# istellartech/GELATO

Measured on AMD Instinct MI355X. Metric: residual+Jacobian evals/sec (and ms/eval), 6-phase x 64-node LGR mesh, higher is better.
Workload: dtype f64

## Files before the change

gelato_amd/csrc/gel_eval_kernel.h:

```cpp
#pragma once

namespace gel {

enum ParkSlot { PK_Q0 = 0, PK_Q1, PK_Q2, PK_Q3, PK_V0, PK_V1, PK_V2, PK_DJJ, PK_LV0, PK_LV1, PK_LV2,
                PK_FP0, PK_FP1, PK_FP2, PK_FP3, PK_FP4, PK_FP5, PK_FP6, PK_FP7, PK_COUNT };
constexpr int kStageLd = 17;
constexpr int kWaveLds = PK_COUNT * 64;
static_assert(kWaveLds >= 64 * kStageLd, "the MFMA staging tile must fit the wave's park region");
constexpr int kCoopStageOff = PK_LV0 * 64;
static_assert(kWaveLds - kCoopStageOff >= 64 * 11, "the cooperative hand-over area must fit behind the early park slots");
constexpr int kXldsPipeFrom = kLongPhaseFrom;
constexpr int kSlabRowsMax = 68, kPackRows = 36, kParkRes = (PK_LV2 + 1) * 64;
constexpr int kPipeSlabK = 8;
constexpr int wave_lds_doubles(bool jac, bool mfma, bool pack, bool split = false, bool longp = true) {
  return jac ? kWaveLds : (!mfma ? kParkRes : (split ? 64 * kStageLd  : (pack ? kParkRes + 4 * 64  : (longp ? 2 * 4 * kPipeSlabK * 11 + 64 * kPipeSlabK  : kSlabRowsMax * 11))));
}
static_assert(wave_lds_doubles(false, true, false, true) >= kParkRes, "residual-only split form: park over the result tile");
static_assert(wave_lds_doubles(false, true, true) >= 64 * 11 && wave_lds_doubles(false, true, false) >= 64 * 11 && wave_lds_doubles(false, true, false, false, false) >= 64 * 11, "hand-over area");
static_assert(wave_lds_doubles(false, true, true) >= kParkRes && wave_lds_doubles(false, true, false) >= kParkRes && wave_lds_doubles(false, true, false, false, false) >= kParkRes, "residual-only park");

constexpr int kSlotPT = 0, kSlotVM = 3, kSlotVP = 6;

#ifndef GEL_MIN_WAVES_PER_SIMD
#define GEL_MIN_WAVES_PER_SIMD 4
#endif
#ifndef GEL_MIN_WAVES_PER_SIMD_PACKJAC
#define GEL_MIN_WAVES_PER_SIMD_PACKJAC 4
#endif
#ifndef GEL_MIN_WAVES_PER_SIMD_RES
#define GEL_MIN_WAVES_PER_SIMD_RES 5
#endif

typedef double gel_double4 __attribute__((ext_vector_type(4)));

#ifndef GEL_CA_CACHE
#define GEL_CA_CACHE 1
#endif
#ifndef GEL_XLDS_A_PF_JAC
#define GEL_XLDS_A_PF_JAC 4
#endif
#ifndef GEL_XLDS_A_PF_RES
#define GEL_XLDS_A_PF_RES 4
#endif
#ifndef GEL_PACK_A_PRELOAD
#define GEL_PACK_A_PRELOAD 1
#endif


#ifndef GEL_XCD_RANGES
#define GEL_XCD_RANGES 1
#endif
#ifndef GEL_XCD_BLOCK
#define GEL_XCD_BLOCK 0
#endif
#ifndef GEL_FRONT_BATCH
#define GEL_FRONT_BATCH 1
#endif
#ifndef GEL_DX_HOLD7
#define GEL_DX_HOLD7 1
#endif

#ifndef GEL_STORE_AUX
#define GEL_STORE_AUX 2
#endif

#ifndef GEL_AERO_STORE_AUX
#define GEL_AERO_STORE_AUX 2
#endif

template <bool JAC, bool MFMA, bool SPLIT = false, bool PACK = false, int SPLITB = 9, bool LONGP = true, bool NTS = true, bool AERO = false>
__device__ __forceinline__ void eval_body(const ProblemDev P, int B, const double* __restrict__ x, double* __restrict__ res,
                                          double* __restrict__ jvar, const unsigned vblk) {
  extern __shared__ double lds[];
  if (MFMA) __builtin_assume(res != nullptr);
  int fB = B, f_chunk0 = P.chunk0, f_vmajor = P.vmajor, f_nchunks = P.nchunks;
  const int4* f_chunks = P.chunks;
  const PhaseDev* f_phases = P.phases;
  if (GEL_FRONT_BATCH && MFMA && !SPLIT) asm volatile("" : "+s"(fB), "+s"(f_chunk0), "+s"(f_vmajor), "+s"(f_nchunks), "+s"(f_chunks), "+s"(f_phases));
  const int park_off = P.park_off;
  constexpr bool kSplitStage = MFMA && !SPLIT;
  const double tab_mine = kSplitStage ? stage_tables_issue(P) : 0.0;
  const Tables tb = kSplitStage ? table_view(lds, P.Kw, P.Kc) : stage_tables(P, lds, true);
  const int lane = threadIdx.x & 63;
  typedef __attribute__((address_space(3))) double lds_double;
  constexpr int kWL = wave_lds_doubles(JAC, MFMA, PACK, SPLIT, LONGP);
  constexpr int kHO = JAC ? kCoopStageOff : 0;
  static_assert(!(MFMA && !SPLIT) || kWL - kHO >= 64 * 11, "the cooperative hand-over area must fit the region");
  lds_double* wave_lds = (lds_double*)lds + park_off + (threadIdx.x >> 6) * kWL;
  lds_double* park = wave_lds + lane;
#define PARK_GET(slot) park[(slot) * 64]
#define PARK_SET(slot, val) park[(slot) * 64] = (val)

  constexpr bool COOP = MFMA && !SPLIT;
  static_assert(!AERO || (JAC && MFMA && !SPLIT && !PACK), "the aero rows ride in the cooperative form with derivatives, one vector per wavefront");
  static_assert(!COOP || kBlock == 256, "the cooperative D.X form is written for four wavefronts per workgroup");
  static_assert(!PACK || COOP, "two vectors per wavefront exist in the cooperative form only");
  constexpr int kVecWg = PACK ? 8 : 4;
  const int wv = __builtin_amdgcn_readfirstlane((int)(threadIdx.x >> 6));
  const int half = PACK ? (lane >> 5) : 0;
  const int nb4 = (fB + kVecWg - 1) / kVecWg;
  const long long item = COOP ? 0 : __builtin_amdgcn_readfirstlane((int)(((long long)vblk * blockDim.x + threadIdx.x) >> 6));
  if (!COOP && item >= (long long)B * (SPLIT ? P.nunits : P.nchunks)) return;
  int q, b0;
  int4 ck_it = int4{0, 0, 0, 0};
  bool ck_same = false;
  if (COOP) {
    const unsigned p = vblk, nb = (unsigned)nb4;
    unsigned it = p / nb, r = p - it * nb;
    if (f_vmajor) {
      const unsigned xcd = p & 7u, qq = p >> 3, items = (unsigned)f_nchunks;
      const unsigned gl = qq / items;
      it = qq - gl * items;
      r = gl * 8u + xcd;
      if (r >= nb) return;
    }
    ck_it = load_const_int4(f_chunks + f_chunk0 + it);
    const int cw = __builtin_amdgcn_readfirstlane(ck_it.w);
    const unsigned pos = (unsigned)cw >> 16, nc = (unsigned)cw & 0xffffu;
    unsigned c = pos, bg = r;
    if (nc > 1) {
      const unsigned l = pos * nb + r;
      const unsigned blk = l / (8 * nc), rem = l - blk * 8 * nc;
      const unsigned m = min(8u, nb - blk * 8);
      c = rem / m;
      bg = blk * 8 + (rem - c * m);
    }
    if (GEL_XCD_RANGES && !f_vmajor) {
      const unsigned G = GEL_XCD_BLOCK ? (unsigned)GEL_XCD_BLOCK : (nb >> 3), blk8 = 8u * G;
      if (G != 0) {
        const unsigned bq = bg / blk8, inb = bg - bq * blk8;
        if ((bq + 1u) * blk8 <= nb) bg = bq * blk8 + (p & 7u) * G + (inb >> 3);
      }
    }
    q = (int)(it - pos + c);
    ck_same = GEL_FRONT_BATCH && nc <= 1;
    b0 = (int)bg * kVecWg;
  } else {
    q = (int)(item / B);
    b0 = 0;
  }
  const int bw = PACK ? b0 + 2 * wv + half : b0 + wv;
  const bool ghost = COOP && bw >= fB;
  const bool pack_full = PACK && __builtin_amdgcn_ballot_w64(ghost) == 0;
  const int b = COOP ? min(bw, fB - 1) : (int)(item - (long long)q * B);
  const int ci = SPLIT ? ((P.unit0 + q) >> 2) : q;
  const int part = SPLIT ? ((P.unit0 + q) & 3) : 0;
  int4 ck = ck_it;
  if (!ck_same) ck = COOP ? load_const_int4(f_chunks + f_chunk0 + ci) : P.chunks[(SPLIT ? 0 : P.chunk0) + ci];
  const int sec = __builtin_amdgcn_readfirstlane(ck.x);
  const int j0 = __builtin_amdgcn_readfirstlane(ck.y);
  const int dsw = __builtin_amdgcn_readfirstlane(ck.z);
  const int j = PACK ? (lane & 31) : j0 + lane;
  const PhaseDev ph = load_phase((COOP ? f_phases : P.phases) + sec);
  const bool csplit = SPLIT && MFMA && !JAC && B == 1 && res != nullptr && P.split_vel && !((P.unit0 | P.nunits) & 3);
  const bool only_dx = SPLIT && part && (!ph.air || !JAC);
  if (only_dx && !csplit) return;
  const bool lead = !(SPLIT && part);
  const int n = ph.n;
  const bool active = j < n;
  if (!MFMA && !active) return;
  const int jc = active ? j : n - 1;
  const int g = ph.ua + j;
  const int xj = ph.xa + 1 + jc;
  const int M = P.M, N = P.N;

  const double* xb = x + (size_t)b * P.nvars;
  const double* xm = xb;
  const double* xr = xb + M;
  const double* xv = xb + 4 * M;
  const double* xq = xb + 7 * M;
  const double* xu = xb + 11 * M;
  const double* xt = xb + 11 * M + 2 * N;
#define GEL_UNI(v) (PACK ? (v) : wave_uniform(v))
#ifndef GEL_KNOT_VLOAD
#define GEL_KNOT_VLOAD 1
#endif
  int sec_ld = sec;
  if (GEL_KNOT_VLOAD && JAC && !SPLIT) asm volatile("" : "+v"(sec_ld));
  const double to_ld = xt[sec_ld], tf_ld = xt[sec_ld + 1];
  double to = 0.0, tf = 0.0, fds = 0.0, fdt = 0.0;
  const double dx = P.dx, ut = P.ut;
  const double hT = P.hT;
  const double inv_dx = P.inv_dx;
#define GEL_TAKE_KNOT_TIMES()                                   \
  do {                                                          \
    to = GEL_UNI(to_ld); tf = GEL_UNI(tf_ld);                   \
    fds = GEL_UNI(inv_dx * (tf - to) * ut / 2.0);               \
    fdt = GEL_UNI(inv_dx * ut / 2.0);                           \
  } while (0)
  unsigned long long bad = 0;
#define GEL_CHK(v) (bad |= __builtin_amdgcn_ballot_w64(!(fabs(v) <= 1.79769313486231570815e308)))
  const bool packed = SPLIT && P.shard_width != 0;
  const int nn = min(64, n - j0);
  const int sub_hi = packed ? (part ? kSlotVP + 3 * (part - 1) : (ph.air ? 9 : 0)) : 0;
  const int sub_lo = (packed && part) ? sub_hi : 0;
  const int pk_nj = (ph.K - sub_hi) * nn + (j0 == 0 ? 1 : 0);
  double* const pk_out = packed ? res + (size_t)b * P.shard_width + load_const(P.unit_base + P.unit0 + q) : nullptr;
  double* rb = packed ? (lead ? pk_out : nullptr) : ((res && lead) ? res + (size_t)b * 11 * N : nullptr);
  const int gn = packed ? lane : g;
  const int rs_m = packed ? pk_nj : 0, rs_p = packed ? pk_nj + nn : N, rs_v = packed ? pk_nj + 4 * nn : 4 * N,
            rs_q = packed ? pk_nj + 7 * nn : 7 * N;
  typedef unsigned gel_u2 __attribute__((ext_vector_type(2)));
  const __amdgpu_buffer_rsrc_t jrs =
      __builtin_amdgcn_make_buffer_rsrc(JAC ? (packed ? (void*)pk_out : (void*)(jvar + (size_t)(PACK ? min(b0 + 2 * wv, B - 1) : b) * P.V + ph.voff + (size_t)j0 * ph.K)) : (void*)nullptr,
                                        0, -1, 0x00020000);
  const int jvo = PACK ? (half * (int)P.V + j) * 8 : lane * 8;
  const int cw8 = nn * 8;
#define EMIT_AT(byteoff, val)                                                           \
  do {                                                                                  \
    const double _v = (val);                                                            \
    gel_u2 _d;                                                                          \
    __builtin_memcpy(&_d, &_v, 8);                                                      \
    __builtin_amdgcn_raw_buffer_store_b64(_d, jrs, jvo, (byteoff), NTS ? GEL_STORE_AUX : 0); \
    if (!rb) GEL_CHK(_v);                                                                 \
  } while (0)
#define EMIT(slot, val) EMIT_AT(((int)(slot) - (SPLIT ? (((int)(slot) >= kSlotVP) ? sub_hi : sub_lo) : 0)) * cw8, val)
  const AeroPhaseDev* const aph = AERO ? P.aero_ph + sec : nullptr;
  const int akinds = AERO ? __builtin_amdgcn_readfirstlane(load_const(&aph->kinds)) : 0;
  const __amdgpu_buffer_rsrc_t ars =
      __builtin_amdgcn_make_buffer_rsrc(AERO ? (void*)(P.aero_out + (size_t)b * P.aero_ld) : (void*)nullptr, 0, -1, 0x00020000);
#define AEMIT(byteoff, val)                                                              \
  do {                                                                                  \
    const double _v = (val);                                                            \
    gel_u2 _d;                                                                          \
    __builtin_memcpy(&_d, &_v, 8);                                                      \
    __builtin_amdgcn_raw_buffer_store_b64(_d, ars, jvo, (byteoff), GEL_AERO_STORE_AUX); \
  } while (0)
#define RSTORE(idx, val) do { if (SPLIT) __builtin_nontemporal_store((val), rb + (idx)); else rb[idx] = (val); } while (0)
#ifndef GEL_RES_XPOSE
#define GEL_RES_XPOSE 1
#endif
  constexpr int kTileOff = JAC ? PK_FP0 * 64 : kParkRes;
  constexpr bool kCanXpose = (GEL_RES_XPOSE != 0) && (kWL >= kTileOff + 4 * 64);
#define RSTORE_LINE(ptr, val) __builtin_nontemporal_store((val), (ptr))
#define xpose (kCanXpose && (PACK ? (cw8 == 256 && pack_full) : cw8 == 512))
#define RSTORE_ROWS(tile, w, rs_off, vals)                                                                   \
  do {                                                                                                       \
    _Pragma("unroll") for (int c_ = 0; c_ < (w); c_++) GEL_CHK((vals)[c_]);                                  \
    if (xpose) {                                                                                             \
      lds_double* t_ = (tile);                                                                               \
      _Pragma("unroll") for (int c_ = 0; c_ < (w); c_++) t_[(w) * lane + c_] = (vals)[c_];                   \
      _Pragma("unroll") for (int i_ = 0; i_ < (w); i_++) {                                                   \
        const double v_ = t_[64 * i_ + lane];                                                                \
        if (PACK) {                                                                                          \
          const int e_ = 64 * i_ + lane, h_ = (e_ >= 32 * (w)) ? 1 : 0;                                      \
          double* rbh_ = res + (size_t)(b0 + 2 * wv + h_) * 11 * N;                                          \
          RSTORE_LINE(rbh_ + (rs_off) + (w) * ph.ua + (e_ - 32 * (w) * h_), v_);                             \
        } else {                                                                                             \
          RSTORE_LINE(rb + (rs_off) + (w) * (gn - lane) + 64 * i_ + lane, v_);                               \
        }                                                                                                    \
      }                                                                                                      \
    } else {                                                                                                 \
      _Pragma("unroll") for (int c_ = 0; c_ < (w); c_++) RSTORE((rs_off) + (w) * gn + c_, (vals)[c_]);       \
    }                                                                                                        \
  } while (0)
  const double inv_uv = P.inv_uv;
#define FDQ(fp, fc) (((fc) - (fp)) * fds)
  const bool coo = SPLIT && !packed && P.coo_full != nullptr;
  enum { CG_PV = 0, CG_PT, CG_VM, CG_VP, CG_VQ, CG_VT, CG_QU, CG_QT };
#define GEL_COO_BASE(g) ((size_t)load_const(P.coo + 8 * sec + (g)))
#define GEL_COO_EMIT(W, base_, vals_, okl_, twin_)                                                                     \
  do {                                                                                                                 \
    double* d_ = P.coo_full + (base_) + (size_t)(W) * j0;                                                              \
    const unsigned long long okm_ = __builtin_amdgcn_ballot_w64(okl_);                                                 \
    _Pragma("unroll") for (int c_ = 0; c_ < (W); c_++) if (!rb) GEL_CHK((vals_)[c_]);                                  \
    if (cw8 == 512) {         \
      lds_double* t_ = wave_lds + kTileOff;                                                                            \
      _Pragma("unroll") for (int c_ = 0; c_ < (W); c_++) t_[(W) * lane + c_] = (vals_)[c_];                            \
      _Pragma("unroll") for (int i_ = 0; i_ < (W); i_++) {                                                             \
        const int e_ = 64 * i_ + lane;                                                                                 \
        const double v_ = t_[e_];                                                                                      \
        const int ln_ = ((W) == 4) ? (e_ >> 2) : ((e_ * 171) >> 9);             \
        if ((okm_ >> ln_) & 1ull) {                   \
          __builtin_nontemporal_store(v_, d_ + e_);                                                                    \
          if (twin_) __builtin_nontemporal_store(-v_, d_ + e_ + (W) * n);                                              \
        }                                                                                                              \
      }                                                                                                                \
    } else if (okl_) {         \
      _Pragma("unroll") for (int c_ = 0; c_ < (W); c_++) {                                                             \
        d_[(W) * lane + c_] = (vals_)[c_];                                                                             \
        if (twin_) d_[(W) * (n + lane) + c_] = -(vals_)[c_];                                                           \
      }                                                                                                                \
    }                                                                                                                  \
  } while (0)
#define EMIT_GROUP(W, slot0, vals_, g, k, twin_, okl_)                                                                 \
  do {                                                                                                                 \
    if (coo) {                                                                                                         \
      GEL_COO_EMIT(W, GEL_COO_BASE(g) + (size_t)(W) * n * (k), vals_, okl_, twin_);                                    \
    } else if (okl_) {                                                                                                 \
      _Pragma("unroll") for (int c_ = 0; c_ < (W); c_++) EMIT((slot0) + c_, (vals_)[c_]);                              \
    }                                                                                                                  \
  } while (0)

  constexpr bool XLDS = COOP;
  double me = 0.0, re[3] = {0.0, 0.0, 0.0};
  if (!XLDS) { me = xm[xj]; re[0] = xr[3 * xj]; re[1] = xr[3 * xj + 1]; re[2] = xr[3 * xj + 2]; }
  const double tau = P.tau[ph.toff + jc];
  {
    double q[4] = {0.0, 0.0, 0.0, 0.0}, ve[3] = {0.0, 0.0, 0.0};
    if (!XLDS) {
#pragma unroll
      for (int c = 0; c < 4; c++) q[c] = xq[4 * xj + c];
#pragma unroll
      for (int c = 0; c < 3; c++) ve[c] = xv[3 * xj + c];
    }
    double u0 = 0.0, u1 = 0.0;
    if (!ph.hold) { u0 = xu[2 * (ph.ua + jc)]; u1 = xu[2 * (ph.ua + jc) + 1]; }
    const double djj = JAC ? P.Dt[ph.doff + (size_t)(jc + 1) * n + jc] : 0.0;
    const bool tail1 = MFMA && ((n + 1) & 3) == 1 && n >= 4;
    const int ksteps = tail1 ? (n >> 2) : ((n + 4) >> 2);
    const double* const dcol = P.Dt + ph.doff + (size_t)n * n;
    double dl4[4] = {0, 0, 0, 0};
    if (COOP && tail1) {
      const int rt = PACK ? (wv & 1) : wv;
#pragma unroll
      for (int i = 0; i < 4; i++) dl4[i] = dcol[min(j0 + 16 * rt + (lane >> 4) + 4 * i, n - 1)];
    }
    const double dlast = (SPLIT && tail1) ? dcol[jc] : 0.0;
    double xl[11] = {0, 0, 0, 0, 0, 0, 0, 0, 0, 0, 0};
#define GEL_DX_TAIL_ACC(nct_, xn_of_ct)                                                             \
  do {                                                                                              \
    if (tail1) {                                                                                    \
      _Pragma("unroll") for (int ct = 0; ct < 3; ct++) {                                            \
        if (ct < (nct_)) {                                   \
          const double xn_ = (xn_of_ct);                                                            \
          _Pragma("unroll") for (int i = 0; i < 4; i++) acc[ct][i] = __builtin_fma(dl4[i], xn_, acc[ct][i]); \
        }                                                                                           \
      }                                                                                             \
    }                                                                                               \
  } while (0)

    double m0 = 0.0, q0[4] = {0, 0, 0, 0};
    bool ref0_done = false;
    double lm = 0.0, lr[3] = {0, 0, 0}, lv[3] = {0, 0, 0}, lq[4] = {0, 0, 0, 0};
    if (rb || csplit) {
      if (XLDS && (PACK || !LONGP || n < kXldsPipeFrom)) {
        const int c16 = lane & 15, kq = lane >> 4;
        constexpr int kSlabK = 17, kSlabRows = 4 * kSlabK;
        static_assert(kSlabRows == kSlabRowsMax, "slab size");
        static_assert(!COOP || kSlabRows * 11 <= kWL, "a slab of state rows must fit the wave's park region");
        lds_double* regions = (lds_double*)lds + park_off;
        const bool h7 = GEL_DX_HOLD7 && !PACK && ph.hold;
        const int ncv = h7 ? 7 : 11;
        const int ncols = ncv * kVecWg;
        const int ct0 = PACK ? (h7 ? 2 : 3) * (wv >> 1) : 0;
        int xoff[3];
#pragma unroll
        for (int ct = 0; ct < 3; ct++) {
          const int c = 16 * (ct0 + ct) + c16;
          const int vb = min(h7 ? c / 7 : c / 11, kVecWg - 1);
          const int col = (c < ncols) ? c - ncv * vb : 0;
          xoff[ct] = PACK ? (vb >> 1) * kWL + (vb & 1) * kPackRows * 11 + col + kq * 11 : vb * kWL + col + kq * 11;
        }
        gel_double4 acc[3];
        const double* ap = P.Dst + (size_t)dsw * 4 + (PACK ? (wv & 1) : wv) * 64 + lane;
        constexpr int kAPF = JAC ? GEL_XLDS_A_PF_JAC : GEL_XLDS_A_PF_RES;
        constexpr int kAllN = PACK ? 9 : kSlabK;
        constexpr bool kAAll = PACK ? (GEL_PACK_A_PRELOAD != 0) : (kAPF >= kSlabK);
        double a_all[kAAll ? kAllN : 1], a_ring[kAAll ? 1 : kAPF];
        if (kAAll) {
#pragma unroll
          for (int ks = 0; ks < kAllN; ks++) a_all[ks] = ap[min(ks, ksteps - 1) * 256];
        } else {
#pragma unroll
// ... 312 lines not shown
          lm = row[0];
#pragma unroll
          for (int c = 0; c < 3; c++) { lr[c] = row[1 + c]; lv[c] = row[4 + c]; }
#pragma unroll
          for (int c = 0; c < 4; c++) lq[c] = row[7 + c];
        }
      } else if (MFMA) {
        const int c16 = lane & 15, kq = lane >> 4;
        const double* bp = xm + ph.xa;
        int bs = 1;
        if (c16 >= 1 && c16 < 4) { bp = xr + 3 * ph.xa + (c16 - 1); bs = 3; }
        if (c16 >= 4 && c16 < 7) { bp = xv + 3 * ph.xa + (c16 - 4); bs = 3; }
        if (c16 >= 7) { bp = xq + 4 * ph.xa + ((c16 < 11) ? (c16 - 7) : 0); bs = 4; }
        gel_double4 acc[4];
#pragma unroll
        for (int t = 0; t < 4; t++) acc[t] = gel_double4{0.0, 0.0, 0.0, 0.0};
        const gel_double4* ap = reinterpret_cast<const gel_double4*>(P.Dsw) + (size_t)dsw * 1 + lane;
        const unsigned un = (unsigned)n, ubs = (unsigned)bs;
        if (tail1) {
          xl[0] = xm[ph.xa + n];
#pragma unroll
          for (int c = 0; c < 3; c++) { xl[1 + c] = xr[3 * (ph.xa + n) + c]; xl[4 + c] = xv[3 * (ph.xa + n) + c]; }
#pragma unroll
          for (int c = 0; c < 4; c++) xl[7 + c] = xq[4 * (ph.xa + n) + c];
        }
        constexpr int kSplitB = SPLITB, kSplitA = 2;
        for (int k0 = 0; k0 < ksteps; k0 += kSplitB) {
          double bl[kSplitB];
          gel_double4 a4[kSplitA];
#pragma unroll
          for (int i = 0; i < kSplitB; i++) bl[i] = bp[min(4u * (k0 + i) + kq, un) * ubs];
#pragma unroll
          for (int i = 0; i < kSplitA; i++) a4[i] = ap[min(k0 + i, ksteps - 1) * 64];
#pragma unroll
          for (int i = 0; i < kSplitB; i++) {
            if (k0 + i < ksteps) {
#pragma unroll
              for (int t = 0; t < 4; t++) acc[t] = __builtin_amdgcn_mfma_f64_16x16x4f64(a4[i % kSplitA][t], bl[i], acc[t], 0, 0, 0);
              a4[i % kSplitA] = ap[min(k0 + i + kSplitA, ksteps - 1) * 64];
            }
          }
        }
#pragma unroll
        for (int t = 0; t < 4; t++)
#pragma unroll
          for (int i = 0; i < 4; i++) wave_lds[(16 * t + kq + 4 * i) * kStageLd + c16] = acc[t][i];
        lds_double* row = wave_lds + lane * kStageLd;
        lm = row[0];
#pragma unroll
        for (int c = 0; c < 3; c++) { lr[c] = row[1 + c]; lv[c] = row[4 + c]; }
#pragma unroll
        for (int c = 0; c < 4; c++) lq[c] = row[7 + c];
      } else {
        const double* Dt = P.Dt + ph.doff + j;
        const double* pm = xm + ph.xa;
        const double* pr = xr + 3 * ph.xa;
        const double* pv = xv + 3 * ph.xa;
        const double* pq = xq + 4 * ph.xa;
        for (int i = 0; i <= n; i++) {
          const double d = Dt[(size_t)i * n];
          lm += d * pm[i];
#pragma unroll
          for (int c = 0; c < 3; c++) lr[c] += d * pr[3 * i + c];
#pragma unroll
          for (int c = 0; c < 3; c++) lv[c] += d * pv[3 * i + c];
#pragma unroll
          for (int c = 0; c < 4; c++) lq[c] += d * pq[4 * i + c];
        }
      }
    }
    GEL_TAKE_KNOT_TIMES();
#undef GEL_DX_TAIL_ACC
    if (SPLIT && tail1 && rb) {
      lm = __builtin_fma(dlast, xl[0], lm);
#pragma unroll
      for (int c = 0; c < 3; c++) { lr[c] = __builtin_fma(dlast, xl[1 + c], lr[c]); lv[c] = __builtin_fma(dlast, xl[4 + c], lv[c]); }
#pragma unroll
      for (int c = 0; c < 4; c++) lq[c] = __builtin_fma(dlast, xl[7 + c], lq[c]);
    }
    if (MFMA && !active) return;
    PARK_SET(PK_Q0, q[0]); PARK_SET(PK_Q1, q[1]); PARK_SET(PK_Q2, q[2]); PARK_SET(PK_Q3, q[3]);
    PARK_SET(PK_V0, ve[0]); PARK_SET(PK_V1, ve[1]); PARK_SET(PK_V2, ve[2]);
    if (JAC) PARK_SET(PK_DJJ, djj);
    if (rb) { PARK_SET(PK_LV0, lv[0]); PARK_SET(PK_LV1, lv[1]); PARK_SET(PK_LV2, lv[2]); }
    if (!ref0_done) {
      if (rb && !ph.engine_on) m0 = xm[ph.xa];
      if (rb && ph.hold) {
#pragma unroll
        for (int c = 0; c < 4; c++) q0[c] = xq[4 * ph.xa + c];
      }
    }

    if (JAC && lead) {
      if (coo) {
        const double sc = -(P.kpt * (tf - to));
        double* d_ = P.coo_full + GEL_COO_BASE(CG_PV) + (size_t)3 * j0;
#pragma unroll
        for (int i = 0; i < 3; i++) d_[(cw8 == 512) ? 64 * i + lane : 3 * lane + i] = sc;
      } else if (j == 0) EMIT_AT(packed ? (ph.K - sub_hi) * cw8 : ph.K * n * 8, -(P.kpt * (tf - to)));
      {
        const double pt[3] = {ve[0] * P.kpt, ve[1] * P.kpt, ve[2] * P.kpt};
        EMIT_GROUP(3, kSlotPT, pt, CG_PT, 0, true, true);
      }
    }
    if (!ph.hold && lead) {
      double fq[4];
      quat_rate(q, u0, u1, P.uu, fq);
      if (rb) {
        double cq[4];
#pragma unroll
        for (int c = 0; c < 4; c++) cq[c] = lq[c] - fq[c] * (tf - to) * hT;
        RSTORE_ROWS(wave_lds + kTileOff, 4, rs_q, cq);
      }
      if (JAC && ph.q_fd) {
        double f[4];
#pragma unroll
        for (int k = 0; k < 4; k++) {
          double qp[4];
#pragma unroll
          for (int c = 0; c < 4; c++) qp[c] = (k == c) ? (q[c] + dx) : q[c];
          quat_rate(qp, u0, u1, P.uu, f);
          const int c0 = (k < 2) ? 2 : 0;
          EMIT(ph.s_qq + 2 * k, FDQ(f[c0], fq[c0]));
          EMIT(ph.s_qq + 2 * k + 1, FDQ(f[c0 + 1], fq[c0 + 1]));
        }
#pragma unroll 1
        for (int k = 0; k < 2; k++) {
          quat_rate(q, (k == 0) ? u0 + dx : u0, (k == 1) ? u1 + dx : u1, P.uu, f);
#pragma unroll
          for (int c = 0; c < 4; c++) EMIT(ph.s_qq + 8 + 4 * k + c, FDQ(f[c], fq[c]));
        }
#pragma unroll
        for (int c = 0; c < 4; c++) EMIT(ph.s_qq + 16 + c, fq[c] * hT);
      } else if (JAC) {
        const double hS = (tf - to) * ut / 2.0;
        const double d2r = 0.017453292519943295769;
        EMIT(ph.s_qq + 0, 0.5 * ((u0 * P.uu) * d2r) * hS);
        EMIT(ph.s_qq + 1, 0.5 * ((u1 * P.uu) * d2r) * hS);
        const double kq = 0.5 * (P.uu * d2r) * hS;
        if (coo) {
          const double C0 = kq * q[0], C1 = kq * q[1], C2 = kq * q[2], C3 = kq * q[3];
          const double u0v[4] = {C2, C3, -C0, -C1}, u1v[4] = {C3, -C2, C1, -C0};
          EMIT_GROUP(4, 0, u0v, CG_QU, 0, false, true);
          EMIT_GROUP(4, 0, u1v, CG_QU, 1, false, true);
        } else {
          EMIT(ph.s_qq + 2, -(kq * q[0]));
          EMIT(ph.s_qq + 3, kq * q[1]);
          EMIT(ph.s_qq + 4, kq * q[2]);
          EMIT(ph.s_qq + 5, kq * q[3]);
        }
        {
          const double qt[4] = {fq[0] * hT, fq[1] * hT, fq[2] * hT, fq[3] * hT};
          EMIT_GROUP(4, ph.s_qq + 6, qt, CG_QT, 0, true, true);
        }
      }
    }
    if (rb) {
      double cm;
      if (ph.engine_on) {
        const double rh = ph.mf_um * (tf - to) * ut / 2.0;
        cm = lm - rh;
      } else {
        cm = me - m0;
      }
      RSTORE(rs_m + gn, cm);
      GEL_CHK(cm);
      {
        double cp[3];
        const double kpos = P.kpt * (tf - to);
#pragma unroll
        for (int c = 0; c < 3; c++) cp[c] = lr[c] - ve[c] * kpos;
        RSTORE_ROWS(wave_lds + kTileOff, 3, rs_p, cp);
      }
      if (ph.hold) {
        double cq[4];
#pragma unroll
        for (int c = 0; c < 4; c++) cq[c] = q[c] - q0[c];
        RSTORE_ROWS(wave_lds + kTileOff, 4, rs_q, cq);
      }
    }
  }
  asm volatile("" ::: "memory");

  double fc[3];
  {
    const double tn = tau * (tf - to) / 2 + (tf + to) / 2;
    const double inv_m = frcp(me * P.um);

#define GEL_QUAT_CLOSED(Tval)                                                                                          \
  do {                                                                                                                 \
    const double kq_ = ((Tval) * inv_m) * (inv_uv * fds);                                                              \
    const double q_[4] = {PARK_GET(PK_Q0), PARK_GET(PK_Q1), PARK_GET(PK_Q2), PARK_GET(PK_Q3)};                         \
    _Pragma("unroll") for (int k = 0; k < 4; k++) {                                                                    \
      const double dl_ = (q_[k] + dx) - q_[k];                                                                         \
      const double a_ = (k < 2) ? -(dl_ * kq_) : dl_ * kq_;    \
      const double b_ = -2.0 * (dl_ * kq_);                                                                            \
      const double vq_[3] = {(2.0 * q_[k] + dl_) * a_,                                                                 \
                             q_[3 - k] * b_,                                    \
                             ((k & 1) ? q_[k ^ 2] : -q_[k ^ 2]) * b_};        \
      EMIT_GROUP(3, ph.s_vq + 3 * k, vq_, CG_VQ, k, false, true);                                                      \
    }                                                                                                                  \
  } while (0)
#define GEL_MASS_CLOSED(tm_)                                                                                           \
  do {                                                                                                                 \
          \
    const double e_ = (fresh_product(me + dx, P.um) - fresh_product(me, P.um)) * inv_m;                                \
    const double k_ = (e_ * (1.0 - e_ * (1.0 - e_))) * (inv_uv * fds);                                                 \
    const double vm_[3] = {(tm_)[0] * k_, (tm_)[1] * k_, (tm_)[2] * k_};                                               \
    EMIT_GROUP(3, kSlotVM, vm_, CG_VM, 0, false, true);                                                                \
  } while (0)
    if (ph.air) {
      EarthHalf eh{1.0, 0.0};
      bool have_eh = false;
#define GEL_NEED_EARTH_ANGLE(ip_, wn_, we_)                                                                            \
  do {                                                                                                                 \
    if (!have_eh && __builtin_amdgcn_ballot_w64(wind_needs_angle(ip_, wn_, we_)) != 0) {                                \
      int jl_ = jc;                                                                                                    \
      if (AERO) asm volatile("" : "+v"(jl_));    \
      const double tau_ = P.tau[ph.toff + jl_];                                                                        \
      const EarthAngle e_ = earth_angle(tau_ * (tf - to) / 2 + (tf + to) / 2);                                         \
      eh.ch = e_.ch; eh.sh = e_.sh; have_eh = true;                                                                    \
    }                                                                                                                  \
  } while (0)
      PosCentreTail pt;
      double cen_rho = 0.0, cen_P = 0.0, cen_inv_a = 0.0;
      double dir2 = 0.0;
      EarthHalf aeh{1.0, 0.0};
      bool have_aeh = false;
#ifndef GEL_AEH
#define GEL_AEH aeh
#endif
#ifndef GEL_X_NOPOS
#define GEL_X_NOPOS 0
#endif
#ifndef GEL_X_NOQUAT
#define GEL_X_NOQUAT 0
#endif
#ifndef GEL_X_NOVEL
#define GEL_X_NOVEL 0
#endif
      const bool aero_on = AERO && akinds != 0;
      const bool a_need_alpha = AERO && (akinds & 5) != 0;
#define GEL_AERO_NEED_EA(ip_, wn_, we_)                                                                                \
  do {                                                                                                                 \
    if (!have_aeh && __builtin_amdgcn_ballot_w64(wind_needs_angle(ip_, wn_, we_)) != 0) {                               \
      int jl_ = jc;                                                                                                    \
      asm volatile("" : "+v"(jl_));    \
      const double tau_ = P.tau[ph.toff + jl_];                                                                        \
      const EarthAngle e_ = earth_angle((tau_ * (tf - to) / 2 + (tf + to) / 2) * P.ut);                                \
      aeh.ch = e_.ch; aeh.sh = e_.sh; have_aeh = true;                                                                 \
    }                                                                                                                  \
  } while (0)
#define GEL_AERO_FETCH()                                                                                               \
  const int ab_[3] = {load_const(&aph->base[0]), load_const(&aph->base[1]), load_const(&aph->base[2])};                \
  const double ax_[3] = {load_const(&aph->ilx[0]), load_const(&aph->ilx[1]), load_const(&aph->ilx[2])};                \
  const int n8_ = 8 * n, j08_ = 8 * j0
#define GEL_AERO_ENTRY(blk, col, a_, nv2_, d_, ind_, rho_, okl_, a_cc, a_ac, a_qc, a_isc, a_ok)                         \
  do {                                                                                                                 \
    double t_ = 0.0, dq_ = 0.0, qp_ = 0.0;                                                                             \
    const double ac_ = a_ac;                                                                                           \
    {                                                                                                                  \
      const double qc_ = a_qc;                                                                                         \
      qp_ = 0.5 * (rho_) * (nv2_);                                                                                     \
      dq_ = qp_ - qc_;                                                                                                 \
      if (a_need_alpha) {                                                                                              \
        const double cp_ = aero_cos(a_, nv2_, d_, ind_);                                                               \
        const bool okd_ = aero_dalpha(cp_, nv2_, a_cc, a_isc, a_ok, t_);                                               \
        if (__builtin_amdgcn_ballot_w64(!okd_) != 0) {                                                                 \
          const double t2_ = aero_acos(cp_, nv2_) - ac_;                                                               \
          t_ = okd_ ? t_ : t2_;                                                                                        \
        }                                                                                                              \
      }                                                                                                                \
    }                                                                                                                  \
    _Pragma("unroll") for (int kind = 0; kind < 3; kind++) {                                                           \
      if ((blk) == 2 && kind == 1) continue;                             \
      const double df_ = (kind == 0) ? t_ : ((kind == 1) ? dq_ : qp_ * t_ + dq_ * ac_);                                \
      const double gv = -(df_ * ax_[kind]);                                                                            \
      if (okl_) AEMIT(ab_[kind] + (((blk) == 0 ? 1 : ((blk) == 1 ? 4 : 7)) + (col)) * n8_ + j08_, gv);                 \
    }                                                                                                                  \
  } while (0)
#if GEL_CA_CACHE
      Bracket ca_br = no_bracket();
#define GEL_CA_BRACKET (JAC ? &ca_br : (Bracket*)nullptr)
#else
#define GEL_CA_BRACKET nullptr
#endif
      struct ParkSink { lds_double* park; GEL_DEV void put(int i, double v) const { if (!(AERO && (i == PCS_P || i == PCS_IH))) park[(PK_FP0 + i) * 64] = v; } };
      constexpr int PK_ACC = PK_FP0 + PCS_P, PK_AAC = PK_FP0 + PCS_IH, PK_AQC = PK_LV2;
      static_assert(PCS_COUNT == 8 && PK_FP7 == PK_FP0 + 7, "PosCentre's early members fill FP0-7");
      {
        PosPart pp;
        double v[3], w[3], F[3], dir[3];
        const double r[3] = {fresh_product(re[0], P.up), fresh_product(re[1], P.up), fresh_product(re[2], P.up)};
        if (JAC) pp = pos_part<true, ParkSink>(r, tb, P.barC20, nullptr, ParkSink{park}, &pt);
        else pp = pos_part(r, tb, P.barC20);
        const bool cen_windy = AERO && __builtin_amdgcn_ballot_w64(!(pp.wn == 0.0 && pp.we == 0.0)) != 0;
        if (__builtin_amdgcn_ballot_w64(wind_needs_angle(pp.inv_p, pp.wn, pp.we)) != 0) {
          const EarthAngle e0 = earth_angle(tn);
          eh.ch = e0.ch; eh.sh = e0.sh; have_eh = true;
          if (aero_on) PARK_SET(PK_ACC, tn);
        }
        EarthAngle ea{1.0, 0.0, 1.0, 0.0};
        if (have_eh) ea = full_angle(eh);
        wind_eci_or_calm(r, ea, pp.shp, pp.chp, pp.inv_p, pp.wn, pp.we, w);
#pragma unroll
        for (int c = 0; c < 3; c++) v[c] = PARK_GET(PK_V0 + c) * P.uv;
        aero_force(r, v, pp.rho, pp.inv_a, w, ph.area, tb, F, GEL_CA_BRACKET);
#define GEL_T (ph.thrust - ph.nozzle * pp.P)
#define GEL_TDC(name) const double name[3] = {GEL_T * dir[0], GEL_T * dir[1], GEL_T * dir[2]}
        {
          const double q[4] = {PARK_GET(PK_Q0), PARK_GET(PK_Q1), PARK_GET(PK_Q2), PARK_GET(PK_Q3)};
          thrust_dir(q, dir);
        }
        double tm[3];
        {
          GEL_TDC(Tdc);
          accel_parts(Tdc, F, inv_m, pp.g, inv_uv, tm, fc);
        }
        if (rb) {
#ifndef GEL_RES_XPOSE_VEL_AIR
#define GEL_RES_XPOSE_VEL_AIR 1
#endif
          if (!JAC || GEL_RES_XPOSE_VEL_AIR) {
            double cv[3];
#pragma unroll
            for (int c = 0; c < 3; c++) cv[c] = PARK_GET(PK_LV0 + c) - fc[c] * (tf - to) * hT;
            RSTORE_ROWS(wave_lds + PK_LV0 * 64, 3, rs_v, cv);
          } else {
#pragma unroll
            for (int c = 0; c < 3; c++) {
              const double cv = PARK_GET(PK_LV0 + c) - fc[c] * (tf - to) * hT;
              RSTORE(rs_v + 3 * gn + c, cv);
              GEL_CHK(cv);
            }
          }
        }
        if (JAC) {
          asm volatile("" ::: "memory");
          PARK_SET(PK_LV0, pp.shp); PARK_SET(PK_LV1, pp.chp);
          if (!AERO) PARK_SET(PK_LV2, pp.inv_p);
        }
        if (JAC && lead && !P.fd_recompute) GEL_MASS_CLOSED(tm);
        if (JAC && ph.air_fd && (SPLIT && P.split_vel ? !lead : lead)) {
          double f[3];
          {
            const double djj = PARK_GET(PK_DJJ);
#pragma unroll
            for (int k = 0; k < 3; k++) {
              if (SPLIT && P.split_vel && k != part - 1) continue;
              double vp[3], Fp[3];
#pragma unroll
              for (int c = 0; c < 3; c++) vp[c] = ((k == c) ? (PARK_GET(PK_V0 + c) + dx) : PARK_GET(PK_V0 + c)) * P.uv;
              const double r[3] = {fresh_product(re[0], P.up), fresh_product(re[1], P.up), fresh_product(re[2], P.up)};
              aero_force(r, vp, pp.rho, pp.inv_a, w, ph.area, tb, Fp, GEL_CA_BRACKET);
              GEL_TDC(Tdc);
              accel(Tdc, Fp, inv_m, pp.g, inv_uv, f);
#pragma unroll
              for (int c = 0; c < 3; c++) EMIT(ph.s_vv + 3 * k + c, ((c == k) ? djj : 0.0) + FDQ(f[c], fc[c]));
            }
          }
        }
        if (JAC && lead) {
          double f[3];
          if (!P.fd_recompute) {
            GEL_QUAT_CLOSED(GEL_T);
          } else if (P.fd_recompute) {
            const double q[4] = {PARK_GET(PK_Q0), PARK_GET(PK_Q1), PARK_GET(PK_Q2), PARK_GET(PK_Q3)};
#pragma unroll 1
            for (int k = 0; k < 4; k++) {
              double qp[4];
#pragma unroll
              for (int c = 0; c < 4; c++) qp[c] = (k == c) ? (q[c] + dx) : q[c];
              double dp[3];
              thrust_dir(qp, dp);
              const double Td[3] = {GEL_T * dp[0], GEL_T * dp[1], GEL_T * dp[2]};
              accel(Td, F, inv_m, pp.g, inv_uv, f);
#pragma unroll
              for (int c = 0; c < 3; c++) EMIT(ph.s_vq + 3 * k + c, FDQ(f[c], fc[c]));
            }
            GEL_TDC(Tdc);
            accel(Tdc, F, frcp((me + dx) * P.um), pp.g, inv_uv, f);
#pragma unroll
            for (int c = 0; c < 3; c++) EMIT(kSlotVM + c, FDQ(f[c], fc[c]));
          }
          if (!ph.t_fd) {
            const double vt[3] = {fc[0] * hT, fc[1] * hT, fc[2] * hT};
            EMIT_GROUP(3, ph.s_vt, vt, CG_VT, 0, true, true);
          }
        }
        if (aero_on) {
          asm volatile("" ::: "memory");
          const double ra[3] = {fresh_product(re[0], P.up), fresh_product(re[1], P.up), fresh_product(re[2], P.up)};
          double va[3], wa[3], a0[3];
#pragma unroll
          for (int c = 0; c < 3; c++) va[c] = PARK_GET(PK_V0 + c) * P.uv;
          if (have_eh) {
            const EarthAngle e1 = earth_angle(PARK_GET(PK_ACC) * P.ut);
            aeh.ch = e1.ch; aeh.sh = e1.sh; have_aeh = true;
          }
          if (cen_windy) {
            PosCentre pcx;
            double wn_, we_, p_, ip_, ih_;
            pos_centre_tail(pt, pp.rho, pp.P, tb, pcx, wn_, we_);
            geodetic_p_ih(ra[0], ra[1], ra[2], p_, ip_, ih_);
            EarthAngle e2{1.0, 0.0, 1.0, 0.0};
            if (have_aeh) e2 = full_angle(GEL_AEH);
            wind_eci(ra, e2, PARK_GET(PK_LV0), PARK_GET(PK_LV1), ip_, wn_, we_, wa);
          } else {
            wa[0] = 0.0; wa[1] = 0.0; wa[2] = 0.0;
          }
          const double nv2 = aero_vair2(ra, va, wa, a0);
          const double ind = frsqrt(fmax(dir[0] * dir[0] + dir[1] * dir[1] + dir[2] * dir[2], 1.0e-300));
          const double cc = a_need_alpha ? aero_cos(a0, nv2, dir, ind) : 0.0;
          const double alpha_c = a_need_alpha ? aero_acos(cc, nv2) : 0.0;
          const double qdyn_c = 0.5 * pp.rho * nv2;
          double sc, isc;
          fsqrt_rsqrt(fmax((1.0 - cc) * (1.0 + cc), 1.0e-300), sc, isc);
          const bool centre_ok = (cc <= 1.0) && (nv2 >= 1.0e-12) && (sc > 1.0e-6);
          GEL_AERO_FETCH();
          const double ail_[3] = {load_const(&aph->il[0]), load_const(&aph->il[1]), load_const(&aph->il[2])};
#pragma unroll
          for (int kind = 0; kind < 3; kind++) {
            const double il = ail_[kind];
            const double cv = 1.0 - ((kind == 0) ? alpha_c : (kind == 1) ? qdyn_c : qdyn_c * alpha_c) * il;
            AEMIT(ab_[kind] + j08_, cv);
            GEL_CHK(cv);
          }
          if (a_need_alpha && !GEL_X_NOQUAT) {
            const double q[4] = {PARK_GET(PK_Q0), PARK_GET(PK_Q1), PARK_GET(PK_Q2), PARK_GET(PK_Q3)};
#pragma unroll
            for (int c = 0; c < 4; c++) {
              double qp[4], dp[3];
#pragma unroll
              for (int d = 0; d < 4; d++) qp[d] = (d == c) ? q[d] + dx : q[d];
              thrust_dir(qp, dp);
              const double indp = frsqrt(fmax(dp[0] * dp[0] + dp[1] * dp[1] + dp[2] * dp[2], 1.0e-300));
              GEL_AERO_ENTRY(2, c, a0, nv2, dp, indp, pp.rho, true, cc, alpha_c, qdyn_c, isc, centre_ok);
              __builtin_amdgcn_sched_barrier(0);
            }
          }
#pragma unroll
          for (int c = 0; c < (GEL_X_NOVEL ? 0 : 3); c++) {
            double vp[3], a[3];
#pragma unroll
            for (int d = 0; d < 3; d++) vp[d] = ((d == c) ? PARK_GET(PK_V0 + d) + dx : PARK_GET(PK_V0 + d)) * P.uv;
            const double nv2p = aero_vair2(ra, vp, wa, a);
            GEL_AERO_ENTRY(1, c, a, nv2p, dir, ind, pp.rho, true, cc, alpha_c, qdyn_c, isc, centre_ok);
            __builtin_amdgcn_sched_barrier(0);
          }
          PARK_SET(PK_ACC, cc); PARK_SET(PK_AAC, centre_ok ? alpha_c : -alpha_c); PARK_SET(PK_AQC, qdyn_c);
        }
        if (JAC) {
          asm volatile("" ::: "memory");
          PARK_SET(PK_Q0, fc[0]); PARK_SET(PK_Q1, fc[1]); PARK_SET(PK_Q2, fc[2]); PARK_SET(PK_Q3, dir[0]); PARK_SET(PK_DJJ, dir[1]);
          dir2 = dir[2];
          cen_rho = pp.rho; cen_P = pp.P; cen_inv_a = pp.inv_a;
        }
#undef GEL_TDC
#undef GEL_T
      }
      if (JAC && (!SPLIT || part)) {
        const int k0 = SPLIT ? part - 1 : 0, k1 = SPLIT ? part : 3;
#define GEL_POS_SWEEP_F(rp, pq, f_)                                                                           \
  do {                                                                                                        \
    double wq_[3], Fp_[3];                                                                                    \
    GEL_NEED_EARTH_ANGLE((pq).inv_p, (pq).wn, (pq).we);                                                       \
    EarthAngle ea{1.0, 0.0, 1.0, 0.0};                                                                        \
    if (have_eh) ea = full_angle(eh);                                                                         \
    wind_eci_or_calm(rp, ea, (pq).shp, (pq).chp, (pq).inv_p, (pq).wn, (pq).we, wq_);                          \
    const double vq_[3] = {PARK_GET(PK_V0) * P.uv, PARK_GET(PK_V1) * P.uv, PARK_GET(PK_V2) * P.uv};           \
    aero_force(rp, vq_, (pq).rho, (pq).inv_a, wq_, ph.area, tb, Fp_, GEL_CA_BRACKET);                         \
    const double Tp_ = ph.thrust - ph.nozzle * (pq).P;                                                        \
    const double Td_[3] = {Tp_ * PARK_GET(PK_Q3), Tp_ * PARK_GET(PK_DJJ), Tp_ * dir2};                        \
    accel(Td_, Fp_, inv_m, (pq).g, inv_uv, f_);                                                               \
  } while (0)
#define GEL_POS_SWEEP_EMIT(kk, f_, okl_)                                                                      \
  do {                                                                                                        \
    const double vp_[3] = {FDQ((f_)[0], PARK_GET(PK_Q0)), FDQ((f_)[1], PARK_GET(PK_Q1)), FDQ((f_)[2], PARK_GET(PK_Q2))}; \
    EMIT_GROUP(3, kSlotVP + 3 * (kk), vp_, CG_VP, kk, false, okl_);                                           \
  } while (0)
#define GEL_AERO_POS(kk, rp, pq, okl_)                                                                        \
  do {                                                                                                        \
    double wq_[3], a_[3];                                                                                     \
    GEL_AERO_NEED_EA((pq).inv_p, (pq).wn, (pq).we);                                                           \
    EarthAngle ea_{1.0, 0.0, 1.0, 0.0};                                                                       \
    if (have_aeh) ea_ = full_angle(GEL_AEH);                                                                  \
    wind_eci_or_calm(rp, ea_, (pq).shp, (pq).chp, (pq).inv_p, (pq).wn, (pq).we, wq_);                         \
    const double vq_[3] = {PARK_GET(PK_V0) * P.uv, PARK_GET(PK_V1) * P.uv, PARK_GET(PK_V2) * P.uv};           \
    const double nv2_ = aero_vair2(rp, vq_, wq_, a_);                                                         \
    const double dd_[3] = {PARK_GET(PK_Q3), PARK_GET(PK_DJJ), dir2};                                          \
    const double ind_ = frsqrt(fmax(dd_[0] * dd_[0] + dd_[1] * dd_[1] + dd_[2] * dd_[2], 1.0e-300));          \
    const double cc_ = PARK_GET(PK_ACC);                                                                      \
    double sc_, isc_;                                                                                         \
    fsqrt_rsqrt(fmax((1.0 - cc_) * (1.0 + cc_), 1.0e-300), sc_, isc_);                                        \
    const double acs_ = PARK_GET(PK_AAC);    \
    GEL_AERO_FETCH();                                                                                         \
    GEL_AERO_ENTRY(0, kk, a_, nv2_, dd_, ind_, (pq).rho, okl_, cc_, fabs(acs_), PARK_GET(PK_AQC), isc_, !__builtin_signbit(acs_)); \
  } while (0)
#define GEL_LOAD_POS_CENTRE(pc, pcv)                                                                                   \
  PosCentre pc;                                                                                                        \
  pc.ihy = PARK_GET(PK_FP0 + PCS_IHY);                                                                                 \
  pc.sl = PARK_GET(PK_FP0 + PCS_SL); pc.cl = PARK_GET(PK_FP0 + PCS_CL); pc.icl = PARK_GET(PK_FP0 + PCS_ICL);           \
  pc.N = PARK_GET(PK_FP0 + PCS_N); pc.G = PARK_GET(PK_FP0 + PCS_G);                                                    \
  PosPart pcv;                                                                                                         \
  pcv.rho = cen_rho; pcv.P = cen_P; pcv.inv_a = cen_inv_a;                                                             \
  pcv.shp = PARK_GET(PK_LV0); pcv.chp = PARK_GET(PK_LV1);                                                              \
  if (AERO) {                                                                                                          \
    geodetic_p_ih(fresh_product(re[0], P.up), fresh_product(re[1], P.up), fresh_product(re[2], P.up), pc.p, pcv.inv_p, pc.ih); \
  } else {                                                                                                             \
    pc.p = PARK_GET(PK_FP0 + PCS_P); pc.ih = PARK_GET(PK_FP0 + PCS_IH); pcv.inv_p = PARK_GET(PK_LV2);                  \
  }                                                                                                                    \
  pos_centre_tail(pt, cen_rho, cen_P, tb, pc, pcv.wn, pcv.we)
        unsigned todo = 0;
        unsigned long long coo_okm = 0;
        if (P.fd_recompute) {
          todo = ((1u << k1) - 1u) & ~((1u << k0) - 1u);
        } else {
#pragma unroll
          for (int k = k0; k < k1; k++) {
            asm volatile("" ::: "memory");
            GEL_LOAD_POS_CENTRE(pc, pcv);
            const double r[3] = {fresh_product(re[0], P.up), fresh_product(re[1], P.up), fresh_product(re[2], P.up)};
            double rp[3];
#pragma unroll
            for (int c = 0; c < 3; c++) rp[c] = (k == c) ? (re[c] + dx) * P.up : r[c];
            const double dlt = (k == 0) ? rp[0] - r[0] : ((k == 1) ? rp[1] - r[1] : rp[2] - r[2]);
            PosPart pq;
            const bool ok = pos_delta(r, k, dlt, pcv, pc, tb, pq);
            if (coo) coo_okm = __builtin_amdgcn_ballot_w64(ok);
            if (__builtin_amdgcn_ballot_w64(!ok) != 0) {
              todo |= 1u << k;
              if (__builtin_amdgcn_ballot_w64(ok) == 0) continue;
            }
            gravity_eci(rp, P.barC20, pq.g);
            double f[3];
            GEL_POS_SWEEP_F(rp, pq, f);
            GEL_POS_SWEEP_EMIT(k, f, ok);
            if (aero_on && !GEL_X_NOPOS) GEL_AERO_POS(k, rp, pq, ok);
          }
        }
        if (todo) {
#pragma unroll 1
          for (int k = k0; k < k1; k++) {
            if (!((todo >> k) & 1u)) continue;
            asm volatile("" ::: "memory");
            double rp[3];
#pragma unroll
            for (int c = 0; c < 3; c++) rp[c] = fresh_product((k == c) ? re[c] + dx : re[c], P.up);
            bool ok = false;
            if (!P.fd_recompute && coo) {
              ok = ((coo_okm >> lane) & 1ull) != 0;
            } else if (!P.fd_recompute) {
              GEL_LOAD_POS_CENTRE(pc, pcv);
              const double r[3] = {fresh_product(re[0], P.up), fresh_product(re[1], P.up), fresh_product(re[2], P.up)};
              const double dlt = (k == 0) ? rp[0] - r[0] : ((k == 1) ? rp[1] - r[1] : rp[2] - r[2]);
              PosPart pd;
              ok = pos_delta(r, k, dlt, pcv, pc, tb, pd);
            }
            asm volatile("" ::: "memory");
            PosPart pq = pos_part(rp, tb, P.barC20);
            double f[3];
            GEL_POS_SWEEP_F(rp, pq, f);
            GEL_POS_SWEEP_EMIT(k, f, !ok);
            if (aero_on && !GEL_X_NOPOS) GEL_AERO_POS(k, rp, pq, !ok);
          }
        }
#undef GEL_AERO_POS
#undef GEL_LOAD_POS_CENTRE
#undef GEL_NEED_EARTH_ANGLE
#undef GEL_AERO_NEED_EA
#undef GEL_AERO_ENTRY
#undef GEL_AERO_FETCH
#undef GEL_POS_SWEEP_F
#undef GEL_POS_SWEEP_EMIT
      }
      if (JAC && lead && ph.t_fd) {
        asm volatile("" ::: "memory");
        const double fcc[3] = {PARK_GET(PK_Q0), PARK_GET(PK_Q1), PARK_GET(PK_Q2)};
        int jl2 = jc;
        if (AERO) asm volatile("" : "+v"(jl2));
        const double tau2 = P.tau[ph.toff + jl2];
        {
          const double r[3] = {fresh_product(re[0], P.up), fresh_product(re[1], P.up), fresh_product(re[2], P.up)};
          const PosPart p2 = pos_part(r, tb, P.barC20);
          const double T2 = ph.thrust - ph.nozzle * p2.P;
          PARK_SET(PK_FP0, p2.shp); PARK_SET(PK_FP1, p2.chp); PARK_SET(PK_FP2, p2.inv_p); PARK_SET(PK_FP3, p2.wn); PARK_SET(PK_FP4, p2.we);
          PARK_SET(PK_FP5, p2.rho); PARK_SET(PK_FP6, p2.inv_a);
          PARK_SET(PK_LV0, p2.g[0]); PARK_SET(PK_LV1, p2.g[1]); PARK_SET(PK_LV2, p2.g[2]);
          PARK_SET(PK_Q0, T2 * PARK_GET(PK_Q3)); PARK_SET(PK_Q1, T2 * PARK_GET(PK_DJJ)); PARK_SET(PK_Q2, T2 * dir2);
        }
#pragma unroll 1
        for (int k = 0; k < 2; k++) {
          asm volatile("" ::: "memory");
          const double to_p = (k == 0) ? to + dx : to;
          const double tf_p = (k == 1) ? tf + dx : tf;
          const double tnp = tau2 * (tf_p - to_p) / 2 + (tf_p + to_p) / 2;
          const EarthAngle eq = earth_angle(tnp);
          double wq[3], Fp[3], f[3];
          const double rq[3] = {re[0] * P.up, re[1] * P.up, re[2] * P.up};
          wind_eci_chain_or_calm(rq, eq, PARK_GET(PK_FP0), PARK_GET(PK_FP1), PARK_GET(PK_FP2), PARK_GET(PK_FP3), PARK_GET(PK_FP4), wq);
          const double vq[3] = {PARK_GET(PK_V0) * P.uv, PARK_GET(PK_V1) * P.uv, PARK_GET(PK_V2) * P.uv};
          aero_force(rq, vq, PARK_GET(PK_FP5), PARK_GET(PK_FP6), wq, ph.area, tb, Fp, GEL_CA_BRACKET);
          const double Tq[3] = {PARK_GET(PK_Q0), PARK_GET(PK_Q1), PARK_GET(PK_Q2)};
          const double gq[3] = {PARK_GET(PK_LV0), PARK_GET(PK_LV1), PARK_GET(PK_LV2)};
          accel(Tq, Fp, inv_m, gq, inv_uv, f);
#pragma unroll
          for (int c = 0; c < 3; c++)
            EMIT(ph.s_vt + 3 * k + c, (fcc[c] * (tf - to) - f[c] * (tf_p - to_p)) * fdt);
        }
      }
    } else {
      const double T = ph.thrust;
      double dir[3];
      {
        const double q[4] = {PARK_GET(PK_Q0), PARK_GET(PK_Q1), PARK_GET(PK_Q2), PARK_GET(PK_Q3)};
        thrust_dir(q, dir);
      }
      const double Td[3] = {T * dir[0], T * dir[1], T * dir[2]};
      double gc[3];
      {
        const double r[3] = {re[0] * P.up, re[1] * P.up, re[2] * P.up};
        gravity_eci(r, P.barC20, gc);
      }
      double tm[3];
#pragma unroll
      for (int c = 0; c < 3; c++) { tm[c] = Td[c] * inv_m; fc[c] = (tm[c] + gc[c]) * inv_uv; }
      if (rb) {
        double cv[3];
#pragma unroll
        for (int c = 0; c < 3; c++) cv[c] = PARK_GET(PK_LV0 + c) - fc[c] * (tf - to) * hT;
        RSTORE_ROWS(wave_lds + PK_LV0 * 64, 3, rs_v, cv);
      }
      if (JAC) {
        double f[3];
        if (!P.fd_recompute) {
          GEL_MASS_CLOSED(tm);
        } else {
          accel_noair(Td, frcp((me + dx) * P.um), gc, inv_uv, f);
#pragma unroll
          for (int c = 0; c < 3; c++) EMIT(kSlotVM + c, FDQ(f[c], fc[c]));
        }
#pragma unroll
        for (int k = 0; k < 3; k++) {
          double r[3], gp[3];
#pragma unroll
          for (int c = 0; c < 3; c++) r[c] = ((k == c) ? (re[c] + dx) : re[c]) * P.up;
          gravity_eci(r, P.barC20, gp);
          accel_noair(Td, inv_m, gp, inv_uv, f);
          const double vp[3] = {FDQ(f[0], fc[0]), FDQ(f[1], fc[1]), FDQ(f[2], fc[2])};
          EMIT_GROUP(3, kSlotVP + 3 * k, vp, CG_VP, k, false, true);
        }
        if (!P.fd_recompute) {
          GEL_QUAT_CLOSED(T);
        } else {
          const double q[4] = {PARK_GET(PK_Q0), PARK_GET(PK_Q1), PARK_GET(PK_Q2), PARK_GET(PK_Q3)};
#pragma unroll 1
          for (int k = 0; k < 4; k++) {
            double qp[4];
#pragma unroll
            for (int c = 0; c < 4; c++) qp[c] = (k == c) ? (q[c] + dx) : q[c];
            double dp[3];
            thrust_dir(qp, dp);
            const double Tp[3] = {T * dp[0], T * dp[1], T * dp[2]};
            accel_noair(Tp, inv_m, gc, inv_uv, f);
#pragma unroll
            for (int c = 0; c < 3; c++) EMIT(ph.s_vq + 3 * k + c, FDQ(f[c], fc[c]));
          }
        }
        {
          const double vt[3] = {fc[0] * hT, fc[1] * hT, fc[2] * hT};
          EMIT_GROUP(3, ph.s_vt, vt, CG_VT, 0, true, true);
        }
      }
    }
  }
#undef EMIT_GROUP
#undef GEL_COO_EMIT
#undef GEL_COO_BASE
#undef EMIT
#undef GEL_CA_BRACKET
#undef GEL_QUAT_CLOSED
#undef GEL_MASS_CLOSED
#undef AEMIT
#undef EMIT_AT
#undef RSTORE
#undef RSTORE_ROWS
#undef RSTORE_LINE
#undef xpose
#undef FDQ
#undef GEL_CHK
#undef GEL_UNI
#undef GEL_TAKE_KNOT_TIMES
#undef PARK_GET
#undef PARK_SET
  if (bad) *(volatile int32_t*)P.flag = 1;
}

__device__ __forceinline__ void signal_done(const ProblemDev& P) {
  if (!P.done_flag) return;
  __threadfence_system();
  __syncthreads();
  if (threadIdx.x == 0) {
    const int old = __hip_atomic_fetch_add(P.done_ctr, 1, __ATOMIC_ACQ_REL, __HIP_MEMORY_SCOPE_AGENT);
    if (old == P.done_total - 1) {
      __hip_atomic_store(P.done_ctr, 0, __ATOMIC_RELAXED, __HIP_MEMORY_SCOPE_AGENT);
      __hip_atomic_store(P.done_flag, P.done_seq, __ATOMIC_RELEASE, __HIP_MEMORY_SCOPE_SYSTEM);
    }
  }
}

template <bool JAC, bool MFMA, bool SPLIT = false, bool PACK = false, bool LONGP = true, bool NTS = true, bool AERO = false>
__global__ __launch_bounds__(kBlock, (!JAC && PACK) ? GEL_MIN_WAVES_PER_SIMD_RES : ((JAC && PACK) ? GEL_MIN_WAVES_PER_SIMD_PACKJAC : GEL_MIN_WAVES_PER_SIMD)) void eval_kernel(ProblemDev P, int B, const double* __restrict__ x,
                                                      double* __restrict__ res, double* __restrict__ jvar) {
  eval_body<JAC, MFMA, SPLIT, PACK, 9, LONGP, NTS, AERO>(P, B, x, res, jvar, blockIdx.x);
  if constexpr (SPLIT) signal_done(P);
}

}
```

gelato_amd/csrc/gel_host.hip:

```cpp
#include <hip/hip_runtime.h>

#include <algorithm>
#include <cmath>
#include <cstdio>
#include <chrono>
#include <atomic>
#include <cstdlib>
#include <cstring>
#include <memory>
#include <string>
#include <thread>
#include <vector>

#include "gel_host_handle.h"

namespace gelhost {
namespace {
thread_local std::string g_err;
}
int fail(int code, const std::string& msg) {
  g_err = msg;
  return code;
}
}
// ... 1036 lines not shown
        const int64_t nn = std::min(64, h.n - j0);
        const int skip = h.air ? 9 : 0;
        usize[4 * item] = (int64_t)(h.K - skip) * nn + (j0 == 0 ? 1 : 0) + 11 * nn;
        for (int k = 1; k < 4; k++) usize[4 * item + k] = h.air ? 3 * nn : 0;
      }
  }
  std::vector<int64_t> base(nunits, 0);
  int64_t w = 0;
  for (int r = 0; r < nranks; r++) {
    int64_t off = 0;
    for (int u = unit_begin[r]; u < unit_begin[r + 1]; u++) { base[u] = off; off += usize[u]; }
    w = std::max(w, off);
  }
  w = (w + 1) & ~(int64_t)1;
  {
    int item = 0;
    for (const HostPhase& h : p->ph)
      for (int j0 = 0; j0 < h.n; j0 += 64, item++) {
        const int nn = std::min(64, h.n - j0);
        const int skip = h.air ? 9 : 0;
        const int64_t nj = (int64_t)(h.K - skip) * nn + (j0 == 0 ? 1 : 0);
        const int u0 = 4 * item;
        const int64_t b0 = (int64_t)urank[u0] * w + base[u0];
        for (int jl = 0; jl < nn; jl++) {
          const int j = j0 + jl, g = h.ua + j;
          pos[g] = b0 + nj + jl;
          for (int c = 0; c < 3; c++) { pos[N + 3 * g + c] = b0 + nj + nn + 3 * jl + c; pos[4 * N + 3 * g + c] = b0 + nj + 4 * nn + 3 * jl + c; }
          for (int c = 0; c < 4; c++) pos[7 * N + 4 * g + c] = b0 + nj + 7 * nn + 4 * jl + c;
          for (int sl = 0; sl < h.K; sl++) {
            const int part = (h.air && sl >= 6 && sl < 15) ? 1 + (sl - 6) / 3 : 0;
            const int u = u0 + part;
            const int local = part ? sl - (6 + 3 * (part - 1)) : (sl >= 6 ? sl - skip : sl);
            pos[(size_t)11 * N + compact_index(h, sl, j)] = (int64_t)urank[u] * w + base[u] + (int64_t)local * nn + jl;
          }
        }
        if (j0 == 0) pos[(size_t)11 * N + h.voff + (int64_t)h.K * h.n] = b0 + (int64_t)(h.K - skip) * nn;
      }
  }
  for (int64_t v : pos)
    if (v < 0) return fail(GEL_ERR_ARG, "shard plan: an output entry without an owner (internal)");
  DeviceArray<int64_t> d_base, d_pos;
  if (p->device != GEL_DEVICE_NONE) {
    HIPCHK(hipSetDevice(p->device));
    HIPCHK(d_base.upload(base)); HIPCHK(d_pos.upload(pos));
    HIPCHK(drain(p));
  }
  p->d_unit_base = std::move(d_base);
  p->d_shard_pos = std::move(d_pos);
  p->shard_begin.assign(unit_begin, unit_begin + nranks + 1);
  p->unit_base = base;
  p->shard_width = w;
  *width = w;
  if (res_pos) std::memcpy(res_pos, pos.data(), sizeof(int64_t) * 11 * (size_t)N);
  if (jvar_pos) std::memcpy(jvar_pos, pos.data() + (size_t)11 * N, sizeof(int64_t) * (size_t)V);
  return GEL_OK;
}

static int check_plan(const gel_problem* p, int32_t nranks, int64_t width) {
  if (p->shard_width <= 0) return fail(GEL_ERR_ARG, "gel_shard_plan has not been called on this handle");
  if (nranks != (int32_t)p->shard_begin.size() - 1 || width != p->shard_width)
    return fail(GEL_ERR_ARG, "the handle's shard plan is not the one this buffer was sized for (gel_shard_plan was called again: plan once more, or use one handle per plan)");
  return GEL_OK;
}

int gel_eval_shard_packed_device(gel_problem* p, int32_t B, const double* d_x, double* d_out, int32_t rank, int32_t nranks_expected,
                                 int64_t width_expected, void* stream) {
  if (!p || !d_x || !d_out || B < 1) return fail(GEL_ERR_ARG, "bad argument");
  NO_EXACT(p, "gel_eval_shard_packed_device");
  NEED_DEVICE(p, GEL_ERR_HIP, kNoGpu);
  if (int rc = check_plan(p, nranks_expected, width_expected)) return rc;
  if (!p->d_unit_base.get()) return fail(GEL_ERR_ARG, "gel_shard_plan has not been called on this handle");
  const int nranks = (int)p->shard_begin.size() - 1;
  if (rank < 0 || rank >= nranks) return fail(GEL_ERR_ARG, "rank outside the plan");
  const int32_t u0 = p->shard_begin[rank], cnt = p->shard_begin[rank + 1] - u0;
  if (cnt == 0) return GEL_OK;
  gel::ProblemDev dv = p->dev;
  dv.chunks = p->d_chunks.get();
  dv.chunk0 = 0;
  dv.unit0 = u0;
  dv.nunits = cnt;
  dv.shard_width = p->shard_width;
  dv.unit_base = p->d_unit_base.get();
  double* slice = d_out + (size_t)rank * (size_t)B * (size_t)p->shard_width;
  HIPCHK(gel::launch_eval(dv, B, d_x, slice, slice, stream_of(p, stream)));
  return GEL_OK;
}

int gel_shard_unpack_device(gel_problem* p, int32_t B, const double* d_out, double* d_res, double* d_jvar, int32_t nranks_expected,
                            int64_t width_expected, void* stream) {
  if (!p || !d_out || B < 1 || (!d_res && !d_jvar)) return fail(GEL_ERR_ARG, "bad argument");
  NEED_DEVICE(p, GEL_ERR_HIP, kNoGpu);
  if (int rc = check_plan(p, nranks_expected, width_expected)) return rc;
  if (!p->d_shard_pos.get()) return fail(GEL_ERR_ARG, "gel_shard_plan has not been called on this handle");
  HIPCHK(gel::launch_shard_unpack(11 * p->dims.N, p->dims.num_var_entries, p->shard_width, B, p->d_shard_pos.get(), d_out, d_res, d_jvar,
                                  stream_of(p, stream)));
  return GEL_OK;
}

int gel_fill_full_device(gel_problem* p, int32_t B, double* d_jfull, void* stream) {
  if (!p || !d_jfull || B < 1) return fail(GEL_ERR_ARG, "bad argument");
  NEED_DEVICE(p, GEL_ERR_HIP, kNoGpu);
  HIPCHK(gel::launch_fill_full(p->dims.total_nnz, B, p->d_cval.get(), d_jfull, stream_of(p, stream)));
  return GEL_OK;
}

int gel_update_full_device(gel_problem* p, int32_t B, const double* d_jvar, double* d_jfull, void* stream) {
  if (!p || !d_jvar || !d_jfull || B < 1) return fail(GEL_ERR_ARG, "bad argument");
  NEED_DEVICE(p, GEL_ERR_HIP, kNoGpu);
  HIPCHK(gel::launch_update_full(p->dims.total_nnz, p->dims.num_var_entries, p->nvar_entries, B, p->d_vdst.get(), p->d_vsrc.get(),
                                 p->nvar_lines, p->d_vline.get(), p->d_src.get(), p->d_cval.get(), d_jvar, d_jfull,
                                 stream_of(p, stream)));
  return GEL_OK;
}

int gel_eval_full_device(gel_problem* p, int32_t B, const double* d_x, double* d_res, double* d_jvar, double* d_jfull, void* stream) {
  if (!p || !d_x || !d_jvar || !d_jfull || B < 1) return fail(GEL_ERR_ARG, "bad argument");
  NEED_DEVICE(p, GEL_ERR_HIP, kNoGpu);
  hipStream_t s = stream_of(p, stream);
  gel::ProblemDev dv = p->dev;
  dv.cached_out = 1;
  HIPCHK(launch_defects(p, dv, B, d_x, d_res, d_jvar, s));
  HIPCHK(gel::launch_update_full(p->dims.total_nnz, p->dims.num_var_entries, p->nvar_entries, B, p->d_vdst.get(), p->d_vsrc.get(),
                                 p->nvar_lines, p->d_vline.get(), p->d_src.get(), p->d_cval.get(), d_jvar, d_jfull, s));
  return GEL_OK;
}

int gel_expand_full_device(gel_problem* p, int32_t B, const double* d_jvar, double* d_jfull, void* stream) {
  if (!p || !d_jvar || !d_jfull || B < 1) return fail(GEL_ERR_ARG, "bad argument");
  NEED_DEVICE(p, GEL_ERR_HIP, kNoGpu);
  HIPCHK(gel::launch_expand(p->dims.total_nnz, p->dims.num_var_entries, B, p->d_cval.get(), p->d_src.get(), d_jvar, d_jfull,
                            stream_of(p, stream)));
  return GEL_OK;
}

int gel_sync(gel_problem* p, void* stream) {
  if (!p) return fail(GEL_ERR_ARG, "null argument");
  NEED_DEVICE(p, GEL_ERR_HIP, kNoGpu);
  hipStream_t s = stream_of(p, stream);
  HIPCHK(hipMemcpyAsync(p->h_flag.get(), p->d_flag.get(), 4, hipMemcpyDeviceToHost, s));
  HIPCHK(hipStreamSynchronize(s));
  int rc = GEL_OK;
  if (*p->h_flag.get()) {
    HIPCHK(clear_flag(p, s));
    *p->h_flag.get() = 0;
    rc = GEL_NONFINITE;
  }
  if (s == p->caller_stream) p->caller_stream = nullptr;
  return rc;
}

int gel_output_table(gel_problem* p, const double* x, const double* tx_res, double launch_lat_deg, double launch_lon_deg,
                     double* out) {
  if (!p || !x || !tx_res || !out) return fail(GEL_ERR_ARG, "null argument");
  NEED_DEVICE(p, GEL_ERR_HIP, kNoGpu);
  HIPCHK(hipSetDevice(p->device));
  const int M = p->dims.M;
  std::vector<int32_t> sec((size_t)M);
  for (size_t i = 0; i < p->ph.size(); i++)
    for (int k = 0; k <= p->ph[i].n; k++) sec[(size_t)p->ph[i].xa + k] = (int32_t)i;
  const size_t nx = (size_t)p->dims.num_vars, no = (size_t)M * gel::kOutputColumns;
  return staged_call(p, kStagedNoFlag, {staged_in(x, nx), staged_in(tx_res, (size_t)M), staged_in(sec.data(), (size_t)M), staged_out(out, no)},
                     [&](const gel::ProblemDev&, double* const* a) -> int {
                       HIPCHK(gel::launch_output(p->dev, M, a[0], a[1], reinterpret_cast<const int32_t*>(a[2]), launch_lat_deg, launch_lon_deg,
                                                 a[3], p->stream.get()));
                       return GEL_OK;
                     });
}

int gel_initial_guess(const gel_problem* p, int32_t nref, const double* t_ref, const double* table,
                      const double* knot_times, double* x) {
  if (!p || !t_ref || !table || !knot_times || !x || nref < 2) return fail(GEL_ERR_ARG, "bad argument (>= 2 reference rows)");
  for (int k = 1; k < nref; k++)
    if (!(t_ref[k] >= t_ref[k - 1])) return fail(GEL_ERR_ARG, "reference times must not decrease");
  const int S = p->dims.S, M = p->dims.M, N = p->dims.N;
  auto interp = [&](double t, int col0, int ncol, double unit, double* out) {
    int hi = (int)(std::lower_bound(t_ref, t_ref + nref, t) - t_ref);
    hi = std::min(std::max(hi, 1), nref - 1);
    const int lo = hi - 1;
    for (int c = 0; c < ncol; c++) {
      const double ylo = table[(size_t)lo * 13 + col0 + c], yhi = table[(size_t)hi * 13 + col0 + c];
      const double slope = (yhi - ylo) / (t_ref[hi] - t_ref[lo]);
      const double rise = slope * (t - t_ref[lo]);
      out[c] = (rise + ylo) / unit;
    }
  };
  double* xm = x; double* xr = x + M; double* xv = x + 4 * (size_t)M; double* xq = x + 7 * (size_t)M;
  double* xu = x + 11 * (size_t)M; double* xt = x + 11 * (size_t)M + 2 * (size_t)N;
  for (int i = 0; i < S; i++) {
    const HostPhase& h = p->ph[i];
    const double to = knot_times[i], tf = knot_times[i + 1];
    for (int k = 0; k <= h.n; k++) {
      const double tau = (k == 0) ? -1.0 : h.tau[k - 1];
      const double t = tau * (tf - to) / 2.0 + (tf + to) / 2.0;
      const int node = h.xa + k;
      interp(t, 0, 1, p->um, xm + node);
      interp(t, 1, 3, p->up, xr + 3 * (size_t)node);
      interp(t, 4, 3, p->uv, xv + 3 * (size_t)node);
      interp(t, 7, 4, 1.0, xq + 4 * (size_t)node);
    }
    for (int k = 0; k < h.n; k++) {
      const double t = h.tau[k] * (tf - to) / 2.0 + (tf + to) / 2.0;
      interp(t, 11, 2, p->uu, xu + 2 * (size_t)(h.ua + k));
    }
  }
  for (int i = 0; i <= S; i++) xt[i] = knot_times[i] / p->ut;
  for (int64_t i = 0; i < p->dims.num_vars; i++)
    if (!std::isfinite(x[i])) return GEL_NONFINITE;
  return GEL_OK;
}

int gel_eval_callback(gel_problem* p, const double* x, const gel_callback_io* io) {
  if (!p || !x || !io) return fail(GEL_ERR_ARG, "null argument");
  NEED_DEVICE(p, GEL_ERR_HIP, kNoGpu);
  HIPCHK(hipSetDevice(p->device));
  int rc = ensure_capacity(p, 1);
  if (rc) return rc;
  const size_t nlin = p->lin_rows.size(), nfn = p->fn_rows.size(), R = nlin + nfn;
  const bool rows = io->rows_con && R;
  size_t off_c[3], off_j[3], atotal = 0;
  bool aero = false;
  for (int k = 0; k < 3; k++) {
    const size_t n = p->aero.rows[k].size();
    off_c[k] = atotal; atotal += (io->aero_con[k] && n) ? n : 0;
    off_j[k] = atotal; atotal += (io->aero_con[k] && n && io->aero_jac[k]) ? aero_jac_len(p, k) : 0;
    aero = aero || (io->aero_con[k] && n);
  }
  const size_t nrows_out = rows ? R + 7 * nfn : 0;
  if (rows || aero) HIPCHK(p->h_arena.reserve(nrows_out + atotal));
  double* const h_rows = p->h_arena.get();
  double* const h_aero = h_rows + nrows_out;
  const bool x_pinned = p->cb_x[0].get() && (x == p->cb_x[0].get() || x == p->cb_x[1].get());
  if (!x_pinned) std::memcpy(p->h_x.get(), x, (size_t)p->dims.num_vars * 8);
  const double* const xin = x_pinned ? x : p->h_x.get();
  gel::ProblemDev dv = p->dev;
  dv.flag = p->h_flag.get();
  const bool want_jac = io->vals_full != nullptr;
  const bool fused = io->res || want_jac;
  static const int cb_mode = [] { const char* e = getenv("GEL_CB_MODE"); return e ? atoi(e) : 0; }();
  const bool split_exact = p->exact && want_jac;
  bool aero_jac = false;
  for (int k = 0; k < 3; k++) aero_jac = aero_jac || (io->aero_con[k] && io->aero_jac[k] && !p->aero.rows[k].empty());
  const bool split_aero = p->exact_aero && aero_jac;
  const bool split_rows = p->exact_rows && rows && io->rows_jfn;
  const bool coo = want_jac && cb_mode != 3 && !p->exact && !split_aero && !split_rows && coo_direct(p);
  if (coo) {
    if ((rc = ensure_full(p))) return rc;
    dv.coo_full = p->h_full.get(); dv.coo = p->d_coo.get();
  }
  dv.split_vel = 1;
  const bool own_res = io->res && p->cb_res.get() && io->res == p->cb_res.get();
  double* const res_to = own_res ? p->cb_res.get() : p->h_res.get();
  gel::AeroLaunchOut out;
  if (aero)
    for (int k = 0; k < 3; k++) {
      const size_t n = p->aero.rows[k].size();
      out.nrows[k] = (int32_t)n;
      out.con[k] = (io->aero_con[k] && n) ? h_aero + off_c[k] : nullptr;
      out.jac[k] = (out.con[k] && io->aero_jac[k]) ? h_aero + off_j[k] : nullptr;
    }
  if (cb_mode == 3 || !fused || split_exact || split_aero || split_rows) {
    if (fused) HIPCHK(launch_defects(p, dv, 1, xin, res_to, want_jac ? p->h_jv.get() : nullptr, p->stream.get()));
    if (rows) HIPCHK(launch_rows_kinds(p, dv, 1, xin, h_rows, io->rows_jfn ? h_rows + R : nullptr, p->stream.get()));
    if (aero) HIPCHK(launch_aero_kinds(p, dv, (int)p->aero.nodes.size(), p->aero.d_nodes.get(), 1, xin, out, p->stream.get()));
  } else {
    arm_done(p, dv);
    HIPCHK(gel::launch_callback(dv, want_jac, xin, res_to, want_jac ? p->h_jv.get() : nullptr,
                                aero ? (int)p->aero.nodes.size() : 0, p->aero.d_nodes.get(), aero ? &out : nullptr,
                                (int)nlin, p->d_lin_rows.get(), (int)nfn, p->d_fn_rows.get(), rows ? h_rows : nullptr,
                                (rows && io->rows_jfn) ? h_rows + R : nullptr, p->stream.get()));
  }
  HIPCHK(wait_done(p, dv));
  if (io->res && !own_res) std::memcpy(io->res, p->h_res.get(), (size_t)11 * p->dims.N * 8);
  if (want_jac) {
    if (coo) finish_full(p, io->vals_full, io->fill_constants);
    else scatter_full(p, p->h_jv.get(), io->vals_full, io->fill_constants);
  }
  if (rows) {
    std::memcpy(io->rows_con, h_rows, R * 8);
    if (io->rows_jfn) std::memcpy(io->rows_jfn, h_rows + R, 7 * nfn * 8);
  }
  if (aero)
    for (int k = 0; k < 3; k++) {
      if (out.con[k]) std::memcpy(io->aero_con[k], out.con[k], p->aero.rows[k].size() * 8);
      if (out.jac[k]) std::memcpy(io->aero_jac[k], out.jac[k], aero_jac_len(p, k) * 8);
    }
  if (*p->h_flag.get()) { *p->h_flag.get() = 0; return GEL_NONFINITE; }
  return GEL_OK;
}

int gel_table_limits(int32_t wind_rows, int32_t ca_rows, int32_t n, int64_t* info) {
  if (wind_rows < 2 || ca_rows < 2 || !info) return fail(GEL_ERR_ARG, "bad argument");
  const size_t T = gel::staged_table_doubles(wind_rows, ca_rows), Tp = gel::padded_table_doubles(wind_rows, ca_rows);
  info[0] = (int64_t)T;
  info[1] = (int64_t)lds_room(gel::eval_lds_bytes_max(wind_rows, ca_rows) / 8 - Tp, true);
  info[2] = (int64_t)lds_room(gel::aero_lds_bytes(wind_rows, ca_rows) / 8 - Tp, true);
  info[3] = (n >= 2 && n < gel::kMeshMaxThreads) ? (int64_t)lds_room(gel::mesh_vector_doubles(n), true) : -1;
  info[4] = (int64_t)lds_room(gel::table_lds_bytes(wind_rows, ca_rows) / 8 - T, false);
  info[5] = (int64_t)gel::kLaunchMaxLds;
  info[6] = info[3] < 0 ? -1 : (int64_t)gel::mesh_vectors_per_group(wind_rows, ca_rows, n);
  return GEL_OK;
}

int gel_point_eval(int32_t kind, int32_t n, const double* in, const double* aux, int32_t aux_rows, double* out) {
  static const int nin[16] = {1, 3, 3, 6, 7, 1, 1, 2, 2, 8, 8, 8, 7, 4, 1, 5}, nout[16] = {5, 3, 3, 3, 3, 3, 1, 4, 6, 8, 16, 4, 3, 7, 2, 18};
  if (kind < 0 || kind > 15 || n < 0 || !in || !out) return fail(GEL_ERR_ARG, "bad argument");
  if (n == 0) return GEL_OK;
  const bool tabulated = kind == 5 || kind == 6 || kind == 9 || kind == 10 || kind == 15;
  int rc = tabulated ? check_launch_lds("gel_point_eval", gel::point_lds_bytes(aux_rows), 5 * (size_t)std::max(aux_rows, 0), 5 * (size_t)std::max(aux_rows, 0), false) : GEL_OK;
  if (rc) return rc;
  rc = need_device();
  if (rc) return rc;
  double atm[gel::kAtmTableDoubles];
  size_t naux = 0;
  const double* hax = aux;
  std::vector<double> ext;
  if (kind == 0) { gel::fill_atmosphere_table(atm); hax = atm; naux = gel::kAtmTableDoubles; aux_rows = 0; }
  else if (kind == 2) { if (!aux) return fail(GEL_ERR_ARG, "kind 2 needs aux[0] = barC20"); naux = 1; aux_rows = 0; }
  else if (tabulated) {
    const int w = (kind == 5 || kind == 10 || kind == 15) ? 3 : 2;
    if (!aux || aux_rows < 2) return fail(GEL_ERR_ARG, "kinds 5, 6, 9, 10 and 15 need a table of at least two rows");
    if (kind == 15) { gel::fill_atmosphere_table(atm); ext.assign(atm, atm + gel::kAtmTableDoubles); }
    for (int k = 1; k < aux_rows; k++)
      if (!(aux[(size_t)w * k] > aux[(size_t)w * (k - 1)])) return fail(GEL_ERR_ARG, "table abscissae must increase strictly");
    std::vector<double> slopes;
    gel::append_rows_and_slopes(ext, slopes, aux, aux_rows, w);
    ext.insert(ext.end(), slopes.begin(), slopes.end());
    hax = ext.data(); naux = ext.size();
  }
  else { aux_rows = 0; }
  DeviceArray<double> i, a, o;
  HIPCHK(i.upload(in, (size_t)n * nin[kind])); HIPCHK(a.upload(hax, naux)); HIPCHK(o.reserve((size_t)n * nout[kind]));
  HIPCHK(gel::launch_point(kind, n, i.get(), a.get(), aux_rows, o.get(), nullptr));
  HIPCHK(hipMemcpy(out, o.get(), (size_t)n * nout[kind] * 8, hipMemcpyDeviceToHost));
  return GEL_OK;
}

}
```

gelato_amd/csrc/gel_kernels.hip:

```cpp
#include <hip/hip_runtime.h>

#include "gel_tables.h"
#include "gel_output_row.h"

#include "gel_eval_kernel.h"
namespace gel {

constexpr int kExpandGroup = 8;
__global__ __launch_bounds__(kBlock) void expand_kernel(long long nnz, long long V, int B, const double* __restrict__ cval,
                                                        const int32_t* __restrict__ src,
                                                        const double* __restrict__ jvar, double* __restrict__ full) {
  const int b0 = blockIdx.y * kExpandGroup;
  const int nb = min(kExpandGroup, B - b0);
  const bool even = (nnz & 1) == 0;
  for (long long i = 2 * ((long long)blockIdx.x * kBlock + threadIdx.x); i < nnz; i += 2LL * gridDim.x * kBlock) {
    const bool two = i + 1 < nnz;
    const int s0 = src[i], s1 = two ? src[i + 1] : -1;
    const double c0 = (s0 == -1) ? cval[i] : 0.0, c1 = (two && s1 == -1) ? cval[i + 1] : 0.0;
    const int g0 = (s0 >= 0) ? s0 : -2 - s0, g1 = (s1 >= 0) ? s1 : -2 - s1;
    for (int g = 0; g < nb; g++) {
      const double* jv = jvar + (size_t)(b0 + g) * V;
      double* out = full + (size_t)(b0 + g) * nnz + i;
      const double v0 = (s0 == -1) ? c0 : ((s0 >= 0) ? jv[g0] : -jv[g0]);
      const double v1 = (s1 == -1) ? c1 : ((s1 >= 0) ? jv[g1] : -jv[g1]);
      if (two && (even || ((b0 + g) & 1) == 0)) {
        typedef double gel_d2 __attribute__((ext_vector_type(2)));
        __builtin_nontemporal_store(gel_d2{v0, v1}, reinterpret_cast<gel_d2*>(out));
      } else {
        __builtin_nontemporal_store(v0, out);
        if (two) __builtin_nontemporal_store(v1, out + 1);
      }
    }
  }
}

__global__ __launch_bounds__(kBlock) void update_full_kernel(long long nnz, long long V, int nvar, int B, const int32_t* __restrict__ vdst,
                                                             const int32_t* __restrict__ vsrc, const double* __restrict__ jvar,
                                                             double* __restrict__ full) {
  const int i = blockIdx.x * kBlock + threadIdx.x;
  if (i >= nvar) return;
  const int d = vdst[i], s = vsrc[i];
  const int g = (s >= 0) ? s : -2 - s;
  for (int b = blockIdx.y; b < B; b += gridDim.y) {
    const double v = jvar[(size_t)b * V + g];
    full[(size_t)b * nnz + d] = (s >= 0) ? v : -v;
  }
}
__global__ __launch_bounds__(kBlock) void update_lines_kernel(long long nnz, long long V, int nlines, int B, const int32_t* __restrict__ vline,
                                                              const int32_t* __restrict__ src, const double* __restrict__ cval,
                                                              const double* __restrict__ jvar, double* __restrict__ full) {
  const int t = blockIdx.x * kBlock + threadIdx.x;
  if (t >= 8 * nlines) return;
  const long long i = 8LL * vline[t >> 3] + (t & 7);
  const int s = src[i];
  const double c = (s == -1) ? cval[i] : 0.0;
  const int g = (s >= 0) ? s : -2 - s;
  for (int b = blockIdx.y; b < B; b += gridDim.y) {
    double v = c;
    if (s != -1) { const double w = jvar[(size_t)b * V + g]; v = (s >= 0) ? w : -w; }
    __builtin_nontemporal_store(v, full + (size_t)b * nnz + i);
  }
}
__global__ __launch_bounds__(kBlock) void fill_full_kernel(long long nnz, int B, const double* __restrict__ cval, double* __restrict__ full) {
  for (long long i = (long long)blockIdx.x * kBlock + threadIdx.x; i < nnz; i += (long long)gridDim.x * kBlock) {
    const double c = cval[i];
    for (int b = blockIdx.y; b < B; b += gridDim.y) __builtin_nontemporal_store(c, full + (size_t)b * nnz + i);
  }
}

__global__ void perturb_local_kernel(int nloc, double dx, const double* __restrict__ x, const int32_t* __restrict__ colmap,
                                     double* __restrict__ Xp) {
  const long long t = (long long)blockIdx.x * blockDim.x + threadIdx.x;
  if (t >= (long long)(nloc + 1) * nloc) return;
  const int row = (int)(t / nloc), col = (int)(t - (long long)row * nloc);
  double v = x[colmap[col]];
  if (row == col + 1) v += dx;
  Xp[t] = v;
}

__global__ void quotient_local_kernel(int nloc, int nres, int roff, int nrows, double dx, const double* __restrict__ res,
                                      double* __restrict__ J, long long ldJ, int row0, const int32_t* __restrict__ colmap) {
  __shared__ double tile[32][33];
  const int c0 = blockIdx.x * 32, r0 = blockIdx.y * 32;
  for (int k = threadIdx.y; k < 32; k += blockDim.y) {
    const int c = c0 + k, r = r0 + threadIdx.x;
    if (c < nloc && r < nrows) tile[k][threadIdx.x] = res[(size_t)(c + 1) * nres + roff + r];
  }
  __syncthreads();
  for (int k = threadIdx.y; k < 32; k += blockDim.y) {
    const int r = r0 + k, c = c0 + threadIdx.x;
    if (c < nloc && r < nrows) J[(size_t)(row0 + r) * ldJ + (colmap ? colmap[c] : c)] = (tile[threadIdx.x][k] - res[roff + r]) / dx;
  }
}

struct RhsArgs {
  int n, Kw, Kc;
  const double *mass_e, *pos_e, *vel_e, *quat, *t, *tables;
  double thrust, area, nozzle, um, up, uv, barC20;
  double* out;
};

__global__ void rhs_vel_air_kernel(RhsArgs A) {
  extern __shared__ double lds[];
  ProblemDev P{};
  P.Kw = A.Kw; P.Kc = A.Kc; P.tables = A.tables;
  const Tables tb = stage_tables(P, lds);
  const int i = blockIdx.x * blockDim.x + threadIdx.x;
  if (i >= A.n) return;
  const double m = A.mass_e[i] * A.um;
  const double r[3] = {A.pos_e[3 * i] * A.up, A.pos_e[3 * i + 1] * A.up, A.pos_e[3 * i + 2] * A.up};
  const double v[3] = {A.vel_e[3 * i] * A.uv, A.vel_e[3 * i + 1] * A.uv, A.vel_e[3 * i + 2] * A.uv};
  const double q[4] = {A.quat[4 * i], A.quat[4 * i + 1], A.quat[4 * i + 2], A.quat[4 * i + 3]};
  const PosPart pp = pos_part(r, tb, A.barC20);
  const EarthAngle ea = earth_angle(A.t[i]);
  double w[3], F[3], dir[3], f[3];
  wind_eci(r, ea, pp.shp, pp.chp, pp.inv_p, pp.wn, pp.we, w);
  aero_force(r, v, pp.rho, pp.inv_a, w, A.area, tb, F);
  thrust_dir(q, dir);
  const double T = A.thrust - A.nozzle * pp.P;
  const double Td[3] = {T * dir[0], T * dir[1], T * dir[2]};
  accel(Td, F, 1.0 / m, pp.g, 1.0 / A.uv, f);
  for (int c = 0; c < 3; c++) A.out[3 * i + c] = f[c];
}

__global__ void rhs_vel_noair_kernel(RhsArgs A) {
  const int i = blockIdx.x * blockDim.x + threadIdx.x;
  if (i >= A.n) return;
  const double m = A.mass_e[i] * A.um;
  const double r[3] = {A.pos_e[3 * i] * A.up, A.pos_e[3 * i + 1] * A.up, A.pos_e[3 * i + 2] * A.up};
  const double q[4] = {A.quat[4 * i], A.quat[4 * i + 1], A.quat[4 * i + 2], A.quat[4 * i + 3]};
  double dir[3], g[3], f[3];
  thrust_dir(q, dir);
  gravity_eci(r, A.barC20, g);
  const double Td[3] = {A.thrust * dir[0], A.thrust * dir[1], A.thrust * dir[2]};
  accel_noair(Td, 1.0 / m, g, 1.0 / A.uv, f);
  for (int c = 0; c < 3; c++) A.out[3 * i + c] = f[c];
}

__global__ void rhs_quat_kernel(int n, const double* quat, const double* u_e, double unit_u, double* out) {
  const int i = blockIdx.x * blockDim.x + threadIdx.x;
  if (i >= n) return;
  const double q[4] = {quat[4 * i], quat[4 * i + 1], quat[4 * i + 2], quat[4 * i + 3]};
  double dq[4];
  quat_rate(q, u_e[2 * i], u_e[2 * i + 1], unit_u, dq);
  for (int c = 0; c < 4; c++) out[4 * i + c] = dq[c];
}

__global__ void point_kernel(int kind, int n, const double* in, const double* aux, int aux_rows, double* out) {
  extern __shared__ double lds[];
  const int naux = (kind == 5 || kind == 10) ? 3 * aux_rows + 2 * (aux_rows - 1)
                   : (kind == 6 || kind == 9) ? 2 * aux_rows + (aux_rows - 1)
                   : (kind == 15) ? kAtmDoubles + 3 * aux_rows + 2 * (aux_rows - 1) : (kind == 0 ? kAtmDoubles : 0);
  for (int i = threadIdx.x; i < naux; i += blockDim.x) lds[i] = aux[i];
  __syncthreads();
  const int i = blockIdx.x * blockDim.x + threadIdx.x;
  if (i >= n) return;
  switch (kind) {
    case 0: {
      const double h = geopotential_altitude(in[i]);
      const Air a = atmosphere(h, lds);
      out[5 * i] = h; out[5 * i + 1] = a.T; out[5 * i + 2] = a.P; out[5 * i + 3] = a.rho; out[5 * i + 4] = a.a;
    } break;
    case 1: {
      double lat, sl, cl, p, ip;
      geodetic_lat_p(in[3 * i], in[3 * i + 1], in[3 * i + 2], lat, p, ip);
      geodetic_sincos_p(in[3 * i], in[3 * i + 1], in[3 * i + 2], sl, cl, p, ip);
      const double lon = atan2(in[3 * i + 1], in[3 * i]);
      out[3 * i] = lat * 180.0 / kPi; out[3 * i + 1] = lon * 180.0 / kPi;
      out[3 * i + 2] = geodetic_alt_from(p, sl, cl);
    } break;
    case 2: {
      const double r[3] = {in[3 * i], in[3 * i + 1], in[3 * i + 2]};
      double g[3];
      gravity_eci(r, aux[0], g);
      out[3 * i] = g[0]; out[3 * i + 1] = g[1]; out[3 * i + 2] = g[2];
    } break;
    case 3: {
      const double* a = in + 6 * i;
      const double r[3] = {a[0], a[1], a[2]};
      double sl, cl, p, ip, w[3];
      geodetic_sincos_p(r[0], r[1], r[2], sl, cl, p, ip);
      const EarthAngle ea = earth_angle(a[3]);
      double chp, irt;
      fsqrt_rsqrt(0.5 * (1.0 + cl), chp, irt);
      wind_eci(r, ea, (0.5 * sl) * irt, chp, ip, a[4], a[5], w);
      out[3 * i] = w[0]; out[3 * i + 1] = w[1]; out[3 * i + 2] = w[2];
    } break;
    case 4: {
      const double* a = in + 7 * i;
      double s, c;
      sincos(kOmega * a[6], &s, &c);
      const double d0 = a[0] - (0.0 * a[5] - kOmega * a[4]);
      const double d1 = a[1] - (kOmega * a[3] - 0.0 * a[5]);
      const double d2 = a[2] - (0.0 * a[4] - 0.0 * a[3]);
      out[3 * i] = d0 * c + d1 * s; out[3 * i + 1] = -d0 * s + d1 * c; out[3 * i + 2] = d2;
    } break;
    case 5: {
      double wn, we;
      wind_ned2(in[i], lds, lds + 3 * aux_rows, aux_rows, wn, we);
      out[3 * i] = wn; out[3 * i + 1] = we; out[3 * i + 2] = 0.0;
    } break;
    case 6: out[i] = interp_tab(in[i], lds, lds + 2 * aux_rows, aux_rows, 2, 1); break;
    case 7: {
      const double a = in[2 * i], b = in[2 * i + 1];
      out[4 * i] = fsqrt(a); out[4 * i + 1] = sqrt(a); out[4 * i + 2] = fdiv(a, b); out[4 * i + 3] = a / b;
    } break;
    case 8: {
      double s1, c1, s2, c2;
      fsincos(in[2 * i], &s1, &c1);
      sincos(in[2 * i], &s2, &c2);
      out[6 * i] = s1; out[6 * i + 1] = c1; out[6 * i + 2] = s2; out[6 * i + 3] = c2;
      out[6 * i + 4] = flog_ratio(in[2 * i + 1]); out[6 * i + 5] = log(in[2 * i + 1]);
    } break;
    case 9: {
      Bracket br = no_bracket();
      for (int k = 0; k < 8; k++) out[8 * i + k] = interp_tab_cached(in[8 * i + k], lds, lds + 2 * aux_rows, aux_rows, 2, 1, br);
    } break;
    case 10: {
      Bracket2 br = no_bracket2();
      for (int k = 0; k < 8; k++) {
        double wn, we;
        wind_ned2_cached(in[8 * i + k], lds, lds + 3 * aux_rows, aux_rows, wn, we, br);
        out[16 * i + 2 * k] = wn; out[16 * i + 2 * k + 1] = we;
      }
    } break;
    case 11: {
      double o[4];
      quatmult(in + 8 * i, in + 8 * i + 4, o);
      for (int c = 0; c < 4; c++) out[4 * i + c] = o[c];
    } break;
    case 12: {
      double o[3];
      quatrot(in + 7 * i, in + 7 * i + 4, o);
      for (int c = 0; c < 3; c++) out[3 * i + c] = o[c];
    } break;
    case 13: {
      const double* q = in + 4 * i;
      out[7 * i] = q[0]; out[7 * i + 1] = -q[1]; out[7 * i + 2] = -q[2]; out[7 * i + 3] = -q[3];
      double d[3];
      thrust_dir(q, d);
      for (int c = 0; c < 3; c++) out[7 * i + 4 + c] = d[c];
    } break;
    case 14: out[2 * i] = fexp(in[i]); out[2 * i + 1] = exp(in[i]); break;
    case 15: {
      Tables tb;
      tb.atm = lds; tb.wind = lds + kAtmDoubles; tb.winds = tb.wind + 3 * aux_rows; tb.ca = nullptr; tb.cas = nullptr;
      tb.Kw = aux_rows; tb.Kc = 0;
      const double* a = in + 5 * i;
      const double r[3] = {a[0], a[1], a[2]};
      const int kk = min(max((int)a[3], 0), 2);
      PosCentre pc;
      PosCentreTail pt;
      PosPart pp = pos_part<true, PosCentreSink, false>(r, tb, 0.0, nullptr, PosCentreSink{&pc}, &pt);
      pos_centre_tail(pt, pp.rho, pp.P, tb, pc, pp.wn, pp.we);
      PosPart pq;
      const bool ok = pos_delta(r, kk, a[4], pp, pc, tb, pq);
      double* o = out + 18 * i;
      o[0] = pp.rho; o[1] = pp.P; o[2] = pp.inv_a; o[3] = pp.wn; o[4] = pp.we; o[5] = pp.shp; o[6] = pp.chp; o[7] = pp.inv_p;
      o[8] = pq.rho; o[9] = pq.P; o[10] = pq.inv_a; o[11] = pq.wn; o[12] = pq.we; o[13] = pq.shp; o[14] = pq.chp; o[15] = pq.inv_p;
      o[16] = ok ? 1.0 : 0.0; o[17] = pc.margin;
    } break;
    default: break;
  }
}

struct AeroPos {
  double rho;
  double wn, we;
  double shp, chp, inv_p;
};

GEL_DEV AeroPos aero_pos_part(const double r[3], const Tables& tb) {
  AeroPos o;
  double lat, p, sl, cl;
  geodetic_lat_p(r[0], r[1], r[2], lat, p, o.inv_p);
  fsincos(lat, &sl, &cl);
  const double h = geopotential_altitude(geodetic_alt_from(p, sl, cl));
  wind_ned2(h, tb.wind, tb.winds, tb.Kw, o.wn, o.we);
  double irt;
  fsqrt_rsqrt(0.5 * (1.0 + cl), o.chp, irt);
  o.shp = (0.5 * sl) * irt;
  o.rho = atmosphere(h, tb.atm).rho;
  return o;
}

GEL_DEV double aero_vair(const double r[3], const double v[3], const EarthAngle& ea, const double w[3], double a[3]) {
  const double d0 = v[0] + kOmega * r[1], d1 = v[1] - kOmega * r[0];
  const double e0 = d0 * ea.c + d1 * ea.s, e1 = -d0 * ea.s + d1 * ea.c;
  a[0] = (e0 * ea.c - e1 * ea.s) - w[0]; a[1] = (e0 * ea.s + e1 * ea.c) - w[1]; a[2] = v[2] - w[2];
  return sqrt(a[0] * a[0] + a[1] * a[1] + a[2] * a[2]);
}

GEL_DEV double aero_alpha(const double a[3], double nv, const double q[4]) {
  double dir[3];
  thrust_dir(q, dir);
  const double nd = sqrt(dir[0] * dir[0] + dir[1] * dir[1] + dir[2] * dir[2]);
  const double c_alpha = (a[0] / nv) * (dir[0] / nd) + (a[1] / nv) * (dir[1] / nd) + (a[2] / nv) * (dir[2] / nd);
  return (c_alpha > 1.0) ? 0.0 : ((nv < 1e-6) ? 0.0 : acos(c_alpha));
}

struct AeroOut {
  double* con[3];
  double* jac[3];
  int32_t nrows[3];
  int64_t ld;
  int32_t sm;
};

#ifndef GEL_AERO_UNROLL
#define GEL_AERO_UNROLL 1
#endif
constexpr int kAeroWaves = 4;
enum { AP_ILIM = 0, AP_AC = 3, AP_QC, AP_CC, AP_IS, AP_IND, AP_W = 8, AP_A0 = 11, AP_DIR = 14, AP_RHO = 17, AP_NV2 = 18, AP_INTS = 19,
       kAeroParkSlots = 25 };
static_assert(wave_lds_doubles(false, false, false) <= kWaveLds && wave_lds_doubles(false, true, false, true) <= kWaveLds &&
              wave_lds_doubles(false, true, true) <= kWaveLds && wave_lds_doubles(false, true, false, false, true) <= kWaveLds &&
              wave_lds_doubles(false, true, false, false, false) <= kWaveLds, "kWaveLds is the largest region");
static size_t eval_lds_bytes(size_t park_off, int wave_doubles) { return sizeof(double) * (park_off + (size_t)wave_doubles * (kBlock / 64)); }
size_t eval_lds_bytes_max(int Kw, int Kc) { return eval_lds_bytes(padded_table_doubles(Kw, Kc), kWaveLds); }
size_t aero_lds_bytes(int Kw, int Kc) { return sizeof(double) * (padded_table_doubles(Kw, Kc) + (size_t)kAeroWaves * kAeroParkSlots * 64); }
typedef __attribute__((address_space(3))) int lds_int;
typedef __attribute__((address_space(3))) double lds_f64;
template <bool ROLES, bool WIDE = false, bool SM = false>
__device__ __forceinline__ void aero_body(const ProblemDev P, int nnodes, const AeroNodeDev* __restrict__ nodes, int tiles, int B,
                                          const double* __restrict__ x, const AeroOut O, const unsigned vblk) {
  extern __shared__ double lds[];
  const Tables tb = stage_tables(P, lds);
  const int lane = (int)(threadIdx.x & 63);
  const int sw = ROLES ? (int)(threadIdx.x >> 6) : -1;
  const long long wid = ROLES ? (long long)vblk : (long long)vblk * kAeroWaves + __builtin_amdgcn_readfirstlane((int)(threadIdx.x >> 6));
  const bool flat = !ROLES && !WIDE && tiles == 0;
  int b, ni_raw;
  bool live;
  if (WIDE) {
    const long long total = (long long)B * nnodes, f = wid * 64 + lane;
    if (wid * 64 >= total) return;
    live = f < total;
    const long long fc = live ? f : total - 1;
    b = (int)(fc / nnodes);
    ni_raw = live ? (int)(fc - (long long)b * nnodes) : nnodes;
  } else if (flat) {
    const long long total = (long long)B * nnodes, f0 = wid * 64;
    if (f0 >= total) return;
    const int b0 = (int)(f0 / nnodes), r0 = (int)(f0 - (long long)b0 * nnodes);
    const bool wrap = r0 + lane >= nnodes;
    live = f0 + lane < total;
    b = live ? (wrap ? b0 + 1 : b0) : b0;
    ni_raw = live ? (wrap ? r0 + lane - nnodes : r0 + lane) : nnodes;
  } else {
    if (wid >= (long long)B * tiles) return;
    b = (int)(wid / tiles);
    ni_raw = (int)(wid - (long long)b * tiles) * 64 + lane;
    live = ni_raw < nnodes;
  }
  const int ni = live ? ni_raw : nnodes - 1;
  const AeroNodeDev Nd = nodes[ni];
  const PhaseDev& ph = P.phases[Nd.phase];
  const double* xb = x + (size_t)b * P.nvars;
  const int M = P.M, N = P.N, xi = ph.xa + Nd.k;
  const double dx = P.dx;
  double re[3];
#pragma unroll
  for (int c = 0; c < 3; c++) re[c] = xb[M + 3 * xi + c];
  const bool want_jac = O.jac[0] || O.jac[1] || O.jac[2];
  const bool need_alpha = __builtin_amdgcn_ballot_w64(live && ((O.con[0] && Nd.row[0] >= 0) || (O.con[2] && Nd.row[2] >= 0))) != 0;
  lds_f64* park = (lds_f64*)lds + ((table_doubles(P.Kw, P.Kc) + 1) & ~1) + (size_t)(threadIdx.x >> 6) * (kAeroParkSlots * 64) + lane;
  lds_int* ipark = (lds_int*)(park - lane + AP_INTS * 64) + lane;
#define AP_AIDX(kind, w) ((kind) == 0 ? ((w) == 3 ? 3 : ((w) == 4 ? 4 : 5)) : ((kind) == 1 ? ((w) == 3 ? 6 : 7) : ((w) == 3 ? 8 : ((w) == 4 ? 9 : 10))))
#define AP_GET(i) (park[(i) * 64])
#define AP_SET(i, v) (park[(i) * 64] = (v))
  PosCentre pc;
  PosPart pp;
  EarthAngle ea{1.0, 0.0, 1.0, 0.0};
  bool have_ea = false;
#define GEL_AERO_NEED_EA(ip_, wn_, we_)                                                                                \
  do {                                                                                                                 \
    if (!have_ea && __builtin_amdgcn_ballot_w64(wind_needs_angle(ip_, wn_, we_)) != 0) {                                \
      const int kn_ = nodes[ni].k, phn_ = nodes[ni].phase;                                                             \
      const double to_ = xb[11 * M + 2 * N + phn_], tf_ = xb[11 * M + 2 * N + phn_ + 1];                               \
      const double tau_ = (kn_ == 0) ? 0.0 : P.tau[P.phases[phn_].toff + kn_ - 1];                                     \
         \
      ea = earth_angle(((kn_ == 0) ? to_ : (tau_ * (tf_ - to_) / 2 + (tf_ + to_) / 2)) * P.ut);                         \
      have_ea = true;                                                                                                  \
    }                                                                                                                  \
  } while (0)
  double chk = 0.0;
  {
    double r[3], v[3], q[4], w[3], a0[3], dir[3];
#pragma unroll
    for (int c = 0; c < 3; c++) { r[c] = re[c] * P.up; v[c] = xb[4 * M + 3 * xi + c] * P.uv; }
#pragma unroll
    for (int c = 0; c < 4; c++) q[c] = xb[7 * M + 4 * xi + c];
    PosCentreTail pt;
    pp = pos_part<true, PosCentreSink, false>(r, tb, 0.0, nullptr, PosCentreSink{&pc}, &pt);
    pos_centre_tail(pt, pp.rho, pp.P, tb, pc, pp.wn, pp.we);
    GEL_AERO_NEED_EA(pp.inv_p, pp.wn, pp.we);
    wind_eci_or_calm(r, ea, pp.shp, pp.chp, pp.inv_p, pp.wn, pp.we, w);
    const double nv2 = aero_vair2(r, v, w, a0);
    thrust_dir(q, dir);
    const double ind = frsqrt(fmax(dir[0] * dir[0] + dir[1] * dir[1] + dir[2] * dir[2], 1.0e-300));
    const double cc = need_alpha ? aero_cos(a0, nv2, dir, ind) : 0.0;
    const double alpha_c = need_alpha ? aero_acos(cc, nv2) : 0.0;
    const double qdyn_c = 0.5 * pp.rho * nv2;
    double sc, isc;
    fsqrt_rsqrt(fmax((1.0 - cc) * (1.0 + cc), 1.0e-300), sc, isc);
    const bool centre_ok = (cc <= 1.0) && (nv2 >= 1.0e-12) && (sc > 1.0e-6);
#pragma unroll
    for (int kind = 0; kind < 3; kind++) {
      const double il = frcp(Nd.limit[kind]);
      AP_SET(AP_ILIM + kind, il * P.inv_dx);
      const int row = Nd.row[kind];
      {
        const bool has = live && O.jac[kind] && row >= 0;
        const unsigned vb = flat ? (unsigned)b * (unsigned)(O.ld ? (int)O.ld * 8 : O.nrows[kind] * (8 + ((kind == 1) ? 0 : 4)) * 8) : 0u;
        ipark[kind * 64] = 8 * Nd.nk[kind];
        ipark[AP_AIDX(kind, 3) * 64] = has ? (int)(vb + 8u * (unsigned)((SM ? 1 : 3) * Nd.row0[kind] + Nd.ko)) : -1;
        ipark[AP_AIDX(kind, 2) * 64] = has ? (int)(vb + 8u * (unsigned)((SM ? 1 : 2) * Nd.row0[kind] + Nd.ko)) : -1;
        if (kind != 1) ipark[AP_AIDX(kind, 4) * 64] = has ? (int)(vb + 8u * (unsigned)((SM ? 1 : 4) * Nd.row0[kind] + Nd.ko)) : -1;
      }
      if (!live || row < 0 || !O.con[kind] || (ROLES && sw != 0)) continue;
      const double cv = 1.0 - ((kind == 0) ? alpha_c : (kind == 1) ? qdyn_c : qdyn_c * alpha_c) * il;
      if (ROLES) __builtin_nontemporal_store(cv, O.con[kind] + (size_t)b * O.nrows[kind] + row);
      else if (WIDE) O.con[kind][(size_t)b * O.ld + row] = cv;
      else O.con[kind][(size_t)b * (O.ld ? (size_t)O.ld : (size_t)O.nrows[kind]) + row] = cv;
      chk += cv;
    }
    ipark[11 * 64] = centre_ok ? 1 : 0;
    AP_SET(AP_AC, alpha_c); AP_SET(AP_QC, qdyn_c); AP_SET(AP_CC, cc); AP_SET(AP_IS, isc); AP_SET(AP_IND, ind);
#pragma unroll
    for (int c = 0; c < 3; c++) { AP_SET(AP_W + c, w[c]); AP_SET(AP_A0 + c, a0[c]); AP_SET(AP_DIR + c, dir[c]); }
    AP_SET(AP_RHO, pp.rho); AP_SET(AP_NV2, nv2);
  }
#define GEL_AERO_EMIT(boff, width, col, a, nv2, d, ind, rho, skip_q, zero, skip_lane)                                      \
  do {                                                                                                            \
    double t_ = 0.0, dq_ = 0.0, qp_ = 0.0;                                                                        \
    const double ac_ = AP_GET(AP_AC);                                                                             \
    if (!(zero)) {                                                                                                \
      const double qc_ = AP_GET(AP_QC);                                                                           \
      qp_ = 0.5 * (rho) * (nv2);                                                                                  \
      dq_ = qp_ - qc_;                                                                                            \
      if (need_alpha) {                                                                                           \
        const double cp_ = aero_cos(a, nv2, d, ind);                                                              \
        const bool okd_ = aero_dalpha(cp_, nv2, AP_GET(AP_CC), AP_GET(AP_IS), ipark[11 * 64] != 0, t_);           \
        if (__builtin_amdgcn_ballot_w64(!okd_) != 0) {                                                            \
          const double t2_ = aero_acos(cp_, nv2) - ac_;                                                           \
          t_ = okd_ ? t_ : t2_;                                                                                   \
        }                                                                                                         \
      }                                                                                                           \
    }                                                                                                             \
    _Pragma("unroll") for (int kind = 0; kind < 3; kind++) {                                                      \
      if ((skip_q) && kind == 1) continue;                         \
      const int a8_ = ipark[AP_AIDX(kind, width) * 64];                                                           \
      if (a8_ == -1 || (skip_lane)) continue;                                                                     \
      if (SM && (zero)) continue;                           \
      const int nq = (kind == 1) ? 0 : 4;                                                                         \
      const int bo = ((boff) < 0) ? (6 + nq) : (boff);                                                            \
      const double df_ = (kind == 0) ? t_ : ((kind == 1) ? dq_ : qp_ * t_ + dq_ * ac_);                           \
      const double gv = (zero) ? 0.0 : -(df_ * AP_GET(AP_ILIM + kind));                                           \
      gel_au2 gd_;                                                                                                \
      __builtin_memcpy(&gd_, &gv, 8);                                                                             \
      if (WIDE) O.jac[kind][(size_t)b * O.ld + (size_t)bo * O.nrows[kind] + ((a8_ + (col) * ipark[kind * 64]) >> 3)] = gv;                     \
      else if (SM) __builtin_amdgcn_raw_buffer_store_b64(gd_, jrs[kind], a8_ + ((((boff) < 0) ? 11 : ((boff) == 0 ? 1 : ((boff) == 3 ? 4 : 7))) + (col)) * ipark[kind * 64], 0, 0); \
      else __builtin_amdgcn_raw_buffer_store_b64(gd_, jrs[kind], ((col) == 0) ? a8_ : a8_ + (col) * ipark[kind * 64], 8 * bo * O.nrows[kind], ROLES ? 2 : 0);  \
      chk += gv;                                                                                                  \
    }                                                                                                             \
  } while (0)
  typedef unsigned gel_au2 __attribute__((ext_vector_type(2)));
  __amdgpu_buffer_rsrc_t jrs[3];
#pragma unroll
  for (int kind = 0; kind < 3; kind++)
    jrs[kind] = __builtin_amdgcn_make_buffer_rsrc((O.jac[kind] && !WIDE) ? (void*)(O.jac[kind] + (flat ? (size_t)0 : (size_t)__builtin_amdgcn_readfirstlane(b) * (O.ld ? (size_t)O.ld : (size_t)O.nrows[kind] * (8 + ((kind == 1) ? 0 : 4))))) : (void*)nullptr,
                                                  0, -1, 0x00020000);
  if (want_jac) {
#pragma unroll 1
    for (int c = (ROLES && sw != 0) ? 2 : 0; c < 2; c++) {
      if (P.fd_recompute) {
        const int kn = nodes[ni].k, phn = nodes[ni].phase;
        const double to2 = xb[11 * M + 2 * N + phn], tf2 = xb[11 * M + 2 * N + phn + 1];
        const double tau2 = (kn == 0) ? 0.0 : P.tau[P.phases[phn].toff + kn - 1];
        const double to_p = (c == 0) ? to2 + dx : to2, tf_p = (c == 1) ? tf2 + dx : tf2;
        const double tp = ((kn == 0) ? to_p : (tau2 * (tf_p - to_p) / 2 + (tf_p + to_p) / 2)) * P.ut;
        const EarthAngle eq = earth_angle(tp);
        const double r[3] = {fresh_product(re[0], P.up), fresh_product(re[1], P.up), fresh_product(re[2], P.up)};
        const double vq[3] = {xb[4 * M + 3 * xi] * P.uv, xb[4 * M + 3 * xi + 1] * P.uv, xb[4 * M + 3 * xi + 2] * P.uv};
        double wq[3], aq[3];
        wind_eci_chain(r, eq, pp.shp, pp.chp, pp.inv_p, pp.wn, pp.we, wq);
        const double nvq = aero_vair2(r, vq, wq, aq);
        const double dq[3] = {AP_GET(AP_DIR), AP_GET(AP_DIR + 1), AP_GET(AP_DIR + 2)};
        GEL_AERO_EMIT(-1, 2, c, aq, nvq, dq, AP_GET(AP_IND), pp.rho, false, false, false);
      } else {
        const double none[3] = {0.0, 0.0, 0.0};
        GEL_AERO_EMIT(-1, 2, c, none, 0.0, none, 0.0, 0.0, false, true, false);
      }
    }
#define GEL_AERO_POS_TAIL(c, rp, pq, skip_)                                                          \
  do {                                                                                               \
    double wq_[3], a_[3];                                                                            \
    GEL_AERO_NEED_EA((pq).inv_p, (pq).wn, (pq).we);                                                  \
    wind_eci_or_calm(rp, ea, (pq).shp, (pq).chp, (pq).inv_p, (pq).wn, (pq).we, wq_);                 \
    const double vq_[3] = {xb[4 * M + 3 * xi] * P.uv, xb[4 * M + 3 * xi + 1] * P.uv, xb[4 * M + 3 * xi + 2] * P.uv}; \
    const double nv2_ = aero_vair2(rp, vq_, wq_, a_);                                                \
    const double dd_[3] = {AP_GET(AP_DIR), AP_GET(AP_DIR + 1), AP_GET(AP_DIR + 2)};                  \
    GEL_AERO_EMIT(0, 3, c, a_, nv2_, dd_, AP_GET(AP_IND), (pq).rho, false, false, skip_);                  \
  } while (0)
    const unsigned mine = ROLES ? ((sw == 0) ? 0u : (1u << (sw - 1))) : 7u;
    unsigned todo = P.fd_recompute ? mine : 0u;
    unsigned bad = P.fd_recompute ? 7u : 0u;
    if (!P.fd_recompute) {
#if GEL_AERO_UNROLL
#pragma unroll
#else
#pragma unroll 1
#endif
      for (int c = 0; c < 3; c++) {
        if (!((mine >> c) & 1u)) continue;
        asm volatile("" ::: "memory");
        const double r[3] = {fresh_product(re[0], P.up), fresh_product(re[1], P.up), fresh_product(re[2], P.up)};
        double rp[3];
#pragma unroll
        for (int d = 0; d < 3; d++) rp[d] = (d == c) ? (re[d] + dx) * P.up : r[d];
        const double dlt = (c == 0) ? rp[0] - r[0] : ((c == 1) ? rp[1] - r[1] : rp[2] - r[2]);
        PosPart pq;
        const bool okp = pos_delta(r, c, dlt, pp, pc, tb, pq);
        if (__builtin_amdgcn_ballot_w64(!okp) != 0) { todo |= 1u << c; if (!okp) bad |= 1u << c; }
        GEL_AERO_POS_TAIL(c, rp, pq, !okp);
      }
    }
    if (todo) {
      asm volatile("" ::: "memory");
#pragma unroll 1
      for (int c = 0; c < 3; c++) {
        if (!((todo >> c) & 1u)) continue;
        double rp[3];
#pragma unroll
        for (int d = 0; d < 3; d++) rp[d] = ((d == c) ? xb[M + 3 * xi + d] + dx : xb[M + 3 * xi + d]) * P.up;
        const PosPart pf = pos_part<false, NoSink, false>(rp, tb, 0.0);
        GEL_AERO_POS_TAIL(c, rp, pf, !((bad >> c) & 1u));
      }
    }
#undef GEL_AERO_POS_TAIL
    asm volatile("" ::: "memory");
#if GEL_AERO_UNROLL
#pragma unroll
#else
#pragma unroll 1
#endif
    for (int c = (ROLES && sw != 0) ? 3 : 0; c < 3; c++) {
      double vp[3], a[3];
      const double r[3] = {xb[M + 3 * xi] * P.up, xb[M + 3 * xi + 1] * P.up, xb[M + 3 * xi + 2] * P.up};
#pragma unroll
      for (int d = 0; d < 3; d++) vp[d] = ((d == c) ? xb[4 * M + 3 * xi + d] + dx : xb[4 * M + 3 * xi + d]) * P.uv;
      const double wc[3] = {AP_GET(AP_W), AP_GET(AP_W + 1), AP_GET(AP_W + 2)};
      const double dc[3] = {AP_GET(AP_DIR), AP_GET(AP_DIR + 1), AP_GET(AP_DIR + 2)};
      const double nv2 = aero_vair2(r, vp, wc, a);
      GEL_AERO_EMIT(3, 3, c, a, nv2, dc, AP_GET(AP_IND), AP_GET(AP_RHO), false, false, false);
    }
    if (need_alpha && !(ROLES && sw != 0)) {
#if GEL_AERO_UNROLL
#pragma unroll
#else
#pragma unroll 1
#endif
      for (int c = 0; c < 4; c++) {
        double qp[4], dp[3];
#pragma unroll
        for (int d = 0; d < 4; d++) qp[d] = (d == c) ? xb[7 * M + 4 * xi + d] + dx : xb[7 * M + 4 * xi + d];
        thrust_dir(qp, dp);
        const double indp = frsqrt(fmax(dp[0] * dp[0] + dp[1] * dp[1] + dp[2] * dp[2], 1.0e-300));
        const double ac[3] = {AP_GET(AP_A0), AP_GET(AP_A0 + 1), AP_GET(AP_A0 + 2)};
        GEL_AERO_EMIT(6, 4, c, ac, AP_GET(AP_NV2), dp, indp, AP_GET(AP_RHO), true, false, false);
      }
    }
  }
#undef GEL_AERO_EMIT
#undef GEL_AERO_NEED_EA
#undef AP_AIDX
#undef AP_GET
#undef AP_SET
  if (!(fabs(chk) <= 1.79769313486231570815e308)) *(volatile int32_t*)P.flag = 1;
}

#ifndef GEL_AERO_MIN_WAVES
#define GEL_AERO_MIN_WAVES 3
#endif
#ifndef GEL_AERO_XCD_RANGES
#define GEL_AERO_XCD_RANGES 1
#endif
__device__ __forceinline__ unsigned aero_xcd_block(unsigned p, unsigned n) {
  const unsigned n8 = n >> 3;
  return (GEL_AERO_XCD_RANGES && p < 8u * n8) ? (p & 7u) * n8 + (p >> 3) : p;
}
__global__ __launch_bounds__(64 * kAeroWaves, GEL_AERO_MIN_WAVES) void aero_kernel(ProblemDev P, int nnodes, const AeroNodeDev* __restrict__ nodes,
                                                                int tiles, int B, const double* __restrict__ x, AeroOut O) {
  aero_body<false>(P, nnodes, nodes, tiles, B, x, O, aero_xcd_block(blockIdx.x, gridDim.x));
}
__global__ __launch_bounds__(64 * kAeroWaves, GEL_AERO_MIN_WAVES) void aero_sm_kernel(ProblemDev P, int nnodes, const AeroNodeDev* __restrict__ nodes,
                                                                   int tiles, int B, const double* __restrict__ x, AeroOut O) {
  aero_body<false, false, true>(P, nnodes, nodes, tiles, B, x, O, aero_xcd_block(blockIdx.x, gridDim.x));
}
__global__ __launch_bounds__(64 * kAeroWaves, 2) void aero_wide_kernel(ProblemDev P, int nnodes, const AeroNodeDev* __restrict__ nodes,
                                                                int B, const double* __restrict__ x, AeroOut O) {
  aero_body<false, true>(P, nnodes, nodes, 0, B, x, O, blockIdx.x);
}

hipError_t launch_aero_wide(const ProblemDev& P, int nnodes, const AeroNodeDev* nodes, int B, const double* d_x,
                            const AeroLaunchOut& out, long long ld, hipStream_t s) {
  if (B <= 0 || nnodes <= 0) return hipSuccess;
  AeroOut O;
  for (int k = 0; k < 3; k++) { O.con[k] = out.con[k]; O.jac[k] = out.jac[k]; O.nrows[k] = out.nrows[k]; }
  O.ld = ld; O.sm = 0;
  const size_t lds = aero_lds_bytes(P.Kw, P.Kc);
  const long long waves = ((long long)B * nnodes + 63) / 64;
  hipLaunchKernelGGL(aero_wide_kernel, dim3((unsigned)((waves + kAeroWaves - 1) / kAeroWaves)), dim3(64 * kAeroWaves), lds, s, P, nnodes, nodes, B, d_x, O);
  return hipGetLastError();
}

AeroForm aero_form(int nnodes, int B, const int32_t* nrows, long long ld) {
  AeroForm f{false, 1, B, 0};
  if (B <= 0 || nnodes <= 0) return f;
  const bool flat_shape = B > 1 && nnodes >= 64 && (nnodes & 63) != 0;
  if (ld > 0 && flat_shape) {
    const long long run = ((1LL << 32) - (1LL << 25)) / (ld * 8);
    if (run >= 1 && run < B) { f.runs = (B + run - 1) / run; f.run_len = run; }
  }
  for (int k = 0; k < 3; k++) f.max_bytes = std::max(f.max_bytes, f.run_len * (ld ? ld : (long long)nrows[k] * (8 + ((k == 1) ? 0 : 4))) * 8);
  f.flat = f.run_len > 1 && nnodes >= 64 && (nnodes & 63) != 0 && f.max_bytes < (1LL << 32) - (1LL << 24);
  return f;
}

hipError_t launch_aero(const ProblemDev& P, int nnodes, const AeroNodeDev* nodes, int B, const double* d_x,
                       const AeroLaunchOut& out, hipStream_t s, long long ld, bool spec_major) {
  if (B <= 0 || nnodes <= 0) return hipSuccess;
  const AeroForm form = aero_form(nnodes, B, out.nrows, ld);
  if (form.runs > 1) {
    for (long long b0 = 0; b0 < B; b0 += form.run_len) {
      AeroLaunchOut o = out;
      for (int k = 0; k < 3; k++) { if (o.con[k]) o.con[k] += b0 * ld; if (o.jac[k]) o.jac[k] += b0 * ld; }
      const hipError_t e = launch_aero(P, nnodes, nodes, (int)std::min<long long>(form.run_len, B - b0), d_x + b0 * P.nvars, o, s, ld, spec_major);
      if (e != hipSuccess) return e;
    }
    return hipSuccess;
  }
  AeroOut O;
  for (int k = 0; k < 3; k++) { O.con[k] = out.con[k]; O.jac[k] = out.jac[k]; O.nrows[k] = out.nrows[k]; }
  O.ld = ld; O.sm = (ld > 0 && spec_major) ? 1 : 0;
  int tiles = (nnodes + 63) / 64;
  const size_t lds = aero_lds_bytes(P.Kw, P.Kc);
  long long waves = (long long)B * tiles;
  if (form.flat) {
    waves = ((long long)B * nnodes + 63) / 64;
    tiles = 0;
  }
  const unsigned grid = (unsigned)((waves + kAeroWaves - 1) / kAeroWaves);
  if (O.sm) hipLaunchKernelGGL(aero_sm_kernel, dim3(grid), dim3(64 * kAeroWaves), lds, s, P, nnodes, nodes, tiles, B, d_x, O);
  else hipLaunchKernelGGL(aero_kernel, dim3(grid), dim3(64 * kAeroWaves), lds, s, P, nnodes, nodes, tiles, B, d_x, O);
  return hipGetLastError();
}

GEL_DEV double node_fn(int fn, const double r[3], const double v[3], double t, const double* p) {
  if (fn >= 9) {
    double sn, cs;
    sincos(kOmega * t, &sn, &cs);
    const double pe[3] = {r[0] * cs + r[1] * sn, -r[0] * sn + r[1] * cs, r[2]};
    if (fn <= 11) {
      double lat, lon, alt;
      geodetic_full(pe[0], pe[1], pe[2], lat, lon, alt);
      return (fn == 9) ? lat * (180.0 / kPi) : (fn == 10) ? lon * (180.0 / kPi) : alt;
    }
    if (fn == 15) {
      double lat, lon, alt;
      geodetic_full(pe[0], pe[1], pe[2], lat, lon, alt);
      return distance_vincenty(p[2], p[3], lat * (180.0 / kPi), lon * (180.0 / kPi));
    }
    if (fn <= 13) {
      const double d0 = v[0] + kOmega * r[1], d1 = v[1] - kOmega * r[0];
      const double ve[3] = {d0 * cs + d1 * sn, -d0 * sn + d1 * cs, v[2]};
      double la, lo;
      iip_faa(pe, ve, la, lo);
      return (fn == 12) ? la : lo;
    }
    const double d[3] = {pe[0] - p[2], pe[1] - p[3], pe[2] - p[4]};
    const double dn = sqrt(d[0] * d[0] + d[1] * d[1] + d[2] * d[2]);
    return (d[0] / dn) * p[5] + (d[1] / dn) * p[6] + (d[2] / dn) * p[7];
  }
  const double rn = sqrt(r[0] * r[0] + r[1] * r[1] + r[2] * r[2]);
  const double vn = sqrt(v[0] * v[0] + v[1] * v[1] + v[2] * v[2]);
  if (fn == 0) return 0.5 * vn * vn - kMu / rn;
  if (fn == 7) return rn;
  if (fn == 8) return vn;
  const double c[3] = {r[1] * v[2] - r[2] * v[1], r[2] * v[0] - r[0] * v[2], r[0] * v[1] - r[1] * v[0]};
  const double c2 = c[0] * c[0] + c[1] * c[1] + c[2] * c[2];
  if (fn == 1) return sqrt(c2);
  if (fn == 2) return acos(c[2] / sqrt(c2));
  const double f[3] = {v[1] * c[2] - v[2] * c[1] - kMu * (r[0] / rn), v[2] * c[0] - v[0] * c[2] - kMu * (r[1] / rn),
                       v[0] * c[1] - v[1] * c[0] - kMu * (r[2] / rn)};
  const double e = sqrt(f[0] * f[0] + f[1] * f[1] + f[2] * f[2]) / kMu;
  if (fn == 4) return e;
  const double a = (c2 / kMu) / (1.0 - e * e);
  if (fn == 3) return a;
  return (fn == 5) ? a * (1.0 - e) : a * (1.0 + e);
}

__device__ __forceinline__ void rows_body(const ProblemDev P, int nlin, const LinRowDev* __restrict__ lin, int nfn,
                                          const FnRowDev* __restrict__ fr, int B, int lin_blocks, const double* __restrict__ x,
                                          double* __restrict__ con, double* __restrict__ jfn, const unsigned vblk) {
  const int R = nlin + nfn;
  double chk = 0.0;
  if ((int)vblk < lin_blocks) {
    const long long t = (long long)vblk * blockDim.x + threadIdx.x;
    if (t >= (long long)B * nlin) return;
    const int b = (int)(t / nlin), r = (int)(t - (long long)b * nlin);
    const LinRowDev L = lin[r];
    const double* xb = x + (size_t)b * P.nvars;
    double s = L.coef0 * xb[L.idx0];
    if (L.idx1 >= 0) s += L.coef1 * xb[L.idx1];
    chk = con[(size_t)b * R + r] = s + L.c0;
  } else {
    const long long t = (long long)(vblk - lin_blocks) * blockDim.x + threadIdx.x;
    const long long grp = t >> 3;
    const int sw = (int)(t & 7);
    const bool live = grp < (long long)B * nfn;
    const long long g2 = live ? grp : 0;
    const int b = (int)(g2 / nfn), row = (int)(g2 - (long long)b * nfn);
    const FnRowDev F = fr[row];
    const double* xb = x + (size_t)b * P.nvars;
    double r[3], v[3];
#pragma unroll
    for (int c = 0; c < 3; c++) {
      const double pe = xb[P.M + 3 * F.node + c], ve = xb[4 * P.M + 3 * F.node + c];
      r[c] = ((sw == 1 + c) ? pe + P.dx : pe) * P.up;
      v[c] = ((sw == 4 + c) ? ve + P.dx : ve) * P.uv;
    }
    double tk = 0.0;
    if (F.tcol >= 0) {
      const double te = xb[11 * P.M + 2 * P.N + F.tcol];
      tk = ((sw == 7) ? te + P.dx : te) * P.ut;
    }
    const double f = node_fn(F.fn, r, v, tk, F.p);
    const int vm = F.mode & 3;
    double g = (vm == 0) ? f / F.p[0] - F.p[1] : (f - F.p[1]) / F.p[0];
    if (F.mode & 8) g = -g;
    const int lane0 = (int)(threadIdx.x & 63 & ~7);
    const double gc = __shfl(g, lane0, 64), fc = __shfl(f, lane0, 64);
    if (!live) return;
    if (sw == 0) chk = con[(size_t)b * R + nlin + row] = g;
    else if (jfn) {
      double d;
      if (F.mode & 4) { d = ((f - fc) / P.dx) / F.p[0]; if (F.mode & 8) d = -d; }
      else d = (g - gc) / P.dx;
      chk = jfn[((size_t)b * nfn + row) * 7 + (sw - 1)] = d;
    }
  }
  if (!(fabs(chk) <= 1.79769313486231570815e308)) *(volatile int32_t*)P.flag = 1;
}

__global__ void rows_kernel(ProblemDev P, int nlin, const LinRowDev* __restrict__ lin, int nfn,
                            const FnRowDev* __restrict__ fr, int B, int lin_blocks, const double* __restrict__ x,
                            double* __restrict__ con, double* __restrict__ jfn) {
  rows_body(P, nlin, lin, nfn, fr, B, lin_blocks, x, con, jfn, blockIdx.x);
}

struct CallbackArgs {
  int32_t nb_eval, nb_aero;
  int32_t nnodes, tiles;
  const AeroNodeDev* nodes;
  AeroOut O;
  int32_t nlin, nfn, lin_blocks;
  const LinRowDev* lin;
  const FnRowDev* fr;
  double* con;
  double* jfn;
};
static_assert(64 * kAeroWaves == 256, "callback_kernel's workgroup is the aero workgroup (four roles of one tile)");
template <bool JAC, bool MFMA>
__global__ __launch_bounds__(256) void callback_kernel(ProblemDev P, const double* __restrict__ x, double* __restrict__ res,
                                                       double* __restrict__ jvar, CallbackArgs A) {
  const unsigned b = blockIdx.x;
  if (b < (unsigned)A.nb_eval) eval_body<JAC, MFMA, true, false, 17>(P, 1, x, res, jvar, b);
  else if (b < (unsigned)(A.nb_eval + A.nb_aero)) aero_body<true>(P, A.nnodes, A.nodes, A.tiles, 1, x, A.O, b - (unsigned)A.nb_eval);
  else rows_body(P, A.nlin, A.lin, A.nfn, A.fr, 1, A.lin_blocks, x, A.con, A.jfn, b - (unsigned)(A.nb_eval + A.nb_aero));
  signal_done(P);
}

hipError_t launch_callback(const ProblemDev& P0, bool want_jac, const double* d_x, double* d_res, double* d_jvar,
                           int nnodes, const AeroNodeDev* nodes, const AeroLaunchOut* aero,
                           int nlin, const LinRowDev* lin, int nfn, const FnRowDev* fr, double* d_con, double* d_jfn, hipStream_t s) {
  ProblemDev P = P0;
  P.unit0 = 4 * P0.chunk0;
  P.nunits = 4 * P0.nchunks;
  CallbackArgs A{};
  A.nb_eval = (P.nunits + 3) / 4;
  if (aero && nnodes > 0) {
    for (int k = 0; k < 3; k++) { A.O.con[k] = aero->con[k]; A.O.jac[k] = aero->jac[k]; A.O.nrows[k] = aero->nrows[k]; }
    A.O.ld = 0; A.O.sm = 0;
    A.nnodes = nnodes; A.nodes = nodes; A.tiles = (nnodes + 63) / 64; A.nb_aero = A.tiles;
  }
  int rows_blocks = 0;
  if (d_con && nlin + nfn > 0) {
    A.nlin = nlin; A.nfn = nfn; A.lin = lin; A.fr = fr; A.con = d_con; A.jfn = d_jfn;
    A.lin_blocks = (nlin + 255) / 256;
    rows_blocks = A.lin_blocks + (nfn * 8 + 255) / 256;
  }
// ... 197 lines not shown
```

gelato_amd/csrc/gel_kernels_exact.hip:

```cpp
#include <hip/hip_runtime.h>

#include "gel_tables.h"
#include "gel_eval_kernel.h"
#include "gel_exact.h"

namespace gel {

constexpr int kExactBlock = 256;

__global__ __launch_bounds__(kExactBlock) void exact_jac_kernel(ProblemDev P, int B, const double* __restrict__ x,
                                                                double* __restrict__ jvar) {
  extern __shared__ double lds[];
  const Tables tb = stage_tables(P, lds, true);
  const long long t = (long long)blockIdx.x * blockDim.x + threadIdx.x;
  if (t >= (long long)B * P.N) return;
  const int N = P.N, M = P.M;
  const int b = (int)(t / N), g = (int)(t - (long long)b * N);
  const int sec = P.node_phase[g];
  const PhaseDev ph = P.phases[sec];
  const int n = ph.n, j = g - ph.ua;
  const int xj = ph.xa + 1 + j;
  const double* xb = x + (size_t)b * P.nvars;
  const double me = xb[xj];
  const double re[3] = {xb[M + 3 * xj], xb[M + 3 * xj + 1], xb[M + 3 * xj + 2]};
  const double ve[3] = {xb[4 * M + 3 * xj], xb[4 * M + 3 * xj + 1], xb[4 * M + 3 * xj + 2]};
  const double q[4] = {xb[7 * M + 4 * xj], xb[7 * M + 4 * xj + 1], xb[7 * M + 4 * xj + 2], xb[7 * M + 4 * xj + 3]};
  const double u0 = ph.hold ? 0.0 : xb[11 * M + 2 * g], u1 = ph.hold ? 0.0 : xb[11 * M + 2 * g + 1];
  const double to = xb[11 * M + 2 * N + sec], tf = xb[11 * M + 2 * N + sec + 1];
  const double tau = P.tau[ph.toff + j];
  const double djj = P.Dt[ph.doff + (size_t)(j + 1) * n + j];
  const double ut = P.ut, hT = P.hT;
  const double S = (tf - to) * ut / 2.0;
  const double inv_uv = P.inv_uv;

  const int j0 = j & ~63, w = min(64, n - j0);
  double* const out = jvar + (size_t)b * P.V + ph.voff + (size_t)j0 * ph.K + (j - j0);
  bool bad = false;
#define XPUT(slot, val)                                        \
  do {                                                         \
    const double v_ = (val);                                   \
    out[(size_t)(slot) * w] = v_;                              \
    bad = bad || !(fabs(v_) <= 1.79769313486231570815e308);    \
  } while (0)

#pragma unroll
  for (int c = 0; c < 3; c++) XPUT(kSlotPT + c, ve[c] * P.kpt);
  if (j == 0) {
    const double sc = -(P.kpt * (tf - to));
    jvar[(size_t)b * P.V + ph.voff + (size_t)ph.K * n] = sc;
    bad = bad || !(fabs(sc) <= 1.79769313486231570815e308);
  }

  if (!ph.hold) {
    const double hS = (tf - to) * ut / 2.0;
    const double d2r = 0.017453292519943295769;
    XPUT(ph.s_qq + 0, 0.5 * ((u0 * P.uu) * d2r) * hS);
    XPUT(ph.s_qq + 1, 0.5 * ((u1 * P.uu) * d2r) * hS);
    const double kq = 0.5 * (P.uu * d2r) * hS;
    XPUT(ph.s_qq + 2, -(kq * q[0]));
    XPUT(ph.s_qq + 3, kq * q[1]);
    XPUT(ph.s_qq + 4, kq * q[2]);
    XPUT(ph.s_qq + 5, kq * q[3]);
    double fq[4];
    quat_rate(q, u0, u1, P.uu, fq);
#pragma unroll
    for (int c = 0; c < 4; c++) XPUT(ph.s_qq + 6 + c, fq[c] * hT);
  }

  const double tn = tau * (tf - to) / 2 + (tf + to) / 2;
  const double inv_m = frcp(me * P.um);
  const double r[3] = {re[0] * P.up, re[1] * P.up, re[2] * P.up};
  double dir[3];
  thrust_dir(q, dir);
  double T, fc[3], tm[3];
  double dfr[3][3];
  if (ph.air) {
    PosCentre pc;
    PosCentreTail tail;
    const PosPart pp = pos_part<true, PosCentreSink>(r, tb, P.barC20, nullptr, PosCentreSink{&pc}, &tail);
    const EarthAngle ea = earth_angle(tn);
    double wv[3], F[3];
    wind_eci_or_calm(r, ea, pp.shp, pp.chp, pp.inv_p, pp.wn, pp.we, wv);
    const double v[3] = {ve[0] * P.uv, ve[1] * P.uv, ve[2] * P.uv};
    aero_force(r, v, pp.rho, pp.inv_a, wv, ph.area, tb, F);
    T = ph.thrust - ph.nozzle * pp.P;
    {
      const double Td[3] = {T * dir[0], T * dir[1], T * dir[2]};
      accel_parts(Td, F, inv_m, pp.g, inv_uv, tm, fc);
    }
    const double a[3] = {(v[0] + kOmega * r[1]) - wv[0], (v[1] - kOmega * r[0]) - wv[1], v[2] - wv[2]};
    const double s2 = a[0] * a[0] + a[1] * a[1] + a[2] * a[2];
    const double s = fsqrt(fmax(s2, 1.0e-200));
    const double mach = s * pp.inv_a;
    const double ca = interp_tab(mach, tb.ca, tb.cas, tb.Kc, 2, 1);
    const double cas = interp_tab_slope(mach, tb.ca, tb.cas, tb.Kc, 2);
    const double kk = (s2 > 0.0) ? 0.5 * pp.rho * ph.area * ca * s : 0.0;
    if (ph.air_fd) {
#pragma unroll
      for (int k = 0; k < 3; k++) {
        const double da[3] = {(k == 0) ? 1.0 : 0.0, (k == 1) ? 1.0 : 0.0, (k == 2) ? 1.0 : 0.0};
        double dF[3];
        aero_force_tangent(a, s2, s, pp.rho, pp.inv_a, ph.area, ca, cas, kk, da, 0.0, 0.0, dF);
#pragma unroll
        for (int c = 0; c < 3; c++) XPUT(ph.s_vv + 3 * k + c, ((c == k) ? djj : 0.0) - S * ((dF[c] * P.uv) * inv_m * inv_uv));
      }
    }
    double dsl[3], dcl[3], dalt[3], dh[3];
    geodetic_tangent(r, pp.inv_p, pc, dsl, dcl, dalt);
#pragma unroll
    for (int k = 0; k < 3; k++) dh[k] = (pc.G * pc.G) * dalt[k];
    const double Tk = pp.P / (pp.rho * tb.atm[33 + tail.k]);
    const AirTangent at = atmosphere_tangent(tail.h, Tk, pp.P, pp.rho, pp.inv_a, tb.atm);
    const bool in = tail.piece >= 0;
    const double s0 = in ? tb.winds[2 * tail.piece] : 0.0, s1 = in ? tb.winds[2 * tail.piece + 1] : 0.0;
    const double clon = (pp.inv_p > 0.0) ? r[0] * pp.inv_p : ea.c, slon = (pp.inv_p > 0.0) ? r[1] * pp.inv_p : ea.s;
    double dw[3][3];
    wind_eci_tangent(r, pp.inv_p, clon, slon, pc.sl, pc.cl, pp.wn, pp.we, s0, s1, dh, dsl, dcl, dw);
    double dg[3][3];
    gravity_tangent(r, P.barC20, dg);
#pragma unroll
    for (int k = 0; k < 3; k++) {
      const double da[3] = {((k == 1) ? kOmega : 0.0) - dw[k][0], ((k == 0) ? -kOmega : 0.0) - dw[k][1], -dw[k][2]};
      double dF[3];
      aero_force_tangent(a, s2, s, pp.rho, pp.inv_a, ph.area, ca, cas, kk, da, at.drho * dh[k], at.dinv_a * dh[k], dF);
      const double dT = -ph.nozzle * (at.dP * dh[k]);
#pragma unroll
      for (int c = 0; c < 3; c++) dfr[k][c] = ((dT * dir[c] + dF[c]) * inv_m + dg[k][c]) * inv_uv;
    }
  } else {
    T = ph.thrust;
    double gc[3];
    gravity_eci(r, P.barC20, gc);
#pragma unroll
    for (int c = 0; c < 3; c++) { tm[c] = (T * dir[c]) * inv_m; fc[c] = (tm[c] + gc[c]) * inv_uv; }
    double dg[3][3];
    gravity_tangent(r, P.barC20, dg);
#pragma unroll
    for (int k = 0; k < 3; k++)
#pragma unroll
      for (int c = 0; c < 3; c++) dfr[k][c] = dg[k][c] * inv_uv;
  }
#pragma unroll
  for (int k = 0; k < 3; k++)
#pragma unroll
    for (int c = 0; c < 3; c++) XPUT(kSlotVP + 3 * k + c, -S * (P.up * dfr[k][c]));
  {
    const double km = (P.um * inv_m) * (inv_uv * S);
#pragma unroll
    for (int c = 0; c < 3; c++) XPUT(kSlotVM + c, tm[c] * km);
  }
  {
    const double kqe = (T * inv_m) * (inv_uv * S);
#pragma unroll
    for (int k = 0; k < 4; k++) {
      const double a_ = (k < 2) ? -kqe : kqe;
      const double b_ = -2.0 * kqe;
      XPUT(ph.s_vq + 3 * k + 0, (2.0 * q[k]) * a_);
      XPUT(ph.s_vq + 3 * k + 1, q[3 - k] * b_);
      XPUT(ph.s_vq + 3 * k + 2, ((k & 1) ? q[k ^ 2] : -q[k ^ 2]) * b_);
    }
  }
#pragma unroll
  for (int c = 0; c < 3; c++) XPUT(ph.s_vt + c, fc[c] * hT);
#undef XPUT
  if (bad) *(volatile int32_t*)P.flag = 1;
}

hipError_t launch_eval_exact(const ProblemDev& P, int B, const double* d_x, double* d_jvar, hipStream_t s) {
  if (B <= 0) return hipSuccess;
  if (P.fd_recompute || !d_jvar) return hipErrorInvalidValue;
  const long long threads = (long long)B * P.N;
  const unsigned grid = (unsigned)((threads + kExactBlock - 1) / kExactBlock);
  const size_t lds = table_lds_bytes(P.Kw, P.Kc);
  hipLaunchKernelGGL(exact_jac_kernel, dim3(grid), dim3(kExactBlock), lds, s, P, B, d_x, d_jvar);
  return hipGetLastError();
}

}
```

gelato_amd/csrc/gel_kernels_exact_aero.hip:

```cpp
#include <hip/hip_runtime.h>

#include "gel_tables.h"
#include "gel_launch.h"
#include "gel_exact.h"

namespace gel {

constexpr int kExactAeroBlock = 256;

__global__ __launch_bounds__(kExactAeroBlock) void exact_aero_kernel(ProblemDev P, int nnodes, const AeroNodeDev* __restrict__ nodes,
                                                                      int B, const double* __restrict__ x, AeroLaunchOut O,
                                                                      long long ld, int sm) {
  extern __shared__ double lds[];
  const Tables tb = stage_tables(P, lds, true);
  const long long t = (long long)blockIdx.x * blockDim.x + threadIdx.x;
  if (t >= (long long)B * nnodes) return;
  const int b = (int)(t / nnodes), ni = (int)(t - (long long)b * nnodes);
  const AeroNodeDev Nd = nodes[ni];
  const PhaseDev ph = P.phases[Nd.phase];
  const int M = P.M, N = P.N, xi = ph.xa + Nd.k;
  const double* xb = x + (size_t)b * P.nvars;
  const double r[3] = {xb[M + 3 * xi] * P.up, xb[M + 3 * xi + 1] * P.up, xb[M + 3 * xi + 2] * P.up};
  const double v[3] = {xb[4 * M + 3 * xi] * P.uv, xb[4 * M + 3 * xi + 1] * P.uv, xb[4 * M + 3 * xi + 2] * P.uv};
  const double q[4] = {xb[7 * M + 4 * xi], xb[7 * M + 4 * xi + 1], xb[7 * M + 4 * xi + 2], xb[7 * M + 4 * xi + 3]};

  PosCentre pc;
  PosCentreTail tail;
  PosPart pp = pos_part<true, PosCentreSink, false>(r, tb, 0.0, nullptr, PosCentreSink{&pc}, &tail);
  pos_centre_tail(tail, pp.rho, pp.P, tb, pc, pp.wn, pp.we);
  const double to = xb[11 * M + 2 * N + Nd.phase], tf = xb[11 * M + 2 * N + Nd.phase + 1];
  const double tau = (Nd.k == 0) ? 0.0 : P.tau[ph.toff + Nd.k - 1];
  const EarthAngle ea = earth_angle(((Nd.k == 0) ? to : (tau * (tf - to) / 2 + (tf + to) / 2)) * P.ut);
  double w[3], a[3], dir[3];
  wind_eci_or_calm(r, ea, pp.shp, pp.chp, pp.inv_p, pp.wn, pp.we, w);
  const double nv2 = aero_vair2(r, v, w, a);
  thrust_dir(q, dir);
  const double ind = frsqrt(fmax(dir[0] * dir[0] + dir[1] * dir[1] + dir[2] * dir[2], 1.0e-300));
  const double cc = aero_cos(a, nv2, dir, ind);
  const double alpha = aero_acos(cc, nv2);
  const double qdyn = 0.5 * pp.rho * nv2;

  double dsl[3], dcl[3], dalt[3], dh[3];
  geodetic_tangent(r, pp.inv_p, pc, dsl, dcl, dalt);
#pragma unroll
  for (int k = 0; k < 3; k++) dh[k] = (pc.G * pc.G) * dalt[k];
  const double Tk = pp.P / (pp.rho * tb.atm[33 + tail.k]);
  const AirTangent at = atmosphere_tangent(tail.h, Tk, pp.P, pp.rho, pp.inv_a, tb.atm);
  const bool in = tail.piece >= 0;
  const double s0 = in ? tb.winds[2 * tail.piece] : 0.0, s1 = in ? tb.winds[2 * tail.piece + 1] : 0.0;
  const double clon = (pp.inv_p > 0.0) ? r[0] * pp.inv_p : ea.c, slon = (pp.inv_p > 0.0) ? r[1] * pp.inv_p : ea.s;
  double dw[3][3];
  wind_eci_tangent(r, pp.inv_p, clon, slon, pc.sl, pc.cl, pp.wn, pp.we, s0, s1, dh, dsl, dcl, dw);
  const double is = frsqrt(fmax(nv2, 1.0e-300));
  const double u[3] = {a[0] * is, a[1] * is, a[2] * is}, e[3] = {dir[0] * ind, dir[1] * ind, dir[2] * ind};
  double ep[3], upp[3];
#pragma unroll
  for (int c = 0; c < 3; c++) { ep[c] = e[c] - cc * u[c]; upp[c] = u[c] - cc * e[c]; }
  const double ne2 = ep[0] * ep[0] + ep[1] * ep[1] + ep[2] * ep[2], nu2 = upp[0] * upp[0] + upp[1] * upp[1] + upp[2] * upp[2];
  const bool has_da = (cc <= 1.0) && (nv2 >= 1.0e-12) && ne2 > 0.0 && nu2 > 0.0;
  const double kep = has_da ? frsqrt(ne2) * is : 0.0;
  const double kup = has_da ? frsqrt(nu2) * ind : 0.0;
#pragma unroll
  for (int c = 0; c < 3; c++) { ep[c] *= kep; upp[c] *= kup; }

  double* base[3];
  int32_t rowst[3];
#pragma unroll
  for (int kind = 0; kind < 3; kind++) {
    const int nq = (kind == 1) ? 0 : 4;
    const bool has = O.jac[kind] && Nd.row[kind] >= 0;
    const long long vs = ld ? ld : (long long)O.nrows[kind] * (8 + nq);
    base[kind] = has ? O.jac[kind] + (size_t)b * vs + (sm ? (size_t)Nd.row0[kind] : 0) + Nd.ko : nullptr;
    rowst[kind] = Nd.nk[kind];
  }
  const double il[3] = {frcp(Nd.limit[0]), frcp(Nd.limit[1]), frcp(Nd.limit[2])};
  bool bad = false;
#define EXPUT(bo, wd, col, dal, dq_)                                                                                   \
  do {                                                                                                                 \
    const double da_ = (dal), dqv_ = (dq_);                                                                            \
    _Pragma("unroll") for (int kind = 0; kind < 3; kind++) {                                                           \
      if (!base[kind] || ((bo) == 6 && kind == 1) || (sm && (bo) < 0)) continue;                                      \
      const double df_ = (kind == 0) ? da_ : ((kind == 1) ? dqv_ : qdyn * da_ + alpha * dqv_);                        \
      const double gv_ = ((bo) < 0) ? 0.0 : -(df_ * il[kind]);                                                       \
      const int nq_ = (kind == 1) ? 0 : 4, b_ = ((bo) < 0) ? 6 + nq_ : (bo);                                           \
      const size_t o_ = sm ? (size_t)(((bo) == 0 ? 1 : ((bo) == 3 ? 4 : 7)) + (col)) * rowst[kind]                     \
                           : (size_t)b_ * O.nrows[kind] + (size_t)(wd) * Nd.row0[kind] + (size_t)(col) * rowst[kind];  \
      base[kind][o_] = gv_;                                                                                            \
      bad = bad || !(fabs(gv_) <= 1.79769313486231570815e308);                                                         \
    }                                                                                                                  \
  } while (0)

#pragma unroll
  for (int k = 0; k < 3; k++) {
    const double da[3] = {((k == 1) ? kOmega : 0.0) - dw[k][0], ((k == 0) ? -kOmega : 0.0) - dw[k][1], -dw[k][2]};
    const double ada = a[0] * da[0] + a[1] * da[1] + a[2] * da[2];
    const double dq = pp.rho * ada + 0.5 * (at.drho * dh[k]) * nv2;
    const double dal = -(da[0] * ep[0] + da[1] * ep[1] + da[2] * ep[2]);
    EXPUT(0, 3, k, P.up * dal, P.up * dq);
  }
#pragma unroll
  for (int k = 0; k < 3; k++) EXPUT(3, 3, k, P.uv * -ep[k], P.uv * (pp.rho * a[k]));
#pragma unroll
  for (int k = 0; k < 4; k++) {
    const double dd[3] = {(k < 2) ? 2.0 * q[k] : -2.0 * q[k], 2.0 * q[3 - k], 2.0 * ((k & 1) ? q[k ^ 2] : -q[k ^ 2])};
    EXPUT(6, 4, k, -(dd[0] * upp[0] + dd[1] * upp[1] + dd[2] * upp[2]), 0.0);
  }
  EXPUT(-1, 2, 0, 0.0, 0.0);
  EXPUT(-1, 2, 1, 0.0, 0.0);
#undef EXPUT
  if (bad) *(volatile int32_t*)P.flag = 1;
}

hipError_t launch_aero_exact(const ProblemDev& P, int nnodes, const AeroNodeDev* nodes, int B, const double* d_x,
                             const AeroLaunchOut& out, hipStream_t s, long long ld, bool spec_major) {
  if (B <= 0 || nnodes <= 0) return hipSuccess;
  if (P.fd_recompute) return hipErrorInvalidValue;
  const long long threads = (long long)B * nnodes;
  const unsigned grid = (unsigned)((threads + kExactAeroBlock - 1) / kExactAeroBlock);
  const size_t lds = table_lds_bytes(P.Kw, P.Kc);
  hipLaunchKernelGGL(exact_aero_kernel, dim3(grid), dim3(kExactAeroBlock), lds, s, P, nnodes, nodes, B, d_x, out, ld,
                     (ld > 0 && spec_major) ? 1 : 0);
  return hipGetLastError();
}

}
```

gelato_amd/csrc/gel_rhs_parts.h:

```cpp
#pragma once
#include "gel_physics.h"

#ifndef GEL_CALM_SHORTCUT
#define GEL_CALM_SHORTCUT 1
#endif

namespace gel {

struct PosPart {
  double rho, P, inv_a;
  double wn, we;
  double g[3];
  double shp, chp;
  double inv_p;
};

GEL_DEV void geodetic_sincos(double x, double y, double z, double& sl, double& cl, double& p) {
  p = sqrt(x * x + y * y);
  const double a = z * kRa, b = p * kRb;
  const double ih = 1.0 / sqrt(a * a + b * b);
  const double st = a * ih, ct = b * ih;
  const double zz = z + kEp2 * kRb * (st * st * st);
  const double pp = p - kE2 * kRa * (ct * ct * ct);
  const double ihy = 1.0 / sqrt(zz * zz + pp * pp);
  sl = zz * ihy;
  cl = pp * ihy;
}

struct PosCentre {
  double p, ih, ihy;
  double sl, cl, icl;
  double N;
  double G;
  double s0, s1;
  double margin;
  AirCentre air;
};
enum PosCentreSlot { PCS_P = 0, PCS_IH, PCS_IHY, PCS_SL, PCS_CL, PCS_ICL, PCS_N, PCS_G, PCS_COUNT };
struct PosCentreTail { double h; int k, piece; };
struct NoSink { GEL_DEV void put(int, double) const {} };
struct PosCentreSink {
  PosCentre* pc;
  GEL_DEV void put(int i, double v) const {
    if (i == PCS_P) pc->p = v; else if (i == PCS_IH) pc->ih = v; else if (i == PCS_IHY) pc->ihy = v; else if (i == PCS_SL) pc->sl = v;
    else if (i == PCS_CL) pc->cl = v; else if (i == PCS_ICL) pc->icl = v; else if (i == PCS_N) pc->N = v; else pc->G = v;
  }
};

template <bool CENTRE = false, class Sink = NoSink, bool GRAV = true>
GEL_DEV PosPart pos_part(const double r[3], const Tables& tb, double barC20, Bracket2* wbr = nullptr, Sink sink = Sink(),
                         PosCentreTail* tail = nullptr) {
  PosPart o;
  double p, sl, cl;
  if (CENTRE) {
    double ih, ihy;
    geodetic_sincos_p(r[0], r[1], r[2], sl, cl, p, o.inv_p, &ih, &ihy);
    sink.put(PCS_IH, ih); sink.put(PCS_IHY, ihy); sink.put(PCS_P, p);
  } else geodetic_sincos_p(r[0], r[1], r[2], sl, cl, p, o.inv_p);
  {
    double irt;
    fsqrt_rsqrt(0.5 * (1.0 + cl), o.chp, irt);
    o.shp = (0.5 * sl) * irt;
  }
  const double N = fdiv(kRa, fsqrt(1.0 - kE2 * sl * sl));
  const double q = fdiv(p, cl);
  const double alt = q - N;
  if (CENTRE) {
    sink.put(PCS_SL, sl); sink.put(PCS_CL, cl); sink.put(PCS_N, N);
    sink.put(PCS_ICL, q * o.inv_p);
    sink.put(PCS_G, (alt < 86000.0) ? fdiv(6356766.0, 6356766.0 + alt) : 1.0);
  }
  const double h = geopotential_altitude(alt);
  const Air air = atmosphere(h, tb.atm);
  o.rho = air.rho; o.P = air.P; o.inv_a = air.inv_a;
  if (CENTRE) {
    wind_ned2_centre(h, tb.wind, tb.winds, tb.Kw, o.wn, o.we, tail->piece);
    tail->h = h; tail->k = us76_layer(h);
  } else if (wbr) wind_ned2_cached(h, tb.wind, tb.winds, tb.Kw, o.wn, o.we, *wbr);
  else wind_ned2(h, tb.wind, tb.winds, tb.Kw, o.wn, o.we);
  if (GRAV) gravity_eci(r, barC20, o.g);
  else o.g[0] = o.g[1] = o.g[2] = 0.0;
  return o;
}

GEL_DEV void pos_centre_tail(const PosCentreTail& t, double rho, double P, const Tables& tb, PosCentre& pc, double& wn, double& we) {
  double wm;
  wind_piece(t.h, t.piece, tb.wind, tb.winds, tb.Kw, wn, we, pc.s0, pc.s1, wm);
  const double lo = (t.k == 0) ? -1.0e300 : tb.atm[66 + t.k];
  const double hi = (t.k == 6) ? kGeopot86 : ((t.k < 10) ? tb.atm[67 + min(t.k, 9)] : 1.0e300);
  pc.margin = fmin(wm, fmin(t.h - lo, hi - t.h));
  pc.air.iT = rho * tb.atm[33 + t.k] * frcp(P);
  pc.air.h = t.h; pc.air.k = t.k;
}

GEL_DEV bool pos_delta(const double r[3], int kk, double dlt, const PosPart& c, const PosCentre& pc, const Tables& tb, PosPart& o) {
  const bool along_z = kk == 2;
  const double a = r[2] * kRa, b = pc.p * kRb;
  double u = 0.0, dp = 0.0, dh2, dst, dct, dih, ih1;
  o.inv_p = c.inv_p;
  if (!along_z) {
    const double xs = (kk == 0) ? r[0] : r[1];
    const double dp2 = dlt * __builtin_fma(2.0, xs, dlt);
    u = dp2 * c.inv_p * c.inv_p;
    dp = (0.5 * dp2 * c.inv_p) * (1.0 + u * (-0.25 + 0.125 * u));
    o.inv_p = c.inv_p * (1.0 + u * (-0.5 + 0.375 * u));
    const double db = dp * kRb;
    dh2 = db * __builtin_fma(2.0, b, db);
    const double uh = dh2 * pc.ih * pc.ih;
    dih = pc.ih * (uh * (-0.5 + 0.375 * uh));
    ih1 = pc.ih + dih;
    dst = a * dih;
    dct = db * ih1 + b * dih;
  } else {
    const double da = dlt * kRa;
    dh2 = da * __builtin_fma(2.0, a, da);
    const double uh = dh2 * pc.ih * pc.ih;
    dih = pc.ih * (uh * (-0.5 + 0.375 * uh));
    ih1 = pc.ih + dih;
    dst = da * ih1 + a * dih;
    dct = b * dih;
  }
  const double st = a * pc.ih, ct = b * pc.ih;
  const double dst3 = dst * (3.0 * st * (st + dst) + dst * dst);
  const double dct3 = dct * (3.0 * ct * (ct + dct) + dct * dct);
  const double dzz = along_z ? dlt + (kEp2 * kRb) * dst3 : (kEp2 * kRb) * dst3;
  const double dpp = along_z ? -((kE2 * kRa) * dct3) : dp - (kE2 * kRa) * dct3;
  const double e = (pc.cl * dpp + pc.sl * dzz) * pc.ihy;
  const double dlat = ((dzz * pc.cl - dpp * pc.sl) * pc.ihy) * (1.0 + e * (e - 1.0));
  const double hl2 = 0.5 * dlat * dlat;
  const double dsl = pc.cl * dlat - pc.sl * hl2, dcl = -(pc.sl * dlat + pc.cl * hl2);
  const double hd = 0.5 * dlat, hd2 = 0.5 * hd * hd;
  o.shp = c.shp + (c.chp * hd - c.shp * hd2);
  o.chp = c.chp - (c.shp * hd + c.chp * hd2);
  const double v = dcl * pc.icl;
  const double dq = ((dp - (pc.p * pc.icl) * dcl) * pc.icl) * (1.0 + v * (v - 1.0));
  const double nr = pc.N * (1.0 / kRa);
  const double uw = (-kE2 * dsl * __builtin_fma(2.0, pc.sl, dsl)) * (nr * nr);
  const double dN = pc.N * (uw * (-0.5 + 0.375 * uw));
  const double dalt = dq - dN;
  const double g1 = (pc.air.k <= 6) ? pc.G * (1.0 / 6356766.0) : 0.0;
  const double dh = (pc.G * pc.G) * dalt * (1.0 - dalt * g1);
  Air ca_;
  ca_.P = c.P; ca_.rho = c.rho; ca_.inv_a = c.inv_a; ca_.T = 0.0; ca_.a = 0.0;
  atmosphere_delta(ca_, pc.air, dh, tb.atm, o.P, o.rho, o.inv_a);
  o.wn = __builtin_fma(pc.s0, dh, c.wn);
  o.we = __builtin_fma(pc.s1, dh, c.we);
  return (c.inv_p > 0.0) && (fabs(u) < 1.0e-4) && (fabs(v) < 1.0e-4) && (fmax(fabs(dalt), fabs(dh)) < pc.margin);
}

struct EarthAngle { double c, s, ch, sh; };

struct EarthHalf { double ch, sh; };
GEL_DEV EarthAngle full_angle(const EarthHalf& h) {
  EarthAngle e;
  e.ch = h.ch; e.sh = h.sh;
  e.s = fresh_mul(2.0 * h.sh, h.ch);
  e.c = fresh_mul(h.ch - h.sh, h.ch + h.sh);
  return e;
}
GEL_DEV EarthAngle earth_angle(double t) {
  EarthAngle e;
  fsincos(kOmega * t / 2.0, &e.sh, &e.ch);
  e.s = 2.0 * e.sh * e.ch;
  e.c = (e.ch - e.sh) * (e.ch + e.sh);
  return e;
}

#ifndef GEL_WIND_CHAIN
#define GEL_WIND_CHAIN 0
#endif
GEL_DEV bool wind_needs_angle(double inv_p, double wn, double we) {
  const bool windy = !(wn == 0.0 && we == 0.0);
#if GEL_WIND_CHAIN
  return windy;
#else
  return windy && !(inv_p > 0.0);
#endif
}
GEL_DEV void wind_eci_chain(const double r[3], const EarthAngle& e, double s_hp, double c_hp, double inv_p, double wn,
                            double we, double w[3]) {
  const double px = r[0] * e.c + r[1] * e.s;
  const double py = -r[0] * e.s + r[1] * e.c;
  const double clon = (inv_p > 0.0) ? px * inv_p : 1.0, slon = py * inv_p;
  double th, ith;
  fsqrt_rsqrt(0.5 * (1.0 + fabs(clon)), th, ith);
  const double uh = (0.5 * slon) * ith;
  const double c_hl = (clon >= 0.0) ? th : fabs(uh);
  const double s_hl = (clon >= 0.0) ? uh : copysign(th, slon);
  const double irt2 = 0.70710678118654752440;
  const double b0 = c_hl * (c_hp - s_hp) * irt2, b1 = s_hl * (c_hp + s_hp) * irt2;
  const double b2 = -c_hl * (c_hp + s_hp) * irt2, b3 = s_hl * (c_hp - s_hp) * irt2;
  const double q0 = e.ch * b0 - e.sh * b3;
  const double q1 = -(e.ch * b1 - e.sh * b2);
  const double q2 = -(e.ch * b2 + e.sh * b1);
  const double q3 = -(e.ch * b3 + e.sh * b0);
  const double t0 = -wn * q1 - we * q2;
  const double t1 = wn * q0 + we * q3;
  const double t2 = -wn * q3 + we * q0;
  const double t3 = wn * q2 - we * q1;
  w[0] = q0 * t1 - q1 * t0 - q2 * t3 + q3 * t2;
  w[1] = q0 * t2 + q1 * t3 - q2 * t0 - q3 * t1;
  w[2] = q0 * t3 - q1 * t2 + q2 * t1 - q3 * t0;
}
GEL_DEV void wind_eci(const double r[3], const EarthAngle& e, double s_hp, double c_hp, double inv_p, double wn,
                      double we, double w[3]) {
#if GEL_WIND_CHAIN
  wind_eci_chain(r, e, s_hp, c_hp, inv_p, wn, we, w);
#else
  const bool off_axis = inv_p > 0.0;
  const double clon = off_axis ? r[0] * inv_p : e.c;
  const double slon = off_axis ? r[1] * inv_p : e.s;
  const double sl = fresh_mul(2.0 * s_hp, c_hp);
  const double cl = fresh_mul(c_hp - s_hp, c_hp + s_hp);
  const double nh = -fresh_mul(wn, sl);
  w[0] = __builtin_fma(nh, clon, -fresh_mul(we, slon));
  w[1] = __builtin_fma(nh, slon, fresh_mul(we, clon));
  w[2] = fresh_mul(wn, cl);
#endif
}

GEL_DEV void wind_eci_or_calm(const double r[3], const EarthAngle& e, double s_hp, double c_hp, double inv_p, double wn,
                              double we, double w[3]) {
#if GEL_CALM_SHORTCUT
  if (__builtin_amdgcn_ballot_w64(!(wn == 0.0 && we == 0.0)) == 0) {
    w[0] = 0.0; w[1] = 0.0; w[2] = 0.0;
    return;
  }
#endif
  wind_eci(r, e, s_hp, c_hp, inv_p, wn, we, w);
}
GEL_DEV void wind_eci_chain_or_calm(const double r[3], const EarthAngle& e, double s_hp, double c_hp, double inv_p, double wn,
                                    double we, double w[3]) {
#if GEL_CALM_SHORTCUT
  if (__builtin_amdgcn_ballot_w64(!(wn == 0.0 && we == 0.0)) == 0) {
    w[0] = 0.0; w[1] = 0.0; w[2] = 0.0;
    return;
  }
#endif
  wind_eci_chain(r, e, s_hp, c_hp, inv_p, wn, we, w);
}

GEL_DEV void aero_force(const double r[3], const double v[3], double rho, double inv_a_sound, const double w[3], double area,
                        const Tables& tb, double F[3], Bracket* br = nullptr) {
  const double d0 = v[0] + kOmega * r[1];
  const double d1 = v[1] - kOmega * r[0];
  const double a0 = d0 - w[0];
  const double a1 = d1 - w[1];
  const double a2 = v[2] - w[2];
  const double vn = fsqrt(fmax(a0 * a0 + a1 * a1 + a2 * a2, 1.0e-200));
  const double mach = vn * inv_a_sound;
  const double ca = br ? interp_tab_cached(mach, tb.ca, tb.cas, tb.Kc, 2, 1, *br) : interp_tab(mach, tb.ca, tb.cas, tb.Kc, 2, 1);
  const double k = 0.5 * rho * area * ca * vn;
  F[0] = k * -a0; F[1] = k * -a1; F[2] = k * -a2;
}

GEL_DEV void accel(const double Td[3], const double F[3], double inv_m, const double g[3], double inv_uv,
                   double out[3]) {
#pragma unroll
  for (int c = 0; c < 3; c++) out[c] = ((Td[c] + F[c]) * inv_m + g[c]) * inv_uv;
}
GEL_DEV void accel_parts(const double Td[3], const double F[3], double inv_m, const double g[3], double inv_uv, double tm[3],
                         double out[3]) {
#pragma unroll
  for (int c = 0; c < 3; c++) { tm[c] = (Td[c] + F[c]) * inv_m; out[c] = (tm[c] + g[c]) * inv_uv; }
}
GEL_DEV void accel_noair(const double Td[3], double inv_m, const double g[3], double inv_uv, double out[3]) {
#pragma unroll
  for (int c = 0; c < 3; c++) out[c] = (Td[c] * inv_m + g[c]) * inv_uv;
}

GEL_DEV void thrust_dir(const double q[4], double dir[3]) {
  dir[0] = q[0] * q[0] + q[1] * q[1] - q[2] * q[2] - q[3] * q[3];
  dir[1] = q[0] * q[3] + q[1] * q[2] + q[2] * q[1] + q[3] * q[0];
  dir[2] = -q[0] * q[2] + q[1] * q[3] - q[2] * q[0] + q[3] * q[1];
}

GEL_DEV void quat_rate(const double q[4], double u0, double u1, double unit_u, double dq[4]) {
  const double d2r = 0.017453292519943295769;
  const double oy = (u0 * unit_u) * d2r, oz = (u1 * unit_u) * d2r;
  dq[0] = 0.5 * (-q[2] * oy - q[3] * oz);
  dq[1] = 0.5 * (q[2] * oz - q[3] * oy);
  dq[2] = 0.5 * (q[0] * oy - q[1] * oz);
  dq[3] = 0.5 * (q[0] * oz + q[1] * oy);
}

GEL_DEV double aero_vair2(const double r[3], const double v[3], const double w[3], double a[3]) {
  a[0] = (v[0] + kOmega * r[1]) - w[0]; a[1] = (v[1] - kOmega * r[0]) - w[1]; a[2] = v[2] - w[2];
  return a[0] * a[0] + a[1] * a[1] + a[2] * a[2];
}
GEL_DEV double aero_cos(const double a[3], double nv2, const double d[3], double ind) {
  return ((a[0] * d[0] + a[1] * d[1] + a[2] * d[2]) * frsqrt(fmax(nv2, 1.0e-300))) * ind;
}
GEL_DEV double aero_acos(double c, double nv2) { return (c > 1.0) ? 0.0 : ((nv2 < 1.0e-12) ? 0.0 : acos(c)); }
GEL_DEV bool aero_dalpha(double c_p, double nv2_p, double c_c, double inv_s, bool centre_ok, double& t) {
  const double t0 = (c_c - c_p) * inv_s, k = (0.5 * c_c) * inv_s;
  const double t1 = t0 - (k * t0) * t0;
  t = (t0 - (k * t1) * t1) + (t1 * t1) * (t1 * (1.0 / 6.0));
  return centre_ok && (c_p <= 1.0) && (nv2_p >= 1.0e-12) && (fabs(k * t0) < 1.0e-4);
}


}
```

gelato_amd/csrc/gel_section_rhs.h:

```cpp
#pragma once
#include "gel_tables.h"

namespace gel {

template <bool kDisp = false, bool kEns = false>
GEL_DEV void section_rhs(const ProblemDev& P, const PhaseDev& ph, const Tables& tb, double vp, double sig, double to, double tf,
                         const double xt[11], double u0, double u1, double F[11], double fw = 1.0, Bracket2* wbr = nullptr) {
  F[0] = ph.engine_on ? ph.mf_um : 0.0;
#pragma unroll
  for (int c = 0; c < 3; c++) F[1 + c] = xt[4 + c] * vp;
  const double m = xt[0] * P.um;
  const double r[3] = {xt[1] * P.up, xt[2] * P.up, xt[3] * P.up};
  const double q[4] = {xt[7], xt[8], xt[9], xt[10]};
  double dir[3], f[3];
  thrust_dir(q, dir);
  if (ph.air) {
    const double v3[3] = {xt[4] * P.uv, xt[5] * P.uv, xt[6] * P.uv};
    const PosPart pp = pos_part(r, tb, P.barC20, kEns ? wbr : nullptr);
    const EarthAngle ea = earth_angle(sig * (tf - to) / 2 + (tf + to) / 2);
    double w[3], Fa[3];
    if constexpr (kDisp) {
      const double wn = pp.wn * fw, we = pp.we * fw;
      wind_eci_or_calm(r, ea, pp.shp, pp.chp, pp.inv_p, wn, we, w);
    } else {
      wind_eci_or_calm(r, ea, pp.shp, pp.chp, pp.inv_p, pp.wn, pp.we, w);
    }
    aero_force(r, v3, pp.rho, pp.inv_a, w, ph.area, tb, Fa);
    const double T = ph.thrust - ph.nozzle * pp.P;
    const double Td[3] = {T * dir[0], T * dir[1], T * dir[2]};
    accel(Td, Fa, 1.0 / m, pp.g, P.inv_uv, f);
  } else {
    double g[3];
    gravity_eci(r, P.barC20, g);
    const double Td[3] = {ph.thrust * dir[0], ph.thrust * dir[1], ph.thrust * dir[2]};
    accel_noair(Td, 1.0 / m, g, P.inv_uv, f);
  }
#pragma unroll
  for (int c = 0; c < 3; c++) F[4 + c] = f[c];
  double dq[4] = {0.0, 0.0, 0.0, 0.0};
  if (!ph.hold) quat_rate(q, u0, u1, P.uu, dq);
#pragma unroll
  for (int c = 0; c < 4; c++) F[7 + c] = dq[c];
}

}
```

gelato_amd/csrc/gel_section_rhs_lin.h:

```cpp
#pragma once
#include "gel_exact.h"
#include "gel_section_rhs.h"

namespace gel {

struct AirLinearisation {
  PosPart pp;
  PosCentre pc;
  PosCentreTail tail;
  EarthAngle ea;
  AirTangent at;
  double wn, we;
  double T, Td[3], Fa[3];
  double a[3], s2, s;
  double ca, cas, kk;
  double dh[3], clon, slon, dw3[3][3];
};

GEL_DEV void linearise_air(const ProblemDev& P, const PhaseDev& ph, const Tables& tb, double sig, double to, double tf, const double xt[11],
                           const double r[3], const double dir[3], double inv_m, double fw, AirLinearisation& L, double f[3]) {
  const double v3[3] = {xt[4] * P.uv, xt[5] * P.uv, xt[6] * P.uv};
  L.pp = pos_part<true, PosCentreSink>(r, tb, P.barC20, nullptr, PosCentreSink{&L.pc}, &L.tail);
  const PosPart& pp = L.pp;
  const PosCentre& pc = L.pc;
  L.ea = earth_angle(sig * (tf - to) / 2 + (tf + to) / 2);
  double w[3];
  L.wn = pp.wn * fw;
  L.we = pp.we * fw;
  wind_eci_or_calm(r, L.ea, pp.shp, pp.chp, pp.inv_p, L.wn, L.we, w);
  aero_force(r, v3, pp.rho, pp.inv_a, w, ph.area, tb, L.Fa);
  L.T = ph.thrust - ph.nozzle * pp.P;
#pragma unroll
  for (int c = 0; c < 3; c++) L.Td[c] = L.T * dir[c];
  accel(L.Td, L.Fa, inv_m, pp.g, P.inv_uv, f);
  L.a[0] = (v3[0] + kOmega * r[1]) - w[0];
  L.a[1] = (v3[1] - kOmega * r[0]) - w[1];
  L.a[2] = v3[2] - w[2];
  L.s2 = L.a[0] * L.a[0] + L.a[1] * L.a[1] + L.a[2] * L.a[2];
  L.s = fsqrt(fmax(L.s2, 1.0e-200));
  const double mach = L.s * pp.inv_a;
  L.ca = interp_tab(mach, tb.ca, tb.cas, tb.Kc, 2, 1);
  L.cas = interp_tab_slope(mach, tb.ca, tb.cas, tb.Kc, 2);
  L.kk = (L.s2 > 0.0) ? 0.5 * pp.rho * ph.area * L.ca * L.s : 0.0;
  double dsl[3], dcl[3], dalt[3];
  geodetic_tangent(r, pp.inv_p, pc, dsl, dcl, dalt);
#pragma unroll
  for (int k = 0; k < 3; k++) L.dh[k] = (pc.G * pc.G) * dalt[k];
  const double Tk = pp.P / (pp.rho * tb.atm[33 + L.tail.k]);
  L.at = atmosphere_tangent(L.tail.h, Tk, pp.P, pp.rho, pp.inv_a, tb.atm);
  const bool in = L.tail.piece >= 0;
  const double s0 = in ? tb.winds[2 * L.tail.piece] * fw : 0.0, s1 = in ? tb.winds[2 * L.tail.piece + 1] * fw : 0.0;
  L.clon = (pp.inv_p > 0.0) ? r[0] * pp.inv_p : L.ea.c;
  L.slon = (pp.inv_p > 0.0) ? r[1] * pp.inv_p : L.ea.s;
  wind_eci_tangent(r, pp.inv_p, L.clon, L.slon, pc.sl, pc.cl, L.wn, L.we, s0, s1, L.dh, dsl, dcl, L.dw3);
}

}
```

gelato_amd/dynamics.py:

```python
import ctypes as C

import numpy as np

from ._lib import check, lib

_dp = C.POINTER(C.c_double)


def _f(a):
    return np.ascontiguousarray(a, dtype=np.float64)


def _d(a):
    return a.ctypes.data_as(_dp)


def dynamics_velocity(mass_e, pos_eci_e, vel_eci_e, quat_eci2body, t, param, wind_table, CA_table, units, barC20=0.0):
    mass_e, pos, vel, quat, t = _f(mass_e), _f(pos_eci_e), _f(vel_eci_e), _f(quat_eci2body), _f(t)
    param, wind, ca, units = _f(param), _f(wind_table), _f(CA_table), _f(units)
    n = mass_e.shape[0]
    if pos.shape != (n, 3) or vel.shape != (n, 3) or quat.shape != (n, 4) or t.shape != (n,):
        raise TypeError("dynamics_velocity(): incompatible function arguments (shape mismatch)")
    out = np.zeros((n, 3))
    check(lib().gel_dynamics_velocity(n, _d(mass_e), _d(pos), _d(vel), _d(quat), _d(t), _d(param), _d(wind),
                                      wind.shape[0], _d(ca), ca.shape[0], _d(units), float(barC20), _d(out)))
    return out


def dynamics_velocity_NoAir(mass_e, pos_eci_e, quat_eci2body, param, units, barC20=0.0):
    mass_e, pos, quat, param, units = _f(mass_e), _f(pos_eci_e), _f(quat_eci2body), _f(param), _f(units)
    n = mass_e.shape[0]
    if pos.shape != (n, 3) or quat.shape != (n, 4):
        raise TypeError("dynamics_velocity_NoAir(): incompatible function arguments (shape mismatch)")
    out = np.zeros((n, 3))
    check(lib().gel_dynamics_velocity_NoAir(n, _d(mass_e), _d(pos), _d(quat), _d(param), _d(units), float(barC20),
                                            _d(out)))
    return out


def dynamics_quaternion(quat_eci2body, u_e, unit_u):
    quat, u = _f(quat_eci2body), _f(u_e)
    n = quat.shape[0]
    if quat.shape != (n, 4) or u.shape != (n, 2):
        raise TypeError("dynamics_quaternion(): incompatible function arguments (shape mismatch)")
    out = np.zeros((n, 4))
    check(lib().gel_dynamics_quaternion(n, _d(quat), _d(u), float(unit_u), _d(out)))
    return out


def point_eval(kind, x, aux=None):
    nin = [1, 3, 3, 6, 7, 1, 1, 2, 2, 8, 8, 8, 7, 4, 1, 5][kind]
    nout = [5, 3, 3, 3, 3, 3, 1, 4, 6, 8, 16, 4, 3, 7, 2, 18][kind]
    x = _f(x).reshape(-1, nin)
    n = x.shape[0]
    out = np.zeros((n, nout))
    a = _f(aux) if aux is not None else None
    rows = 0 if a is None else (a.shape[0] if a.ndim == 2 else 0)
    check(lib().gel_point_eval(kind, n, _d(x), _d(a) if a is not None else None, rows, _d(out)))
    return out
```

Baseline: 22.85 million.

## Carry geodetic sin/cos latitude instead of half-angles; repark atmosphere tail terms

PosPart now carries sin/cos of latitude directly rather than the half-angle pair. This drops the sqrt/rsqrt that built the half-angles and the products that rebuilt sl/cl inside wind_eci. In the Jacobian path the freed park slots now hold the atmosphere tail's inverse temperature and margin (or ih in the aero variant), so the later centre reconstruction can skip recomputing part of pos_centre_tail. This adds extra work in the primary pass (a pos_centre_tail or geodetic_p_ih call) and changes rounding in the perturbed-latitude updates. A new point_eval kind exercises the kept-tail path for testing.

After: 23.22 million, median of 6. 1.02x the previous value.

```diff
diff --git a/gelato_amd/csrc/gel_eval_kernel.h b/gelato_amd/csrc/gel_eval_kernel.h
--- a/gelato_amd/csrc/gel_eval_kernel.h
+++ b/gelato_amd/csrc/gel_eval_kernel.h
@@ -60,6 +60,9 @@
 #define GEL_DX_HOLD7 1
 #endif
 
+#ifndef GEL_POS_REPARK
+#define GEL_POS_REPARK 1
+#endif
 #ifndef GEL_STORE_AUX
 #define GEL_STORE_AUX 2
 #endif
@@ -978,7 +981,7 @@
         }
         EarthAngle ea{1.0, 0.0, 1.0, 0.0};
         if (have_eh) ea = full_angle(eh);
-        wind_eci_or_calm(r, ea, pp.shp, pp.chp, pp.inv_p, pp.wn, pp.we, w);
+        wind_eci_or_calm(r, ea, pp.sl, pp.cl, pp.inv_p, pp.wn, pp.we, w);
 #pragma unroll
         for (int c = 0; c < 3; c++) v[c] = PARK_GET(PK_V0 + c) * P.uv;
         aero_force(r, v, pp.rho, pp.inv_a, w, ph.area, tb, F, GEL_CA_BRACKET);
@@ -1013,8 +1016,21 @@
         }
         if (JAC) {
           asm volatile("" ::: "memory");
-          PARK_SET(PK_LV0, pp.shp); PARK_SET(PK_LV1, pp.chp);
           if (!AERO) PARK_SET(PK_LV2, pp.inv_p);
+#if GEL_POS_REPARK
+          if (!SPLIT || part) {
+            if (AERO) {
+              double p_, ip_, ih_;
+              geodetic_p_ih(r[0], r[1], r[2], p_, ip_, ih_);
+              PARK_SET(PK_LV1, ih_);
+            } else {
+              PosCentre pcx;
+              double wn_, we_;
+              pos_centre_tail(pt, pp.rho, pp.P, tb, pcx, wn_, we_);
+              PARK_SET(PK_LV0, pcx.air.iT); PARK_SET(PK_LV1, pcx.margin);
+            }
+          }
+#endif
         }
         if (JAC && lead && !P.fd_recompute) GEL_MASS_CLOSED(tm);
         if (JAC && ph.air_fd && (SPLIT && P.split_vel ? !lead : lead)) {
@@ -1081,7 +1097,7 @@
             geodetic_p_ih(ra[0], ra[1], ra[2], p_, ip_, ih_);
             EarthAngle e2{1.0, 0.0, 1.0, 0.0};
             if (have_aeh) e2 = full_angle(GEL_AEH);
-            wind_eci(ra, e2, PARK_GET(PK_LV0), PARK_GET(PK_LV1), ip_, wn_, we_, wa);
+            wind_eci(ra, e2, PARK_GET(PK_FP0 + PCS_SL), PARK_GET(PK_FP0 + PCS_CL), ip_, wn_, we_, wa);
           } else {
             wa[0] = 0.0; wa[1] = 0.0; wa[2] = 0.0;
           }
@@ -1143,7 +1159,7 @@
     GEL_NEED_EARTH_ANGLE((pq).inv_p, (pq).wn, (pq).we);                                                       \
     EarthAngle ea{1.0, 0.0, 1.0, 0.0};                                                                        \
     if (have_eh) ea = full_angle(eh);                                                                         \
-    wind_eci_or_calm(rp, ea, (pq).shp, (pq).chp, (pq).inv_p, (pq).wn, (pq).we, wq_);                          \
+    wind_eci_or_calm(rp, ea, (pq).sl, (pq).cl, (pq).inv_p, (pq).wn, (pq).we, wq_);                          \
     const double vq_[3] = {PARK_GET(PK_V0) * P.uv, PARK_GET(PK_V1) * P.uv, PARK_GET(PK_V2) * P.uv};           \
     aero_force(rp, vq_, (pq).rho, (pq).inv_a, wq_, ph.area, tb, Fp_, GEL_CA_BRACKET);                         \
     const double Tp_ = ph.thrust - ph.nozzle * (pq).P;                                                        \
@@ -1161,7 +1177,7 @@
     GEL_AERO_NEED_EA((pq).inv_p, (pq).wn, (pq).we);                                                           \
     EarthAngle ea_{1.0, 0.0, 1.0, 0.0};                                                                       \
     if (have_aeh) ea_ = full_angle(GEL_AEH);                                                                  \
-    wind_eci_or_calm(rp, ea_, (pq).shp, (pq).chp, (pq).inv_p, (pq).wn, (pq).we, wq_);                         \
+    wind_eci_or_calm(rp, ea_, (pq).sl, (pq).cl, (pq).inv_p, (pq).wn, (pq).we, wq_);                         \
     const double vq_[3] = {PARK_GET(PK_V0) * P.uv, PARK_GET(PK_V1) * P.uv, PARK_GET(PK_V2) * P.uv};           \
     const double nv2_ = aero_vair2(rp, vq_, wq_, a_);                                                         \
     const double dd_[3] = {PARK_GET(PK_Q3), PARK_GET(PK_DJJ), dir2};                                          \
@@ -1180,13 +1196,18 @@
   pc.N = PARK_GET(PK_FP0 + PCS_N); pc.G = PARK_GET(PK_FP0 + PCS_G);                                                    \
   PosPart pcv;                                                                                                         \
   pcv.rho = cen_rho; pcv.P = cen_P; pcv.inv_a = cen_inv_a;                                                             \
-  pcv.shp = PARK_GET(PK_LV0); pcv.chp = PARK_GET(PK_LV1);                                                              \
-  if (AERO) {                                                                                                          \
+  pcv.sl = pc.sl; pcv.cl = pc.cl;                                                                                      \
+  if (AERO && GEL_POS_REPARK) {       \
+    double ih_;                                                                                                        \
+    geodetic_p_ih(fresh_product(re[0], P.up), fresh_product(re[1], P.up), fresh_product(re[2], P.up), pc.p, pcv.inv_p, ih_); \
+    pc.ih = PARK_GET(PK_LV1);                                                                                          \
+  } else if (AERO) {                                                                                                   \
     geodetic_p_ih(fresh_product(re[0], P.up), fresh_product(re[1], P.up), fresh_product(re[2], P.up), pc.p, pcv.inv_p, pc.ih); \
   } else {                                                                                                             \
     pc.p = PARK_GET(PK_FP0 + PCS_P); pc.ih = PARK_GET(PK_FP0 + PCS_IH); pcv.inv_p = PARK_GET(PK_LV2);                  \
   }                                                                                                                    \
-  pos_centre_tail(pt, cen_rho, cen_P, tb, pc, pcv.wn, pcv.we)
+  if (GEL_POS_REPARK && !AERO) pos_centre_tail_kept(pt, PARK_GET(PK_LV0), PARK_GET(PK_LV1), tb, pc, pcv.wn, pcv.we);   \
+  else pos_centre_tail(pt, cen_rho, cen_P, tb, pc, pcv.wn, pcv.we)
         unsigned todo = 0;
         unsigned long long coo_okm = 0;
         if (P.fd_recompute) {
@@ -1260,7 +1281,7 @@
           const double r[3] = {fresh_product(re[0], P.up), fresh_product(re[1], P.up), fresh_product(re[2], P.up)};
           const PosPart p2 = pos_part(r, tb, P.barC20);
           const double T2 = ph.thrust - ph.nozzle * p2.P;
-          PARK_SET(PK_FP0, p2.shp); PARK_SET(PK_FP1, p2.chp); PARK_SET(PK_FP2, p2.inv_p); PARK_SET(PK_FP3, p2.wn); PARK_SET(PK_FP4, p2.we);
+          PARK_SET(PK_FP0, p2.sl); PARK_SET(PK_FP1, p2.cl); PARK_SET(PK_FP2, p2.inv_p); PARK_SET(PK_FP3, p2.wn); PARK_SET(PK_FP4, p2.we);
           PARK_SET(PK_FP5, p2.rho); PARK_SET(PK_FP6, p2.inv_a);
           PARK_SET(PK_LV0, p2.g[0]); PARK_SET(PK_LV1, p2.g[1]); PARK_SET(PK_LV2, p2.g[2]);
           PARK_SET(PK_Q0, T2 * PARK_GET(PK_Q3)); PARK_SET(PK_Q1, T2 * PARK_GET(PK_DJJ)); PARK_SET(PK_Q2, T2 * dir2);
diff --git a/gelato_amd/csrc/gel_host.hip b/gelato_amd/csrc/gel_host.hip
--- a/gelato_amd/csrc/gel_host.hip
+++ b/gelato_amd/csrc/gel_host.hip
@@ -1362,10 +1362,10 @@
 }
 
 int gel_point_eval(int32_t kind, int32_t n, const double* in, const double* aux, int32_t aux_rows, double* out) {
-  static const int nin[16] = {1, 3, 3, 6, 7, 1, 1, 2, 2, 8, 8, 8, 7, 4, 1, 5}, nout[16] = {5, 3, 3, 3, 3, 3, 1, 4, 6, 8, 16, 4, 3, 7, 2, 18};
-  if (kind < 0 || kind > 15 || n < 0 || !in || !out) return fail(GEL_ERR_ARG, "bad argument");
+  static const int nin[17] = {1, 3, 3, 6, 7, 1, 1, 2, 2, 8, 8, 8, 7, 4, 1, 5, 5}, nout[17] = {5, 3, 3, 3, 3, 3, 1, 4, 6, 8, 16, 4, 3, 7, 2, 18, 54};
+  if (kind < 0 || kind > 16 || n < 0 || !in || !out) return fail(GEL_ERR_ARG, "bad argument");
   if (n == 0) return GEL_OK;
-  const bool tabulated = kind == 5 || kind == 6 || kind == 9 || kind == 10 || kind == 15;
+  const bool tabulated = kind == 5 || kind == 6 || kind == 9 || kind == 10 || kind == 15 || kind == 16;
   int rc = tabulated ? check_launch_lds("gel_point_eval", gel::point_lds_bytes(aux_rows), 5 * (size_t)std::max(aux_rows, 0), 5 * (size_t)std::max(aux_rows, 0), false) : GEL_OK;
   if (rc) return rc;
   rc = need_device();
@@ -1377,9 +1377,9 @@
   if (kind == 0) { gel::fill_atmosphere_table(atm); hax = atm; naux = gel::kAtmTableDoubles; aux_rows = 0; }
   else if (kind == 2) { if (!aux) return fail(GEL_ERR_ARG, "kind 2 needs aux[0] = barC20"); naux = 1; aux_rows = 0; }
   else if (tabulated) {
-    const int w = (kind == 5 || kind == 10 || kind == 15) ? 3 : 2;
-    if (!aux || aux_rows < 2) return fail(GEL_ERR_ARG, "kinds 5, 6, 9, 10 and 15 need a table of at least two rows");
-    if (kind == 15) { gel::fill_atmosphere_table(atm); ext.assign(atm, atm + gel::kAtmTableDoubles); }
+    const int w = (kind == 5 || kind == 10 || kind == 15 || kind == 16) ? 3 : 2;
+    if (!aux || aux_rows < 2) return fail(GEL_ERR_ARG, "kinds 5, 6, 9, 10, 15 and 16 need a table of at least two rows");
+    if (kind == 15 || kind == 16) { gel::fill_atmosphere_table(atm); ext.assign(atm, atm + gel::kAtmTableDoubles); }
     for (int k = 1; k < aux_rows; k++)
       if (!(aux[(size_t)w * k] > aux[(size_t)w * (k - 1)])) return fail(GEL_ERR_ARG, "table abscissae must increase strictly");
     std::vector<double> slopes;
diff --git a/gelato_amd/csrc/gel_kernels.hip b/gelato_amd/csrc/gel_kernels.hip
--- a/gelato_amd/csrc/gel_kernels.hip
+++ b/gelato_amd/csrc/gel_kernels.hip
@@ -114,7 +114,7 @@
   const PosPart pp = pos_part(r, tb, A.barC20);
   const EarthAngle ea = earth_angle(A.t[i]);
   double w[3], F[3], dir[3], f[3];
-  wind_eci(r, ea, pp.shp, pp.chp, pp.inv_p, pp.wn, pp.we, w);
+  wind_eci(r, ea, pp.sl, pp.cl, pp.inv_p, pp.wn, pp.we, w);
   aero_force(r, v, pp.rho, pp.inv_a, w, A.area, tb, F);
   thrust_dir(q, dir);
   const double T = A.thrust - A.nozzle * pp.P;
@@ -150,7 +150,7 @@
   extern __shared__ double lds[];
   const int naux = (kind == 5 || kind == 10) ? 3 * aux_rows + 2 * (aux_rows - 1)
                    : (kind == 6 || kind == 9) ? 2 * aux_rows + (aux_rows - 1)
-                   : (kind == 15) ? kAtmDoubles + 3 * aux_rows + 2 * (aux_rows - 1) : (kind == 0 ? kAtmDoubles : 0);
+                   : (kind == 15 || kind == 16) ? kAtmDoubles + 3 * aux_rows + 2 * (aux_rows - 1) : (kind == 0 ? kAtmDoubles : 0);
   for (int i = threadIdx.x; i < naux; i += blockDim.x) lds[i] = aux[i];
   __syncthreads();
   const int i = blockIdx.x * blockDim.x + threadIdx.x;
@@ -181,9 +181,7 @@
       double sl, cl, p, ip, w[3];
       geodetic_sincos_p(r[0], r[1], r[2], sl, cl, p, ip);
       const EarthAngle ea = earth_angle(a[3]);
-      double chp, irt;
-      fsqrt_rsqrt(0.5 * (1.0 + cl), chp, irt);
-      wind_eci(r, ea, (0.5 * sl) * irt, chp, ip, a[4], a[5], w);
+      wind_eci(r, ea, sl, cl, ip, a[4], a[5], w);
       out[3 * i] = w[0]; out[3 * i + 1] = w[1]; out[3 * i + 2] = w[2];
     } break;
     case 4: {
@@ -254,11 +252,48 @@
       PosPart pp = pos_part<true, PosCentreSink, false>(r, tb, 0.0, nullptr, PosCentreSink{&pc}, &pt);
       pos_centre_tail(pt, pp.rho, pp.P, tb, pc, pp.wn, pp.we);
       PosPart pq;
-      const bool ok = pos_delta(r, kk, a[4], pp, pc, tb, pq);
+      double dlat;
+      const bool ok = pos_delta(r, kk, a[4], pp, pc, tb, pq, &dlat);
+      double shp, chp, shq, chq;
+      half_lat_pair(pp.sl, pp.cl, shp, chp);
+      half_lat_step(shp, chp, dlat, shq, chq);
       double* o = out + 18 * i;
-      o[0] = pp.rho; o[1] = pp.P; o[2] = pp.inv_a; o[3] = pp.wn; o[4] = pp.we; o[5] = pp.shp; o[6] = pp.chp; o[7] = pp.inv_p;
-      o[8] = pq.rho; o[9] = pq.P; o[10] = pq.inv_a; o[11] = pq.wn; o[12] = pq.we; o[13] = pq.shp; o[14] = pq.chp; o[15] = pq.inv_p;
+      o[0] = pp.rho; o[1] = pp.P; o[2] = pp.inv_a; o[3] = pp.wn; o[4] = pp.we; o[5] = shp; o[6] = chp; o[7] = pp.inv_p;
+      o[8] = pq.rho; o[9] = pq.P; o[10] = pq.inv_a; o[11] = pq.wn; o[12] = pq.we; o[13] = shq; o[14] = chq; o[15] = pq.inv_p;
       o[16] = ok ? 1.0 : 0.0; o[17] = pc.margin;
+    } break;
+    case 16: {
+      Tables tb;
+      tb.atm = lds; tb.wind = lds + kAtmDoubles; tb.winds = tb.wind + 3 * aux_rows; tb.ca = nullptr; tb.cas = nullptr;
+      tb.Kw = aux_rows; tb.Kc = 0;
+      const double* a = in + 5 * i;
+      const double r[3] = {a[0], a[1], a[2]};
+      PosCentre pc0;
+      PosCentreTail pt;
+      const PosPart pp = pos_part<true, PosCentreSink, false>(r, tb, 0.0, nullptr, PosCentreSink{&pc0}, &pt);
+      double iT, margin;
+      {
+        PosCentre pcx;
+        double wn_, we_;
+        pos_centre_tail(pt, pp.rho, pp.P, tb, pcx, wn_, we_);
+        iT = pcx.air.iT; margin = pcx.margin;
+      }
+      double shp, chp;
+      half_lat_pair(pp.sl, pp.cl, shp, chp);
+#pragma unroll 1
+      for (int kk = 0; kk < 3; kk++) {
+        PosCentre pc = pc0;
+        PosPart pcv = pp;
+        pos_centre_tail_kept(pt, iT, margin, tb, pc, pcv.wn, pcv.we);
+        PosPart pq;
+        double dlat, shq, chq;
+        const bool ok = pos_delta(r, kk, a[4], pcv, pc, tb, pq, &dlat);
+        half_lat_step(shp, chp, dlat, shq, chq);
+        double* o = out + 54 * i + 18 * kk;
+        o[0] = pcv.rho; o[1] = pcv.P; o[2] = pcv.inv_a; o[3] = pcv.wn; o[4] = pcv.we; o[5] = shp; o[6] = chp; o[7] = pcv.inv_p;
+        o[8] = pq.rho; o[9] = pq.P; o[10] = pq.inv_a; o[11] = pq.wn; o[12] = pq.we; o[13] = shq; o[14] = chq; o[15] = pq.inv_p;
+        o[16] = ok ? 1.0 : 0.0; o[17] = pc.margin;
+      }
     } break;
     default: break;
   }
@@ -267,19 +302,16 @@
 struct AeroPos {
   double rho;
   double wn, we;
-  double shp, chp, inv_p;
+  double sl, cl, inv_p;
 };
 
 GEL_DEV AeroPos aero_pos_part(const double r[3], const Tables& tb) {
   AeroPos o;
-  double lat, p, sl, cl;
+  double lat, p;
   geodetic_lat_p(r[0], r[1], r[2], lat, p, o.inv_p);
-  fsincos(lat, &sl, &cl);
-  const double h = geopotential_altitude(geodetic_alt_from(p, sl, cl));
+  fsincos(lat, &o.sl, &o.cl);
+  const double h = geopotential_altitude(geodetic_alt_from(p, o.sl, o.cl));
   wind_ned2(h, tb.wind, tb.winds, tb.Kw, o.wn, o.we);
-  double irt;
-  fsqrt_rsqrt(0.5 * (1.0 + cl), o.chp, irt);
-  o.shp = (0.5 * sl) * irt;
   o.rho = atmosphere(h, tb.atm).rho;
   return o;
 }
@@ -395,7 +427,7 @@
     pp = pos_part<true, PosCentreSink, false>(r, tb, 0.0, nullptr, PosCentreSink{&pc}, &pt);
     pos_centre_tail(pt, pp.rho, pp.P, tb, pc, pp.wn, pp.we);
     GEL_AERO_NEED_EA(pp.inv_p, pp.wn, pp.we);
-    wind_eci_or_calm(r, ea, pp.shp, pp.chp, pp.inv_p, pp.wn, pp.we, w);
+    wind_eci_or_calm(r, ea, pp.sl, pp.cl, pp.inv_p, pp.wn, pp.we, w);
     const double nv2 = aero_vair2(r, v, w, a0);
     thrust_dir(q, dir);
     const double ind = frsqrt(fmax(dir[0] * dir[0] + dir[1] * dir[1] + dir[2] * dir[2], 1.0e-300));
@@ -484,7 +516,7 @@
         const double r[3] = {fresh_product(re[0], P.up), fresh_product(re[1], P.up), fresh_product(re[2], P.up)};
         const double vq[3] = {xb[4 * M + 3 * xi] * P.uv, xb[4 * M + 3 * xi + 1] * P.uv, xb[4 * M + 3 * xi + 2] * P.uv};
         double wq[3], aq[3];
-        wind_eci_chain(r, eq, pp.shp, pp.chp, pp.inv_p, pp.wn, pp.we, wq);
+        wind_eci_chain(r, eq, pp.sl, pp.cl, pp.inv_p, pp.wn, pp.we, wq);
         const double nvq = aero_vair2(r, vq, wq, aq);
         const double dq[3] = {AP_GET(AP_DIR), AP_GET(AP_DIR + 1), AP_GET(AP_DIR + 2)};
         GEL_AERO_EMIT(-1, 2, c, aq, nvq, dq, AP_GET(AP_IND), pp.rho, false, false, false);
@@ -497,7 +529,7 @@
   do {                                                                                               \
     double wq_[3], a_[3];                                                                            \
     GEL_AERO_NEED_EA((pq).inv_p, (pq).wn, (pq).we);                                                  \
-    wind_eci_or_calm(rp, ea, (pq).shp, (pq).chp, (pq).inv_p, (pq).wn, (pq).we, wq_);                 \
+    wind_eci_or_calm(rp, ea, (pq).sl, (pq).cl, (pq).inv_p, (pq).wn, (pq).we, wq_);                 \
     const double vq_[3] = {xb[4 * M + 3 * xi] * P.uv, xb[4 * M + 3 * xi + 1] * P.uv, xb[4 * M + 3 * xi + 2] * P.uv}; \
     const double nv2_ = aero_vair2(rp, vq_, wq_, a_);                                                \
     const double dd_[3] = {AP_GET(AP_DIR), AP_GET(AP_DIR + 1), AP_GET(AP_DIR + 2)};                  \
diff --git a/gelato_amd/csrc/gel_kernels_exact.hip b/gelato_amd/csrc/gel_kernels_exact.hip
--- a/gelato_amd/csrc/gel_kernels_exact.hip
+++ b/gelato_amd/csrc/gel_kernels_exact.hip
@@ -80,7 +80,7 @@
     const PosPart pp = pos_part<true, PosCentreSink>(r, tb, P.barC20, nullptr, PosCentreSink{&pc}, &tail);
     const EarthAngle ea = earth_angle(tn);
     double wv[3], F[3];
-    wind_eci_or_calm(r, ea, pp.shp, pp.chp, pp.inv_p, pp.wn, pp.we, wv);
+    wind_eci_or_calm(r, ea, pp.sl, pp.cl, pp.inv_p, pp.wn, pp.we, wv);
     const double v[3] = {ve[0] * P.uv, ve[1] * P.uv, ve[2] * P.uv};
     aero_force(r, v, pp.rho, pp.inv_a, wv, ph.area, tb, F);
     T = ph.thrust - ph.nozzle * pp.P;
diff --git a/gelato_amd/csrc/gel_kernels_exact_aero.hip b/gelato_amd/csrc/gel_kernels_exact_aero.hip
--- a/gelato_amd/csrc/gel_kernels_exact_aero.hip
+++ b/gelato_amd/csrc/gel_kernels_exact_aero.hip
@@ -32,7 +32,7 @@
   const double tau = (Nd.k == 0) ? 0.0 : P.tau[ph.toff + Nd.k - 1];
   const EarthAngle ea = earth_angle(((Nd.k == 0) ? to : (tau * (tf - to) / 2 + (tf + to) / 2)) * P.ut);
   double w[3], a[3], dir[3];
-  wind_eci_or_calm(r, ea, pp.shp, pp.chp, pp.inv_p, pp.wn, pp.we, w);
+  wind_eci_or_calm(r, ea, pp.sl, pp.cl, pp.inv_p, pp.wn, pp.we, w);
   const double nv2 = aero_vair2(r, v, w, a);
   thrust_dir(q, dir);
   const double ind = frsqrt(fmax(dir[0] * dir[0] + dir[1] * dir[1] + dir[2] * dir[2], 1.0e-300));
diff --git a/gelato_amd/csrc/gel_rhs_parts.h b/gelato_amd/csrc/gel_rhs_parts.h
--- a/gelato_amd/csrc/gel_rhs_parts.h
+++ b/gelato_amd/csrc/gel_rhs_parts.h
@@ -11,7 +11,7 @@
   double rho, P, inv_a;
   double wn, we;
   double g[3];
-  double shp, chp;
+  double sl, cl;
   double inv_p;
 };
 
@@ -57,11 +57,7 @@
     geodetic_sincos_p(r[0], r[1], r[2], sl, cl, p, o.inv_p, &ih, &ihy);
     sink.put(PCS_IH, ih); sink.put(PCS_IHY, ihy); sink.put(PCS_P, p);
   } else geodetic_sincos_p(r[0], r[1], r[2], sl, cl, p, o.inv_p);
-  {
-    double irt;
-    fsqrt_rsqrt(0.5 * (1.0 + cl), o.chp, irt);
-    o.shp = (0.5 * sl) * irt;
-  }
+  o.sl = sl; o.cl = cl;
   const double N = fdiv(kRa, fsqrt(1.0 - kE2 * sl * sl));
   const double q = fdiv(p, cl);
   const double alt = q - N;
@@ -92,8 +88,17 @@
   pc.air.iT = rho * tb.atm[33 + t.k] * frcp(P);
   pc.air.h = t.h; pc.air.k = t.k;
 }
-
-GEL_DEV bool pos_delta(const double r[3], int kk, double dlt, const PosPart& c, const PosCentre& pc, const Tables& tb, PosPart& o) {
+GEL_DEV void pos_centre_tail_kept(const PosCentreTail& t, double iT, double margin, const Tables& tb, PosCentre& pc, double& wn,
+                                  double& we) {
+  double wm;
+  wind_piece(t.h, t.piece, tb.wind, tb.winds, tb.Kw, wn, we, pc.s0, pc.s1, wm);
+  pc.margin = margin;
+  pc.air.iT = iT;
+  pc.air.h = t.h; pc.air.k = t.k;
+}
+
+GEL_DEV bool pos_delta(const double r[3], int kk, double dlt, const PosPart& c, const PosCentre& pc, const Tables& tb, PosPart& o,
+                       double* dlat_out = nullptr) {
   const bool along_z = kk == 2;
   const double a = r[2] * kRa, b = pc.p * kRb;
   double u = 0.0, dp = 0.0, dh2, dst, dct, dih, ih1;
@@ -129,9 +134,8 @@
   const double dlat = ((dzz * pc.cl - dpp * pc.sl) * pc.ihy) * (1.0 + e * (e - 1.0));
   const double hl2 = 0.5 * dlat * dlat;
   const double dsl = pc.cl * dlat - pc.sl * hl2, dcl = -(pc.sl * dlat + pc.cl * hl2);
-  const double hd = 0.5 * dlat, hd2 = 0.5 * hd * hd;
-  o.shp = c.shp + (c.chp * hd - c.shp * hd2);
-  o.chp = c.chp - (c.shp * hd + c.chp * hd2);
+  o.sl = pc.sl + dsl; o.cl = pc.cl + dcl;
+  if (dlat_out) *dlat_out = dlat;
   const double v = dcl * pc.icl;
   const double dq = ((dp - (pc.p * pc.icl) * dcl) * pc.icl) * (1.0 + v * (v - 1.0));
   const double nr = pc.N * (1.0 / kRa);
@@ -177,8 +181,20 @@
   return windy && !(inv_p > 0.0);
 #endif
 }
-GEL_DEV void wind_eci_chain(const double r[3], const EarthAngle& e, double s_hp, double c_hp, double inv_p, double wn,
+GEL_DEV void half_lat_pair(double sl, double cl, double& s_hp, double& c_hp) {
+  double irt;
+  fsqrt_rsqrt(0.5 * (1.0 + cl), c_hp, irt);
+  s_hp = (0.5 * sl) * irt;
+}
+GEL_DEV void half_lat_step(double s_hp, double c_hp, double dlat, double& s_hp1, double& c_hp1) {
+  const double hd = 0.5 * dlat, hd2 = 0.5 * hd * hd;
+  s_hp1 = s_hp + (c_hp * hd - s_hp * hd2);
+  c_hp1 = c_hp - (s_hp * hd + c_hp * hd2);
+}
+GEL_DEV void wind_eci_chain(const double r[3], const EarthAngle& e, double sl, double cl, double inv_p, double wn,
                             double we, double w[3]) {
+  double s_hp, c_hp;
+  half_lat_pair(sl, cl, s_hp, c_hp);
   const double px = r[0] * e.c + r[1] * e.s;
   const double py = -r[0] * e.s + r[1] * e.c;
   const double clon = (inv_p > 0.0) ? px * inv_p : 1.0, slon = py * inv_p;
@@ -202,16 +218,14 @@
   w[1] = q0 * t2 + q1 * t3 - q2 * t0 - q3 * t1;
   w[2] = q0 * t3 - q1 * t2 + q2 * t1 - q3 * t0;
 }
-GEL_DEV void wind_eci(const double r[3], const EarthAngle& e, double s_hp, double c_hp, double inv_p, double wn,
+GEL_DEV void wind_eci(const double r[3], const EarthAngle& e, double sl, double cl, double inv_p, double wn,
                       double we, double w[3]) {
 #if GEL_WIND_CHAIN
-  wind_eci_chain(r, e, s_hp, c_hp, inv_p, wn, we, w);
+  wind_eci_chain(r, e, sl, cl, inv_p, wn, we, w);
 #else
   const bool off_axis = inv_p > 0.0;
   const double clon = off_axis ? r[0] * inv_p : e.c;
   const double slon = off_axis ? r[1] * inv_p : e.s;
-  const double sl = fresh_mul(2.0 * s_hp, c_hp);
-  const double cl = fresh_mul(c_hp - s_hp, c_hp + s_hp);
   const double nh = -fresh_mul(wn, sl);
   w[0] = __builtin_fma(nh, clon, -fresh_mul(we, slon));
   w[1] = __builtin_fma(nh, slon, fresh_mul(we, clon));
@@ -219,7 +233,7 @@
 #endif
 }
 
-GEL_DEV void wind_eci_or_calm(const double r[3], const EarthAngle& e, double s_hp, double c_hp, double inv_p, double wn,
+GEL_DEV void wind_eci_or_calm(const double r[3], const EarthAngle& e, double sl, double cl, double inv_p, double wn,
                               double we, double w[3]) {
 #if GEL_CALM_SHORTCUT
   if (__builtin_amdgcn_ballot_w64(!(wn == 0.0 && we == 0.0)) == 0) {
@@ -227,9 +241,9 @@
     return;
   }
 #endif
-  wind_eci(r, e, s_hp, c_hp, inv_p, wn, we, w);
-}
-GEL_DEV void wind_eci_chain_or_calm(const double r[3], const EarthAngle& e, double s_hp, double c_hp, double inv_p, double wn,
+  wind_eci(r, e, sl, cl, inv_p, wn, we, w);
+}
+GEL_DEV void wind_eci_chain_or_calm(const double r[3], const EarthAngle& e, double sl, double cl, double inv_p, double wn,
                                     double we, double w[3]) {
 #if GEL_CALM_SHORTCUT
   if (__builtin_amdgcn_ballot_w64(!(wn == 0.0 && we == 0.0)) == 0) {
@@ -237,7 +251,7 @@
     return;
   }
 #endif
-  wind_eci_chain(r, e, s_hp, c_hp, inv_p, wn, we, w);
+  wind_eci_chain(r, e, sl, cl, inv_p, wn, we, w);
 }
 
 GEL_DEV void aero_force(const double r[3], const double v[3], double rho, double inv_a_sound, const double w[3], double area,
diff --git a/gelato_amd/csrc/gel_section_rhs.h b/gelato_amd/csrc/gel_section_rhs.h
--- a/gelato_amd/csrc/gel_section_rhs.h
+++ b/gelato_amd/csrc/gel_section_rhs.h
@@ -21,9 +21,9 @@
     double w[3], Fa[3];
     if constexpr (kDisp) {
       const double wn = pp.wn * fw, we = pp.we * fw;
-      wind_eci_or_calm(r, ea, pp.shp, pp.chp, pp.inv_p, wn, we, w);
+      wind_eci_or_calm(r, ea, pp.sl, pp.cl, pp.inv_p, wn, we, w);
     } else {
-      wind_eci_or_calm(r, ea, pp.shp, pp.chp, pp.inv_p, pp.wn, pp.we, w);
+      wind_eci_or_calm(r, ea, pp.sl, pp.cl, pp.inv_p, pp.wn, pp.we, w);
     }
     aero_force(r, v3, pp.rho, pp.inv_a, w, ph.area, tb, Fa);
     const double T = ph.thrust - ph.nozzle * pp.P;
diff --git a/gelato_amd/csrc/gel_section_rhs_lin.h b/gelato_amd/csrc/gel_section_rhs_lin.h
--- a/gelato_amd/csrc/gel_section_rhs_lin.h
+++ b/gelato_amd/csrc/gel_section_rhs_lin.h
@@ -27,7 +27,7 @@
   double w[3];
   L.wn = pp.wn * fw;
   L.we = pp.we * fw;
-  wind_eci_or_calm(r, L.ea, pp.shp, pp.chp, pp.inv_p, L.wn, L.we, w);
+  wind_eci_or_calm(r, L.ea, pp.sl, pp.cl, pp.inv_p, L.wn, L.we, w);
   aero_force(r, v3, pp.rho, pp.inv_a, w, ph.area, tb, L.Fa);
   L.T = ph.thrust - ph.nozzle * pp.P;
 #pragma unroll
diff --git a/gelato_amd/dynamics.py b/gelato_amd/dynamics.py
--- a/gelato_amd/dynamics.py
+++ b/gelato_amd/dynamics.py
@@ -49,8 +49,8 @@
 
 
 def point_eval(kind, x, aux=None):
-    nin = [1, 3, 3, 6, 7, 1, 1, 2, 2, 8, 8, 8, 7, 4, 1, 5][kind]
-    nout = [5, 3, 3, 3, 3, 3, 1, 4, 6, 8, 16, 4, 3, 7, 2, 18][kind]
+    nin = [1, 3, 3, 6, 7, 1, 1, 2, 2, 8, 8, 8, 7, 4, 1, 5, 5][kind]
+    nout = [5, 3, 3, 3, 3, 3, 1, 4, 6, 8, 16, 4, 3, 7, 2, 18, 54][kind]
     x = _f(x).reshape(-1, nin)
     n = x.shape[0]
     out = np.zeros((n, nout))
```
